# ShreyasBhaktharam/RDEIC

Hardware: AMD Instinct MI355X
Metric: 512x512 images/sec encode+relay-decode @ fixed bpp; 1/2/4/8 GPU (higher is better)
Workload: dtype bf16; 1 GPU; config 2: global batch 16 (16/GPU) 512x512, 2-step relay DDIM, encode+entropy-code+decode+VAE-decode; global_batch=16, image_size=512, ddim_steps=2, sampler=ddim, parallelism=dp1, codec_sessions_per_gpu=5

## Files before the change

### include/rdeic_hip.h

```cpp
#ifndef RDEIC_HIP_H
#define RDEIC_HIP_H
#include <stddef.h>
#include <stdint.h>
#ifdef __cplusplus
extern "C" {
#endif

int rdeic_version(void);
int rdeic_abi_count(void);

typedef struct rdeic_conv_desc {
  const void* in0;
  const void* in1;
  int32_t c0, c1;
  int32_t ld0, ld1;
  int32_t n, h, w;
  int32_t up2;
  const void* weight;
  int32_t wld;
  const float* bias;
  int32_t cout, kh, kw, stride, pad_t, pad_l;
  int32_t ho, wo;
  const float* gn_ab;
  int32_t gn_silu;
  const float* emb;
  int32_t emb_ld;
  int32_t act;
  float act_param;
  const void* res;
  int32_t res_ld;
  void* out;
  int32_t out_ld;
  int32_t out_mode;
  int32_t dtype;
  int32_t out_f32;
  int32_t batch;
  int64_t in_bs, w_bs, out_bs;
  float* gn_part;
  int32_t gn_hw;
  int32_t reserved;
  const float* ln_rows;
  const float* ln_colsum;
} rdeic_conv_desc;

int rdeic_conv2d(const rdeic_conv_desc* d, void* stream);
int rdeic_conv2d_tile(const rdeic_conv_desc* d, int32_t tile, void* stream);
int rdeic_conv2d_splitk(const rdeic_conv_desc* d, int32_t splits, float* ws, size_t ws_floats, void* stream);
int rdeic_conv2d_up2_phases(const rdeic_conv_desc* d, int64_t phase_stride, int32_t tile, void* stream);
int rdeic_conv2d_up2_group(const rdeic_conv_desc* d);
int rdeic_conv2d_band_rows(const rdeic_conv_desc* d, int32_t row_tile);
int rdeic_set_conv_path(int32_t path);
int rdeic_set_conv_option(int32_t key, int32_t value);

size_t rdeic_groupnorm_ws_floats(int32_t n, int32_t hw, int32_t c);
size_t rdeic_groupnorm_parts_floats(int64_t rows, int32_t c, int32_t hw);
int rdeic_groupnorm_parts_ab(const float* p0, int32_t c0, const float* p1, int32_t c1, int32_t n, int32_t hw,
                             int32_t groups, float eps, const float* gamma, const float* beta, float* ab,
                             void* stream);
int rdeic_groupnorm_stats(const void* x0, int32_t c0, int32_t ld0, const void* x1, int32_t c1, int32_t ld1,
                          int32_t n, int32_t hw, int32_t groups, float eps, const float* gamma, const float* beta,
                          float* ab, float* ws, int32_t dtype, void* stream);
int rdeic_groupnorm_parts_apply(const float* p0, int32_t c0, const float* p1, int32_t c1, const void* x0, int32_t ld0,
                                const void* x1, int32_t ld1, int32_t n, int32_t hw, int32_t groups, float eps,
                                const float* gamma, const float* beta, int32_t silu, float* ab, void* y, int32_t yld,
                                void* stream);
int rdeic_groupnorm_apply(const void* x, int32_t n, int32_t hw, int32_t c, int32_t ld, const float* ab,
                          int32_t ab_c, int32_t silu, float out_mul, void* y, int32_t yld, int32_t dtype,
                          void* stream);
int rdeic_layernorm(const void* x, int32_t rows, int32_t c, int32_t ld, const float* gamma, const float* beta,
                    float eps, void* y, int32_t yld, int32_t dtype, void* stream);

int rdeic_attention(const void* q, int32_t ldq, const void* k, int32_t ldk, const void* v, int32_t ldv,
                    void* o, int32_t ldo, int32_t batch, int32_t heads, int32_t lq, int32_t lk, int32_t dh,
                    float scale, int32_t kv_bcast, int32_t dtype, void* stream);
int rdeic_softmax_rows(const float* s, int64_t rows, int32_t cols, float scale, void* p, int32_t dtype, void* stream);
int rdeic_transpose(const void* in, int32_t rows, int32_t cols, int32_t ldin, void* out, int32_t ldout,
                    int32_t batch, int64_t in_bs, int64_t out_bs, int32_t dtype, void* stream);
int rdeic_attention_causal(const void* q, int32_t ldq, const void* k, int32_t ldk, const void* v, int32_t ldv,
                           void* o, int32_t ldo, int32_t batch, int32_t heads, int32_t l, int32_t dh,
                           float scale, int32_t dtype, void* stream);
int rdeic_embed_tokens(const float* table, int32_t ld_table, const float* pos, int32_t ld_pos, const int32_t* tokens,
                       int32_t batch, int32_t context, int32_t width, void* out, int32_t ld_out, int32_t dtype,
                       void* stream);

int rdeic_geglu(const void* in, int32_t rows, int32_t c, int32_t ldin, void* out, int32_t ldout,
                int32_t dtype, void* stream);
int rdeic_nchw_to_nhwc(const float* in, int32_t n, int32_t c, int32_t h, int32_t w, float mul, float add,
                       void* out, int32_t ld, int32_t dtype, void* stream);
int rdeic_nhwc_to_nchw(const void* in, int32_t n, int32_t c, int32_t h, int32_t w, int32_t ld, float mul,
                       float add, float* out, int32_t dtype, void* stream);
int rdeic_axpby(const float* x, const float* z, int32_t n_img, int32_t per_img, const float* a,
                const float* b, float* y, void* stream);
int rdeic_timestep_embedding(const int64_t* t, const float* freqs, int32_t n, int32_t dim, float* out, void* stream);
int rdeic_ddim_step(const float* x, const float* e, int64_t count, float c_sq1m, float c_sqa, float c_sqap,
                    float c_dir, float* xp, float* x0, void* stream);
int rdeic_cfg_combine(const float* e_cond, const float* e_uncond, int64_t count, float scale, float* out,
                      void* stream);
int rdeic_spaced_step(const float* x, const float* e, const float* noise, int64_t count, float a, float b, float c1,
                      float c2, float s, float* xp, float* x0, void* stream);
int rdeic_silu_f32(const float* x, float* y, int64_t count, void* stream);
int rdeic_image_u8_to_nhwc(const uint8_t* img, int32_t n, int32_t h, int32_t w, void* out, int32_t ld,
                           int32_t dtype, void* stream);
int rdeic_nhwc_to_image_u8(const void* x, int32_t n, int32_t h, int32_t w, int32_t ld, uint8_t* img,
                           int32_t dtype, void* stream);
int rdeic_image_mse(const uint8_t* a, const uint8_t* b, int32_t n, int64_t per_img, float* out, void* stream);
int rdeic_fill_uniform(float* out, int64_t count, uint64_t seed, float scale, float offset, void* stream);
int rdeic_pack_conv_weight(const float* w, int32_t cout, int32_t cin, int32_t kh, int32_t kw, void* out,
                           int32_t wld, int32_t dtype, void* stream);
int rdeic_cast(const void* in, int32_t in_dtype, void* out, int32_t out_dtype, int64_t count, void* stream);

int rdeic_resample_v_u8(const uint8_t* src, int64_t src_stride, int32_t src_row_bytes, int32_t src_row0,
                        int32_t src_rows, const int32_t* bounds, const int32_t* kk, int32_t ksize,
                        int32_t out_size, int32_t y0, int32_t nrows, int32_t cb0, int32_t ncb, uint8_t* dst,
                        int64_t dst_stride, void* stream);
int rdeic_resample_h_u8(const uint8_t* src, int64_t src_stride, int32_t src_h, int32_t src_w,
                        const int32_t* bounds, const int32_t* kk, int32_t ksize, int32_t out_size,
                        int32_t seg_max, int32_t y0, int32_t nrows, int32_t x0, int32_t npix, uint8_t* dst,
                        int64_t dst_stride, void* stream);
int rdeic_crop_flip_u8(const uint8_t* src, int64_t src_stride, int32_t src_h, int32_t src_w, int32_t crop_y,
                       int32_t crop_x, int32_t h, int32_t w, int32_t hflip, int32_t vflip, int32_t transpose,
                       uint8_t* dst, void* stream);

int rdeic_ckbd_encode(const void* y, int32_t yld, const void* params, int32_t pld, int32_t n, int32_t hy,
                      int32_t wy, int32_t c, int32_t phase, const float* scale_table, int32_t levels,
                      float scale_bound, int32_t* sym, int32_t* idx, int64_t img_stride, int64_t off,
                      void* yhat, int32_t yhld, void* anchor_out, int32_t ald, int32_t dtype, void* stream);
int rdeic_ckbd_indexes(const void* params, int32_t pld, int32_t n, int32_t hy, int32_t wy, int32_t c,
                       int32_t phase, const float* scale_table, int32_t levels, float scale_bound,
                       int32_t* idx, int64_t img_stride, int64_t off, int32_t dtype, void* stream);
int rdeic_ckbd_dequant(const int32_t* sym, const void* params, int32_t pld, int32_t n, int32_t hy,
                       int32_t wy, int32_t c, int32_t phase, int64_t img_stride, int64_t off, void* yhat,
                       int32_t yhld, void* anchor_out, int32_t ald, int32_t dtype, void* stream);
int rdeic_vq_argmin(const float* dot, const float* zn, const float* en, int32_t rows, int32_t ncode, int32_t* idx,
                    void* stream);
int rdeic_gather_rows(const float* table, int32_t ld_table, const int32_t* idx, int32_t rows, int32_t dim,
                      void* out, int32_t ld_out, int32_t dtype, void* stream);
int rdeic_row_sqnorm(const void* x, int32_t rows, int32_t dim, int32_t ld, float* out, int32_t dtype,
                     void* stream);

size_t rdeic_image_ssim_ws_floats(int32_t n, int32_t h, int32_t w, int32_t levels);
int rdeic_image_ssim(const uint8_t* a, const uint8_t* b, int32_t n, int32_t h, int32_t w, int32_t levels, float* ws,
                     size_t ws_floats, float* out, void* stream);

int rdeic_lpips_prep(const uint8_t* img, int32_t n, int32_t h, int32_t w, float* out, void* stream);
int rdeic_maxpool2d(const float* in, int32_t n, int32_t h, int32_t w, int32_t c, int32_t ld_in, int32_t k,
                    int32_t s, float* out, int32_t ld_out, void* stream);
size_t rdeic_lpips_layer_ws_floats(int32_t n, int64_t hw, int32_t c);
int rdeic_lpips_layer(const float* f0, int32_t ld0, const float* f1, int32_t ld1, const float* lin, int32_t n,
                      int64_t hw, int32_t c, int32_t accumulate, float* ws, size_t ws_floats, float* out,
                      void* stream);
int rdeic_lpips_prep_float(const void* img, int32_t ld, int32_t dtype, int64_t npix, float* out, void* stream);
int rdeic_lpips_layer_bwd(const float* f0, int32_t ld0, const float* f1, int32_t ld1, const float* lin,
                          const float* gscore, int32_t n, int64_t hw, int32_t c, int32_t accumulate, float* df0,
                          int32_t ldd, void* stream);
int rdeic_maxpool2d_bwd(const float* in, int32_t n, int32_t h, int32_t w, int32_t c, int32_t ld_in, const float* dy,
                        int32_t ld_dy, int32_t k, int32_t s, float* dx, int32_t ld_dx, void* stream);
int rdeic_conv_dgrad_small(const float* dz, int32_t ld_dz, const float* z, int32_t ld_z, const float* wt, int32_t n,
                           int32_t h, int32_t w, int32_t cin, int32_t cout, int32_t kh, int32_t kw, int32_t stride,
                           int32_t pad, int32_t prep_bwd, void* dx, int32_t ld_dx, int32_t dx_dtype, void* stream);

int rdeic_pmf_to_quantized_cdf(const float* pmf, int32_t n, int32_t precision, uint32_t* cdf_out);
int rdeic_build_gaussian_tables(const float* pmf, const int32_t* pmf_len, int32_t levels, int32_t pmf_ld,
                                int32_t* cdf, int32_t cdf_ld, int32_t* cdf_len, void* reserved);

int rdeic_rans_encode(const int32_t* sym, const int32_t* idx, size_t n, const int32_t* cdf, int32_t cdf_ld,
                      const int32_t* cdf_len, const int32_t* offset, int32_t levels, uint8_t* out, size_t cap,
                      size_t* out_len);
int rdeic_rans_encode_batch(int32_t count, const int32_t* sym, const int32_t* idx, size_t n_per,
                            size_t stride, const int32_t* cdf, int32_t cdf_ld, const int32_t* cdf_len,
                            const int32_t* offset, int32_t levels, uint8_t* out, size_t cap_per,
                            size_t* out_len, int32_t threads);
void* rdeic_rans_enc_tables_create(const int32_t* cdf, int32_t cdf_ld, const int32_t* cdf_len,
                                   const int32_t* offset, int32_t levels);
void rdeic_rans_enc_tables_destroy(void* tables);
int rdeic_rans_encode_batch_t(const void* tables, int32_t count, const int32_t* sym, const int32_t* idx,
                              size_t n_per, size_t stride, uint8_t* out, size_t cap_per, size_t* out_len,
                              int32_t threads);
int rdeic_rans_enc_quotient(const void* tables, int32_t row, int32_t value, uint64_t x, uint64_t* q);
void* rdeic_rans_dec_open(const uint8_t* data, size_t len);
int rdeic_rans_decode(void* handle, const int32_t* idx, size_t n, const int32_t* cdf, int32_t cdf_ld,
                      const int32_t* cdf_len, const int32_t* offset, int32_t levels, int32_t* out);
int rdeic_rans_decode_batch(int32_t count, void** handles, const int32_t* idx, size_t n_per, size_t stride,
                            const int32_t* cdf, int32_t cdf_ld, const int32_t* cdf_len, const int32_t* offset,
                            int32_t levels, int32_t* out, int32_t threads);
void rdeic_rans_dec_close(void* handle);

int rdeic_ac_encode(const int16_t* sym, size_t n, const int16_t* cdf_row, int32_t lp, uint8_t* out,
                    size_t cap, size_t* out_len);
int rdeic_ac_decode(const uint8_t* data, size_t len, size_t n, const int16_t* cdf_row, int32_t lp,
                    int16_t* out);
int rdeic_ac_uniform_cdf(int32_t codebook_size, int16_t* cdf_row);

#define RDEIC_PROF_CONV 0
#define RDEIC_PROF_ATTN 1
#define RDEIC_PROF_ATTN_SMALL 2
#define RDEIC_PROF_GN_STATS 3
#define RDEIC_PROF_GN_APPLY 4
#define RDEIC_PROF_GEMM 5
#define RDEIC_PROF_ATTN_D512 6
#define RDEIC_PROF_CONV_BYTES 7
int rdeic_prof_start(int32_t capacity, int32_t every);
int rdeic_prof_read_keys(int32_t kind, int64_t* keys, int64_t* launches, double* work, double* ms, int32_t cap);
#define RDEIC_COUNT_HALO_CONV 0
#define RDEIC_COUNT_GN_APPLY 1
#define RDEIC_COUNT_LAYERNORM 2
#define RDEIC_COUNT_HALO_SMALL 3
#define RDEIC_COUNT_LN_FUSED 4
#define RDEIC_COUNT_SPLITK 5
#define RDEIC_COUNT_EDGE 6
#define RDEIC_COUNT_GN_PARTS_APPLY 7
#define RDEIC_COUNT_DMA_CONV 8
#define RDEIC_COUNT_UP2_PHASES 9
#define RDEIC_COUNT_KINDS 10
int64_t rdeic_launch_count(int32_t kind);
int rdeic_layernorm_rowstats(const void* x, int32_t rows, int32_t c, int32_t ld, float eps, float* ms,
                             void* stream);
int rdeic_launch_count_reset(void);
int rdeic_prof_stop(void);
int rdeic_prof_read(int32_t kind, int64_t* launches, double* work, double* ms);

typedef struct rdeic_gemm_desc {
  const void* a;
  int64_t a_bs1, a_bs2, a_sm, a_sk;
  const void* b;
  int64_t b_bs1, b_bs2, b_sk, b_sn;
  void* c;
  int64_t c_bs1, c_bs2, c_sm;
  int32_t batch, nb2, m, n, k, ksplit, dtype, c_f32;
  float alpha, beta;
  float* rsum;
  int64_t rsum_bs;
} rdeic_gemm_desc;
int rdeic_gemm_strided(const rdeic_gemm_desc* d, void* stream);
int rdeic_pack_conv_weight_dgrad(const float* w, int32_t cout, int32_t cin, int32_t kh, int32_t kw, void* out,
                                 int32_t wld, int32_t to_bf16, void* stream);
typedef struct rdeic_pack_job {
  const float* w;
  void* out;
  int64_t start;
  int32_t cout, cin, kh, kw, wld, mode;
} rdeic_pack_job;
int rdeic_pack_batch(const rdeic_pack_job* jobs, int32_t njobs, int64_t total, int32_t row_floats, int32_t to_bf16,
                     void* stream);
int rdeic_zero_insert2(const void* src, int32_t n, int32_t h, int32_t w, int32_t c, int32_t ld, void* dst,
                       int32_t dst_ld, int32_t dtype, void* stream);
int rdeic_sum_pool2(const void* src, int32_t n, int32_t h, int32_t w, int32_t c, int32_t ld, void* dst,
                    int32_t dst_ld, int32_t dtype, void* stream);
int rdeic_pixel_unshuffle2(const void* src, int32_t n, int32_t h, int32_t w, int32_t c, int32_t ld, void* dst,
                           int32_t dst_ld, int32_t dtype, void* stream);
int rdeic_im2col(const void* x, int32_t n, int32_t h, int32_t w, int32_t c, int32_t ld, int32_t kh, int32_t kw,
                 int32_t stride, int32_t pad_t, int32_t pad_l, int32_t ho, int32_t wo, int32_t up2, void* out,
                 int64_t out_ld, int32_t dtype, void* stream);
int rdeic_wgrad_finalize(const float* part, int32_t splits, int32_t cout, int32_t cin, int32_t kh, int32_t kw,
                         float* dw, int32_t accumulate, const float* rpart, float* db, void* stream);
size_t rdeic_col_sum_ws_floats(int64_t rows, int32_t c, int32_t groups);
int rdeic_col_sum(const void* x, int64_t rows, int32_t c, int32_t ld, int32_t groups, float* out, int32_t accumulate,
                  float* ws, size_t ws_floats, int32_t dtype, void* stream);
int rdeic_act_fwd(const void* z, int64_t rows, int32_t c, int32_t ldz, const void* res, int32_t ldr, int32_t act,
                  float slope, void* out, int32_t ldo, int32_t dtype, void* stream);
int rdeic_act_bwd(const void* dy, int32_t ldy, const void* z, int32_t ldz, int64_t rows, int32_t c, int32_t act,
                  float slope, void* dz, int32_t lddz, int32_t dtype, void* stream);
size_t rdeic_gn_train_ws_doubles(int32_t n, int32_t hw, int32_t c);
int rdeic_gn_train_fwd(const void* x, int32_t ldx, int32_t n, int32_t hw, int32_t c, int32_t groups, float eps,
                       const float* gamma, const float* beta, float* mr, float* ab, double* ws, int32_t dtype,
                       void* stream);
int rdeic_gn_train_bwd(const void* x, int32_t ldx, const void* dy, int32_t ldy, int32_t n, int32_t hw, int32_t c,
                       int32_t groups, const float* mr, const float* gamma, const float* beta, int32_t silu, void* dx,
                       int32_t lddx, float* dgamma, float* dbeta, int32_t accumulate, double* ws, float* coef,
                       int32_t dtype, void* stream);
int rdeic_gn_train_bwd_res(const void* x, int32_t ldx, const void* dy, int32_t ldy, int32_t n, int32_t hw, int32_t c,
                           int32_t groups, const float* mr, const float* gamma, const float* beta, int32_t silu,
                           const void* dres, int32_t ldr, void* dx, int32_t lddx, float* dgamma, float* dbeta,
                           int32_t accumulate, double* ws, float* coef, int32_t dtype, void* stream);
size_t rdeic_layernorm_bwd_ws_floats(int64_t rows, int32_t c);
int rdeic_layernorm_bwd(const void* x, int32_t ldx, int64_t rows, int32_t c, const float* gamma, float eps,
                        const void* dy, int32_t ldy, void* dx, int32_t lddx, float* dgamma, float* dbeta,
                        int32_t accumulate, float* ws, size_t ws_floats, int32_t dtype, void* stream);
int rdeic_layernorm_bwd_res(const void* x, int32_t ldx, int64_t rows, int32_t c, const float* gamma, float eps,
                            const void* dy, int32_t ldy, const void* dres, int32_t ldr, void* dx, int32_t lddx,
                            float* dgamma, float* dbeta, int32_t accumulate, float* ws, size_t ws_floats,
                            int32_t dtype, void* stream);
int rdeic_softmax_bwd_rows(const void* p, const float* dp, int64_t rows, int32_t cols, float scale, void* ds,
                           int32_t dtype, void* stream);
int rdeic_attention_fwd_lse(const void* q, int32_t ldq, const void* k, int32_t ldk, const void* v, int32_t ldv,
                            void* o, int32_t ldo, float* lse, int32_t batch, int32_t heads, int32_t lq, int32_t lk,
                            int32_t dh, float scale, int32_t dtype, void* stream);
size_t rdeic_attention_bwd_workspace(int32_t batch, int32_t heads, int32_t lq, int32_t lk, int32_t dh);
int rdeic_attention_bwd(const void* q, int32_t ldq, const void* k, int32_t ldk, const void* v, int32_t ldv,
                        const void* o, int32_t ldo, const void* d_o, int32_t lddo, const float* lse,
                        void* dq, int32_t lddq, void* dk, int32_t lddk, void* dv, int32_t lddv,
                        void* ws, size_t ws_bytes, int32_t batch, int32_t heads, int32_t lq, int32_t lk,
                        int32_t dh, float scale, int32_t dtype, void* stream);
int rdeic_geglu_bwd(const void* x, int32_t ldx, int64_t rows, int32_t c, const void* dy, int32_t ldy, void* dx,
                    int32_t lddx, int32_t dtype, void* stream);
int rdeic_ckbd_train_anchor(const void* y, int32_t ldy, const void* pa, int32_t ldpa, int32_t n, int32_t h, int32_t w,
                            int32_t c, void* out, int32_t ldo, int32_t dtype, void* stream);
int rdeic_ckbd_mask(const void* x, int32_t ldx, int32_t n, int32_t h, int32_t w, int32_t c, int32_t which, void* out,
                    int32_t ldo, int32_t dtype, void* stream);
size_t rdeic_ckbd_train_ws_doubles(int32_t n, int32_t h, int32_t w, int32_t c);
int rdeic_ckbd_train_lik(const void* y, int32_t ldy, const void* pa, int32_t ldpa, const void* pn, int32_t ldpn,
                         const float* noise, int32_t n, int32_t h, int32_t w, int32_t c, void* nonanchor_hat,
                         int32_t ldo, double* ws, float* out2, int32_t dtype, void* stream);
int rdeic_ckbd_train_lik_bwd(const void* y, int32_t ldy, const void* pa, int32_t ldpa, const void* pn, int32_t ldpn,
                             const float* noise, int32_t n, int32_t h, int32_t w, int32_t c, const float* g_sum,
                             const void* d_nonanchor, int32_t ldd, void* dy, int32_t lddy, void* dpa, int32_t lddpa,
                             void* dpn, int32_t lddpn, int32_t dtype, void* stream);
int rdeic_vq_train(const float* dot, const float* zn, const float* en, const float* z, const int32_t* idx, int32_t P,
                   int32_t K, int32_t D, float* E, float* embed_prob, float beta, float decay, float temp,
                   float* code_out, float* dE_unit, float* loss3, void* stream);
int rdeic_vq_z_grad(const float* z, const float* zq, const void* dzq, int64_t count, const float* g_loss, float coef,
                    void* dz, int32_t dtype, void* stream);
int rdeic_scale_dev(const float* x, int64_t count, const float* s, float* y, int32_t accumulate, void* stream);
int rdeic_adamw(float* p, const float* g, float* m, float* v, int64_t count, float lr, float beta1, float beta2,
                float eps, float weight_decay, int32_t step, void* stream);
int rdeic_adamw_dev(float* p, const float* g, float* m, float* v, int64_t count, float lr, float beta1, float beta2,
                    float eps, float weight_decay, const float* step_scalars, void* stream);

#ifdef __cplusplus
}
#endif
#endif
```

### rdeic_amd/_lib.py

```python
from __future__ import annotations

import ctypes as C
import os
import threading

_HERE = os.path.dirname(os.path.abspath(__file__))
LIB_PATH = os.environ.get("RDEIC_LIB") or os.path.join(_HERE, "lib", "librdeic_hip.so")

EINVAL, ENOSPC, EBADMSG, ELAUNCH = -22, -28, -74, -5
_ERRNAMES = {EINVAL: "EINVAL (bad argument/shape)", ENOSPC: "ENOSPC (output capacity)",
             EBADMSG: "EBADMSG (corrupt or truncated bitstream)", ELAUNCH: "kernel launch failure"}


class RdeicError(RuntimeError):
    def __init__(self, fn: str, code: int):
        super().__init__(f"{fn} failed: {code} {_ERRNAMES.get(code, '')}")
        self.code = code


class BitstreamError(RdeicError, ValueError):
    """Corrupt / truncated bitstream (the reference's 'decode failure')."""


class ConvDesc(C.Structure):
    _fields_ = [
        ("in0", C.c_void_p), ("in1", C.c_void_p),
        ("c0", C.c_int32), ("c1", C.c_int32), ("ld0", C.c_int32), ("ld1", C.c_int32),
        ("n", C.c_int32), ("h", C.c_int32), ("w", C.c_int32), ("up2", C.c_int32),
        ("weight", C.c_void_p), ("wld", C.c_int32),
        ("bias", C.c_void_p),
        ("cout", C.c_int32), ("kh", C.c_int32), ("kw", C.c_int32), ("stride", C.c_int32),
        ("pad_t", C.c_int32), ("pad_l", C.c_int32),
        ("ho", C.c_int32), ("wo", C.c_int32),
        ("gn_ab", C.c_void_p), ("gn_silu", C.c_int32),
        ("emb", C.c_void_p), ("emb_ld", C.c_int32),
        ("act", C.c_int32), ("act_param", C.c_float),
        ("res", C.c_void_p), ("res_ld", C.c_int32),
        ("out", C.c_void_p), ("out_ld", C.c_int32), ("out_mode", C.c_int32),
        ("dtype", C.c_int32), ("out_f32", C.c_int32),
        ("batch", C.c_int32), ("in_bs", C.c_int64), ("w_bs", C.c_int64), ("out_bs", C.c_int64),
        ("gn_part", C.c_void_p), ("gn_hw", C.c_int32), ("reserved", C.c_int32),
        ("ln_rows", C.c_void_p), ("ln_colsum", C.c_void_p),
    ]


class GemmDesc(C.Structure):
    _fields_ = [
        ("a", C.c_void_p), ("a_bs1", C.c_int64), ("a_bs2", C.c_int64), ("a_sm", C.c_int64), ("a_sk", C.c_int64),
        ("b", C.c_void_p), ("b_bs1", C.c_int64), ("b_bs2", C.c_int64), ("b_sk", C.c_int64), ("b_sn", C.c_int64),
        ("c", C.c_void_p), ("c_bs1", C.c_int64), ("c_bs2", C.c_int64), ("c_sm", C.c_int64),
        ("batch", C.c_int32), ("nb2", C.c_int32), ("m", C.c_int32), ("n", C.c_int32), ("k", C.c_int32),
        ("ksplit", C.c_int32), ("dtype", C.c_int32), ("c_f32", C.c_int32),
        ("alpha", C.c_float), ("beta", C.c_float), ("rsum", C.c_void_p), ("rsum_bs", C.c_int64),
    ]


_p, _i32, _i64, _u64, _f, _sz = C.c_void_p, C.c_int32, C.c_int64, C.c_uint64, C.c_float, C.c_size_t

PROTOTYPES = {
    "rdeic_version": (C.c_int, []),
    "rdeic_abi_count": (C.c_int, []),
    "rdeic_conv2d": (C.c_int, [C.POINTER(ConvDesc), _p]),
    "rdeic_conv2d_splitk": (C.c_int, [C.POINTER(ConvDesc), _i32, _p, C.c_size_t, _p]),
    "rdeic_conv2d_tile": (C.c_int, [C.POINTER(ConvDesc), _i32, _p]),
    "rdeic_conv2d_up2_phases": (C.c_int, [C.POINTER(ConvDesc), _i64, _i32, _p]),
    "rdeic_conv2d_up2_group": (C.c_int, [C.POINTER(ConvDesc)]),
    "rdeic_conv2d_band_rows": (C.c_int, [C.POINTER(ConvDesc), _i32]),
    "rdeic_prof_start": (C.c_int, [_i32, _i32]),
    "rdeic_prof_stop": (C.c_int, []),
    "rdeic_launch_count": (C.c_int64, [_i32]),
    "rdeic_launch_count_reset": (C.c_int, []),
    "rdeic_layernorm_rowstats": (C.c_int, [C.c_void_p, _i32, _i32, _i32, C.c_float, C.c_void_p, C.c_void_p]),
    "rdeic_prof_read": (C.c_int, [_i32, C.POINTER(C.c_int64), C.POINTER(C.c_double), C.POINTER(C.c_double)]),
    "rdeic_prof_read_keys": (C.c_int, [_i32, C.POINTER(C.c_int64), C.POINTER(C.c_int64), C.POINTER(C.c_double),
                                       C.POINTER(C.c_double), _i32]),
    "rdeic_groupnorm_ws_floats": (_sz, [_i32, _i32, _i32]),
    "rdeic_groupnorm_stats": (C.c_int, [_p, _i32, _i32, _p, _i32, _i32, _i32, _i32, _i32, _f, _p, _p, _p, _p,
                                        _i32, _p]),
    "rdeic_groupnorm_apply": (C.c_int, [_p, _i32, _i32, _i32, _i32, _p, _i32, _i32, _f, _p, _i32, _i32, _p]),
    "rdeic_set_conv_path": (C.c_int, [_i32]),
    "rdeic_set_conv_option": (C.c_int, [_i32, _i32]),
    "rdeic_layernorm": (C.c_int, [_p, _i32, _i32, _i32, _p, _p, _f, _p, _i32, _i32, _p]),
    "rdeic_softmax_rows": (C.c_int, [_p, _i64, _i32, _f, _p, _i32, _p]),
    "rdeic_transpose": (C.c_int, [_p, _i32, _i32, _i32, _p, _i32, _i32, _i64, _i64, _i32, _p]),
    "rdeic_attention": (C.c_int, [_p, _i32, _p, _i32, _p, _i32, _p, _i32, _i32, _i32, _i32, _i32, _i32, _f,
                                  _i32, _i32, _p]),
    "rdeic_attention_causal": (C.c_int, [_p, _i32, _p, _i32, _p, _i32, _p, _i32, _i32, _i32, _i32, _i32, _f, _i32,
                                         _p]),
    "rdeic_embed_tokens": (C.c_int, [_p, _i32, _p, _i32, _p, _i32, _i32, _i32, _p, _i32, _i32, _p]),
    "rdeic_geglu": (C.c_int, [_p, _i32, _i32, _i32, _p, _i32, _i32, _p]),
    "rdeic_nchw_to_nhwc": (C.c_int, [_p, _i32, _i32, _i32, _i32, _f, _f, _p, _i32, _i32, _p]),
    "rdeic_nhwc_to_nchw": (C.c_int, [_p, _i32, _i32, _i32, _i32, _i32, _f, _f, _p, _i32, _p]),
    "rdeic_axpby": (C.c_int, [_p, _p, _i32, _i32, _p, _p, _p, _p]),
    "rdeic_timestep_embedding": (C.c_int, [_p, _p, _i32, _i32, _p, _p]),
    "rdeic_ddim_step": (C.c_int, [_p, _p, _i64, _f, _f, _f, _f, _p, _p, _p]),
    "rdeic_spaced_step": (C.c_int, [_p, _p, _p, _i64, _f, _f, _f, _f, _f, _p, _p, _p]),
    "rdeic_cfg_combine": (C.c_int, [_p, _p, _i64, _f, _p, _p]),
    "rdeic_silu_f32": (C.c_int, [_p, _p, _i64, _p]),
    "rdeic_image_u8_to_nhwc": (C.c_int, [_p, _i32, _i32, _i32, _p, _i32, _i32, _p]),
    "rdeic_nhwc_to_image_u8": (C.c_int, [_p, _i32, _i32, _i32, _i32, _p, _i32, _p]),
    "rdeic_image_mse": (C.c_int, [_p, _p, _i32, _i64, _p, _p]),
    "rdeic_fill_uniform": (C.c_int, [_p, _i64, _u64, _f, _f, _p]),
    "rdeic_pack_conv_weight": (C.c_int, [_p, _i32, _i32, _i32, _i32, _p, _i32, _i32, _p]),
    "rdeic_cast": (C.c_int, [_p, _i32, _p, _i32, _i64, _p]),
    "rdeic_resample_v_u8": (C.c_int, [_p, _i64, _i32, _i32, _i32, _p, _p, _i32, _i32, _i32, _i32, _i32, _i32, _p,
                                      _i64, _p]),
    "rdeic_resample_h_u8": (C.c_int, [_p, _i64, _i32, _i32, _p, _p, _i32, _i32, _i32, _i32, _i32, _i32, _i32, _p,
                                      _i64, _p]),
    "rdeic_crop_flip_u8": (C.c_int, [_p, _i64, _i32, _i32, _i32, _i32, _i32, _i32, _i32, _i32, _i32, _p, _p]),
    "rdeic_ckbd_encode": (C.c_int, [_p, _i32, _p, _i32, _i32, _i32, _i32, _i32, _i32, _p, _i32, _f, _p, _p,
                                    _i64, _i64, _p, _i32, _p, _i32, _i32, _p]),
    "rdeic_ckbd_indexes": (C.c_int, [_p, _i32, _i32, _i32, _i32, _i32, _i32, _p, _i32, _f, _p, _i64, _i64,
                                     _i32, _p]),
    "rdeic_ckbd_dequant": (C.c_int, [_p, _p, _i32, _i32, _i32, _i32, _i32, _i32, _i64, _i64, _p, _i32, _p,
                                     _i32, _i32, _p]),
    "rdeic_vq_argmin": (C.c_int, [_p, _p, _p, _i32, _i32, _p, _p]),
    "rdeic_gather_rows": (C.c_int, [_p, _i32, _p, _i32, _i32, _p, _i32, _i32, _p]),
    "rdeic_row_sqnorm": (C.c_int, [_p, _i32, _i32, _i32, _p, _i32, _p]),
    "rdeic_pmf_to_quantized_cdf": (C.c_int, [_p, _i32, _i32, _p]),
    "rdeic_build_gaussian_tables": (C.c_int, [_p, _p, _i32, _i32, _p, _i32, _p, _p]),
    "rdeic_rans_encode": (C.c_int, [_p, _p, _sz, _p, _i32, _p, _p, _i32, _p, _sz, C.POINTER(_sz)]),
    "rdeic_rans_encode_batch": (C.c_int, [_i32, _p, _p, _sz, _sz, _p, _i32, _p, _p, _i32, _p, _sz, _p, _i32]),
    "rdeic_image_ssim_ws_floats": (C.c_size_t, [_i32, _i32, _i32, _i32]),
    "rdeic_image_ssim": (C.c_int, [_p, _p, _i32, _i32, _i32, _i32, _p, C.c_size_t, _p, _p]),
    "rdeic_lpips_prep": (C.c_int, [_p, _i32, _i32, _i32, _p, _p]),
    "rdeic_maxpool2d": (C.c_int, [_p, _i32, _i32, _i32, _i32, _i32, _i32, _i32, _p, _i32, _p]),
    "rdeic_lpips_layer_ws_floats": (_sz, [_i32, _i64, _i32]),
    "rdeic_lpips_layer": (C.c_int, [_p, _i32, _p, _i32, _p, _i32, _i64, _i32, _i32, _p, _sz, _p, _p]),
    "rdeic_lpips_prep_float": (C.c_int, [_p, _i32, _i32, _i64, _p, _p]),
    "rdeic_lpips_layer_bwd": (C.c_int, [_p, _i32, _p, _i32, _p, _p, _i32, _i64, _i32, _i32, _p, _i32, _p]),
    "rdeic_maxpool2d_bwd": (C.c_int, [_p, _i32, _i32, _i32, _i32, _i32, _p, _i32, _i32, _i32, _p, _i32, _p]),
    "rdeic_conv_dgrad_small": (C.c_int, [_p, _i32, _p, _i32, _p, _i32, _i32, _i32, _i32, _i32, _i32, _i32, _i32,
                                         _i32, _i32, _p, _i32, _i32, _p]),
    "rdeic_groupnorm_parts_floats": (C.c_size_t, [_i64, _i32, _i32]),
    "rdeic_groupnorm_parts_ab": (C.c_int, [_p, _i32, _p, _i32, _i32, _i32, _i32, _f, _p, _p, _p, _p]),
    "rdeic_groupnorm_parts_apply": (C.c_int, [_p, _i32, _p, _i32, _p, _i32, _p, _i32, _i32, _i32, _i32, _f, _p, _p,
                                              _i32, _p, _p, _i32, _p]),
    "rdeic_rans_enc_tables_create": (_p, [_p, _i32, _p, _p, _i32]),
    "rdeic_rans_enc_tables_destroy": (None, [_p]),
    "rdeic_rans_encode_batch_t": (C.c_int, [_p, _i32, _p, _p, _sz, _sz, _p, _sz, _p, _i32]),
    "rdeic_rans_enc_quotient": (C.c_int, [_p, _i32, _i32, C.c_uint64, C.POINTER(C.c_uint64)]),
    "rdeic_rans_dec_open": (_p, [_p, _sz]),
    "rdeic_rans_decode": (C.c_int, [_p, _p, _sz, _p, _i32, _p, _p, _i32, _p]),
    "rdeic_rans_decode_batch": (C.c_int, [_i32, _p, _p, _sz, _sz, _p, _i32, _p, _p, _i32, _p, _i32]),
    "rdeic_rans_dec_close": (None, [_p]),
    "rdeic_ac_encode": (C.c_int, [_p, _sz, _p, _i32, _p, _sz, C.POINTER(_sz)]),
    "rdeic_ac_decode": (C.c_int, [_p, _sz, _sz, _p, _i32, _p]),
    "rdeic_ac_uniform_cdf": (C.c_int, [_i32, _p]),
    "rdeic_gemm_strided": (C.c_int, [C.POINTER(GemmDesc), _p]),
    "rdeic_pack_conv_weight_dgrad": (C.c_int, [_p, _i32, _i32, _i32, _i32, _p, _i32, _i32, _p]),
    "rdeic_pack_batch": (C.c_int, [_p, _i32, _i64, _i32, _i32, _p]),
    "rdeic_zero_insert2": (C.c_int, [_p, _i32, _i32, _i32, _i32, _i32, _p, _i32, _i32, _p]),
    "rdeic_sum_pool2": (C.c_int, [_p, _i32, _i32, _i32, _i32, _i32, _p, _i32, _i32, _p]),
    "rdeic_pixel_unshuffle2": (C.c_int, [_p, _i32, _i32, _i32, _i32, _i32, _p, _i32, _i32, _p]),
    "rdeic_im2col": (C.c_int, [_p, _i32, _i32, _i32, _i32, _i32, _i32, _i32, _i32, _i32, _i32, _i32, _i32, _i32, _p,
                               _i64, _i32, _p]),
    "rdeic_wgrad_finalize": (C.c_int, [_p, _i32, _i32, _i32, _i32, _i32, _p, _i32, _p, _p, _p]),
    "rdeic_col_sum_ws_floats": (_sz, [_i64, _i32, _i32]),
    "rdeic_col_sum": (C.c_int, [_p, _i64, _i32, _i32, _i32, _p, _i32, _p, _sz, _i32, _p]),
    "rdeic_act_fwd": (C.c_int, [_p, _i64, _i32, _i32, _p, _i32, _i32, _f, _p, _i32, _i32, _p]),
    "rdeic_act_bwd": (C.c_int, [_p, _i32, _p, _i32, _i64, _i32, _i32, _f, _p, _i32, _i32, _p]),
    "rdeic_gn_train_ws_doubles": (_sz, [_i32, _i32, _i32]),
    "rdeic_gn_train_fwd": (C.c_int, [_p, _i32, _i32, _i32, _i32, _i32, _f, _p, _p, _p, _p, _p, _i32, _p]),
    "rdeic_gn_train_bwd": (C.c_int, [_p, _i32, _p, _i32, _i32, _i32, _i32, _i32, _p, _p, _p, _i32, _p, _i32, _p, _p,
                                     _i32, _p, _p, _i32, _p]),
    "rdeic_gn_train_bwd_res": (C.c_int, [_p, _i32, _p, _i32, _i32, _i32, _i32, _i32, _p, _p, _p, _i32, _p, _i32, _p,
                                         _i32, _p, _p, _i32, _p, _p, _i32, _p]),
    "rdeic_layernorm_bwd_ws_floats": (_sz, [_i64, _i32]),
    "rdeic_layernorm_bwd": (C.c_int, [_p, _i32, _i64, _i32, _p, _f, _p, _i32, _p, _i32, _p, _p, _i32, _p, _sz, _i32,
                                      _p]),
    "rdeic_layernorm_bwd_res": (C.c_int, [_p, _i32, _i64, _i32, _p, _f, _p, _i32, _p, _i32, _p, _i32, _p, _p, _i32, _p,
                                          _sz, _i32, _p]),
    "rdeic_softmax_bwd_rows": (C.c_int, [_p, _p, _i64, _i32, _f, _p, _i32, _p]),
    "rdeic_attention_fwd_lse": (C.c_int, [_p, _i32, _p, _i32, _p, _i32, _p, _i32, _p, _i32, _i32, _i32, _i32, _i32, _f,
                                          _i32, _p]),
    "rdeic_attention_bwd_workspace": (_sz, [_i32, _i32, _i32, _i32, _i32]),
    "rdeic_attention_bwd": (C.c_int, [_p, _i32, _p, _i32, _p, _i32, _p, _i32, _p, _i32, _p, _p, _i32, _p, _i32, _p,
                                      _i32, _p, _sz, _i32, _i32, _i32, _i32, _i32, _f, _i32, _p]),
    "rdeic_geglu_bwd": (C.c_int, [_p, _i32, _i64, _i32, _p, _i32, _p, _i32, _i32, _p]),
    "rdeic_ckbd_train_anchor": (C.c_int, [_p, _i32, _p, _i32, _i32, _i32, _i32, _i32, _p, _i32, _i32, _p]),
    "rdeic_ckbd_mask": (C.c_int, [_p, _i32, _i32, _i32, _i32, _i32, _i32, _p, _i32, _i32, _p]),
    "rdeic_ckbd_train_ws_doubles": (_sz, [_i32, _i32, _i32, _i32]),
    "rdeic_ckbd_train_lik": (C.c_int, [_p, _i32, _p, _i32, _p, _i32, _p, _i32, _i32, _i32, _i32, _p, _i32, _p, _p,
                                       _i32, _p]),
    "rdeic_ckbd_train_lik_bwd": (C.c_int, [_p, _i32, _p, _i32, _p, _i32, _p, _i32, _i32, _i32, _i32, _p, _p, _i32, _p,
                                           _i32, _p, _i32, _p, _i32, _i32, _p]),
    "rdeic_vq_train": (C.c_int, [_p, _p, _p, _p, _p, _i32, _i32, _i32, _p, _p, _f, _f, _f, _p, _p, _p, _p]),
    "rdeic_vq_z_grad": (C.c_int, [_p, _p, _p, _i64, _p, _f, _p, _i32, _p]),
    "rdeic_scale_dev": (C.c_int, [_p, _i64, _p, _p, _i32, _p]),
    "rdeic_adamw": (C.c_int, [_p, _p, _p, _p, _i64, _f, _f, _f, _f, _f, _i32, _p]),
    "rdeic_adamw_dev": (C.c_int, [_p, _p, _p, _p, _i64, _f, _f, _f, _f, _f, _p, _p]),
}

_lib = None
_lock = threading.Lock()


def load() -> C.CDLL:
    global _lib
    if _lib is not None:
        return _lib
    with _lock:
        if _lib is not None:
            return _lib
        if not os.path.exists(LIB_PATH):
            raise ImportError(f"librdeic_hip.so not built at {LIB_PATH}; run `make` (or __graft_entry__.build()).")
        import torch
        lib = C.CDLL(LIB_PATH, mode=C.RTLD_GLOBAL)
        for name, (res, args) in PROTOTYPES.items():
            fn = getattr(lib, name)
            fn.restype = res
            fn.argtypes = args
        _lib = lib
    return _lib


def check(name: str, rc: int) -> None:
    if rc != 0:
        if rc == EBADMSG:
            raise BitstreamError(name, rc)
# ... 24 lines not shown
```

### rdeic_amd/compression.py

```python
from __future__ import annotations

from typing import List, Sequence, Tuple

import numpy as np
import torch

from . import coders, ops
from .params import ParamStore
from .plan import PlanCache, host_step

LEAK = 0.01


class Compression:
    def __init__(self, store: ParamStore, in_nc: int, out_nc: int, N: int, M: int, slice_num: int,
                 slice_ch: Sequence[int], codebook_size: int, prefix: str = "preprocess_model."):
        self.store, self.p = store, prefix
        self.N, self.M = N, M
        self.slice_num, self.slice_ch = slice_num, list(slice_ch)
        self.slice_off = [sum(self.slice_ch[:i]) for i in range(slice_num)]
        self.codebook_size = codebook_size
        p = prefix
        d = store
        self.g_a = []
        spec = [("rb", in_nc, M), ("rb", M, M), ("rb", M, M), ("rb", M, M), ("rbs", M, M), ("rb", M, M),
                ("rb", M, M), ("rb", M, M)]
        for i, (kind, ci, co) in enumerate(spec):
            self.g_a.append(self._declare_block(f"{p}encoder.g_a.{i}", kind, ci, co))
        d.declare_conv(f"{p}encoder.g_a.8", M, M, 3)
        self.g_a.append((f"{p}encoder.g_a.8", "conv", M, M))
        self.hyper_enc = [self._declare_block(f"{p}hyper_enc.hyper_enc.{i}", k, ci, co) for i, (k, ci, co) in
                          enumerate([("rb", M, N), ("rb", N, N), ("rbs", N, N), ("rbs", N, N)])]
        self.hyper_dec = [self._declare_block(f"{p}hyper_dec.hyper_dec.{i}", k, ci, co) for i, (k, ci, co) in
                          enumerate([("rbu", N, M), ("rbu", M, M), ("rb", M, M * 3 // 2), ("rb", M * 3 // 2, M * 2)])]
        d.declare_conv(f"{p}decoder.g_s.0", M, M, 3)
        self.g_s = [(f"{p}decoder.g_s.0", "conv", M, M)]
        for i, (k, ci, co) in enumerate([("rb", M, M)] * 3 + [("rbu", M, M)] + [("rb", M, M)] * 4):
            self.g_s.append(self._declare_block(f"{p}decoder.g_s.{i + 1}", k, ci, co))
        d.declare_conv(f"{p}out", out_nc, M, 3)
        for i, c in enumerate(self.slice_ch):
            d.declare_conv(f"{p}local_context.{i}", 2 * c, c, 5)
            if i:
                cin = sum(self.slice_ch[:i])
                d.declare_conv(f"{p}channel_context.{i}.fushion.0", 224, cin, 5)
                d.declare_conv(f"{p}channel_context.{i}.fushion.2", 128, 224, 5)
                d.declare_conv(f"{p}channel_context.{i}.fushion.4", 2 * c, 128, 5)
            for nm, cin in (("entropy_parameters_anchor", 2 * M + (2 * c if i else 0)),
                            ("entropy_parameters_nonanchor", 2 * M + (4 * c if i else 2 * c))):
                out = 2 * c
                d.declare_conv(f"{p}{nm}.{i}.fusion.0", out * 5 // 3, cin, 1)
                d.declare_conv(f"{p}{nm}.{i}.fusion.2", out * 4 // 3, out * 5 // 3, 1)
                d.declare_conv(f"{p}{nm}.{i}.fusion.4", out, out * 4 // 3, 1)
        d.declare(f"{p}quantize.embedding.weight", (codebook_size, N))
        self.tables = None
        self._en = None
        self.coder_groups = 1
        self.use_plans = True
        self._plans = PlanCache()
        self._io = {}

    def _declare_block(self, pre, kind, ci, co):
        d = self.store
        if kind == "rb":
            d.declare_conv(pre + ".conv1", co, ci, 3)
            d.declare_conv(pre + ".conv2", co, co, 3)
            if ci != co:
                d.declare_conv(pre + ".adaptor", co, ci, 1)
        elif kind == "rbs":
            d.declare_conv(pre + ".conv1", co, ci, 3)
            d.declare_conv(pre + ".conv2", co, co, 3)
            d.declare_conv(pre + ".downsample", co, ci, 1)
        elif kind == "rbu":
            d.declare_conv(pre + ".subpel_conv.0", co * 4, ci, 1)
            d.declare_conv(pre + ".conv", co, co, 3)
            d.declare_conv(pre + ".upsample.0", co * 4, ci, 1)
        return (pre, kind, ci, co)

    def update(self, scale_table=None, force: bool = False):
        if self.tables is None or force or scale_table is not None:
            self.tables = coders.GaussianTables(scale_table)
            self._plans.clear()
        return True

    def _block(self, blk, x):
        pre, kind, ci, co = blk
        s = self.store
        if kind == "conv":
            return ops.conv2d(x, s.conv(pre))
        if kind == "rb":
            identity = x if ci == co else ops.conv2d(x, s.conv(pre + ".adaptor"))
            out = ops.conv2d(x, s.conv(pre + ".conv1"), act=ops.LEAKY, slope=LEAK)
            return ops.conv2d(out, s.conv(pre + ".conv2"), act=ops.LEAKY, slope=LEAK, res=identity)
        if kind == "rbs":
            out = ops.conv2d(x, s.conv(pre + ".conv1", stride=2, pad=1), act=ops.LEAKY, slope=LEAK)
            identity = ops.conv2d(x, s.conv(pre + ".downsample", stride=2, pad=0))
            return ops.conv2d(out, s.conv(pre + ".conv2"), act=ops.LEAKY, slope=0.1, res=identity)
        if kind == "rbu":
            out = ops.conv2d(x, s.conv(pre + ".subpel_conv.0"), pixel_shuffle=True, act=ops.LEAKY, slope=LEAK)
            identity = ops.conv2d(x, s.conv(pre + ".upsample.0"), pixel_shuffle=True)
            return ops.conv2d(out, s.conv(pre + ".conv"), act=ops.LEAKY, slope=0.1, res=identity)
        raise ValueError(kind)

    def _seq(self, blocks, x):
        for b in blocks:
            x = self._block(b, x)
        return x

    def _pad_width(self, c: int):
        if self.store.compute_dtype != torch.bfloat16:
            return None
        return -(-c // 64) * 64 if c > 32 else -(-c // 16) * 16

    def _ep(self, name: str, i: int, x: torch.Tensor, x2: torch.Tensor) -> torch.Tensor:
        s, p = self.store, self.p
        f0, f2, f4 = (f"{p}{name}.{i}.fusion.{j}" for j in (0, 2, 4))
        w0, w2 = s.shapes[f0 + ".weight"][0], s.shapes[f2 + ".weight"][0]
        p0, p2 = self._pad_width(w0), self._pad_width(w2)
        h = ops.conv2d(x, s.conv(f0, cout_pad=p0), x2=x2, act=ops.GELU)
        h = ops.conv2d(h, s.conv(f2, cin_pad=p0, cout_pad=p2), act=ops.GELU)
        return ops.conv2d(h, s.conv(f4, cin_pad=p2))

    def _channel_ctx(self, i: int, yhat_prefix: torch.Tensor, out: torch.Tensor) -> torch.Tensor:
        s, p = self.store, self.p
        f0, f2, f4 = (f"{p}channel_context.{i}.fushion.{j}" for j in (0, 2, 4))
        p0 = self._pad_width(s.shapes[f0 + ".weight"][0])
        h = ops.conv2d(yhat_prefix, s.conv(f0, cout_pad=p0), act=ops.GELU)
        h = ops.conv2d(h, s.conv(f2, cin_pad=p0), act=ops.GELU)
        return ops.conv2d(h, s.conv(f4), out=out)

    def _codebook(self) -> torch.Tensor:
        return self.store.get(self.p + "quantize.embedding.weight")

    def vq_quant(self, z: torch.Tensor):
        B, hz, wz, N = z.shape
        rows = B * hz * wz
        E = self._codebook()
        zf = ops.cast(z.contiguous(), torch.float32).view(rows, N)
        zn = torch.empty(rows, dtype=torch.float32, device=z.device)
        ops.call("rdeic_row_sqnorm", zf.data_ptr(), rows, N, N, zn.data_ptr(), 0, ops.stream_ptr())
        if self._en is None or self._en.device != z.device:
            self._en = torch.empty(E.shape[0], dtype=torch.float32, device=z.device)
            ops.call("rdeic_row_sqnorm", E.data_ptr(), E.shape[0], N, N, self._en.data_ptr(), 0, ops.stream_ptr())
        dot = ops.linear(zf, self.store.conv(self.p + "quantize.embedding", dtype=torch.float32), images=B)
        idx = torch.empty(rows, dtype=torch.int32, device=z.device)
        ops.call("rdeic_vq_argmin", dot.data_ptr(), zn.data_ptr(), self._en.data_ptr(), rows, E.shape[0],
                 idx.data_ptr(), ops.stream_ptr())
        return self.codebook_entry(idx, B, hz, wz), idx.view(B, hz, wz)

    def codebook_entry(self, idx: torch.Tensor, B: int, hz: int, wz: int) -> torch.Tensor:
        E = self._codebook()
        N = E.shape[1]
        zq = torch.empty((B, hz, wz, N), dtype=self.store.compute_dtype, device=E.device)
        ops.call("rdeic_gather_rows", E.data_ptr(), N, idx.contiguous().data_ptr(), B * hz * wz, N, zq.data_ptr(), N,
                 ops.dt_code(zq), ops.stream_ptr())
        return zq

    def _pinned(self, key: str, n: int, dtype=torch.int32) -> torch.Tensor:
        cache = self.__dict__.setdefault("_pin_cache", {})
        buf = cache.get(key)
        if buf is None or buf.numel() < n or buf.dtype != dtype:
            buf = torch.empty(max(n, 1), dtype=dtype, pin_memory=True)
            cache[key] = buf
        return buf[:n]

    def stage_sizes(self, hy: int, wy: int) -> List[int]:
        sizes = []
        for c in self.slice_ch:
            sizes += [c * hy * (wy // 2)] * 2
        return sizes

    def _stage_common(self, hy, wy, B, device, dt):
        yhat = torch.empty((B, hy, wy, self.M), dtype=dt, device=device)
        cmax = max(self.slice_ch)
        ctx = torch.empty((B, hy, wy, 4 * cmax), dtype=dt, device=device)
        anchor = torch.empty((B, hy, wy, cmax), dtype=dt, device=device)
        return yhat, ctx, anchor

    def _stage_gen(self, hyper, hy, wy, emit, bufs):
        yhat, ctxbuf, anchor_full = bufs
        off = 0
        for i, c in enumerate(self.slice_ch):
            s0 = self.slice_off[i]
            ctx = ctxbuf[..., :4 * c]
            anchor = anchor_full[..., :c]
            if i == 0:
                pa = self._ep("entropy_parameters_anchor", 0, hyper, None)
            else:
                self._channel_ctx(i, yhat[..., :s0], out=ctx[..., 2 * c:4 * c])
                pa = self._ep("entropy_parameters_anchor", i, ctx[..., 2 * c:4 * c], hyper)
            r = emit(i, 0, pa, c, off, yhat[..., s0:s0 + c], anchor)
            if r is not None:
                yield from r
            off += c * hy * (wy // 2)
            ops.conv2d(anchor, self.store.conv(f"{self.p}local_context.{i}"), out=ctx[..., :2 * c])
            pn = self._ep("entropy_parameters_nonanchor", i, ctx[..., :(4 * c if i else 2 * c)], hyper)
            r = emit(i, 1, pn, c, off, yhat[..., s0:s0 + c], None)
            if r is not None:
                yield from r
            off += c * hy * (wy // 2)

    def _run_stages(self, hyper, B, hy, wy, emit):
        bufs = self._stage_common(hy, wy, B, hyper.device, hyper.dtype)
        for _ in self._stage_gen(hyper, hy, wy, emit, bufs):
            pass
        return bufs[0]

    def _groups(self, B: int) -> List[Tuple[int, int]]:
        g = max(1, min(int(self.coder_groups), B))
        cut = [B * k // g for k in range(g + 1)]
        return [(cut[k], cut[k + 1]) for k in range(g)]

    @staticmethod
    def _interleave(gens) -> None:
        live = list(gens)
        while live:
            for g in list(live):
                try:
                    next(g)
                except StopIteration:
                    live.remove(g)

    def _run_region(self, name, fn, inputs, before=None):
        if not self.use_plans:
            if before is not None:
                before()
            return fn(*inputs)
        key = (name, self.coder_groups) + tuple((tuple(t.shape), t.dtype) for t in inputs)
        return self._plans.run(key, fn, inputs, before=before)

    def _splitk(self):
        import contextlib
        if self.store.compute_dtype == torch.bfloat16 and ops.SPLITK_ENTROPY:
            return ops.splitk_allowed()
        return contextlib.nullcontext()

    def _compress_gpu(self, h: torch.Tensor) -> torch.Tensor:
        with self._splitk():
            return self._compress_gpu_body(h)

    def _compress_gpu_body(self, h: torch.Tensor) -> torch.Tensor:
        B = h.shape[0]
        y = self._seq(self.g_a, h)
        z = self._seq(self.hyper_enc, y)
        z_q, z_idx = self.vq_quant(z)
        hyper = self._seq(self.hyper_dec, z_q)
        _, hy, wy, _ = y.shape
        total = sum(self.stage_sizes(hy, wy))
        table = self.tables.device_scale_table(h.device)
        dtc = ops.dt_code(h)
        bufs = self._stage_common(hy, wy, B, h.device, hyper.dtype)
        zi_p = self._pinned("enc_zidx", z_idx.numel()).view(z_idx.shape)
        host_step(lambda: zi_p.copy_(z_idx, non_blocking=True))

        def group(gi: int, b0: int, b1: int):
            nb = b1 - b0
            yg = y[b0:b1]
            sym_p = self._pinned(f"enc_sym{gi}", nb * total).view(nb, total)
            idx_p = self._pinned(f"enc_idx{gi}", nb * total).view(nb, total)
            done = torch.cuda.Event()

            def emit(i, phase, params, c, off, yhat_slice, anchor):
                s0 = self.slice_off[i]
                ys = yg[..., s0:s0 + c]
                ops.call("rdeic_ckbd_encode", ys.data_ptr(), ops.pix_ld(ys), params.data_ptr(), ops.pix_ld(params), nb,
                         hy, wy, c, phase, table.data_ptr(), table.numel(), float(coders.SCALE_BOUND), sym_p.data_ptr(),
                         idx_p.data_ptr(), total, off, yhat_slice.data_ptr(), ops.pix_ld(yhat_slice),
                         None if anchor is None else anchor.data_ptr(), 0 if anchor is None else ops.pix_ld(anchor),
                         dtc, ops.stream_ptr())

            yield from self._stage_gen(hyper[b0:b1], hy, wy, emit, [t[b0:b1] for t in bufs])

            def to_host():
                done.record()
# ... 113 lines not shown
```

### rdeic_amd/csrc/coders.cpp

```cpp
#include <stdint.h>
#include <string.h>

#include <algorithm>
#include <atomic>
#include <condition_variable>
#include <functional>
#include <mutex>
#include <cmath>
#include <new>
#include <stdexcept>
#include <thread>
#include <vector>

#include "../../include/rdeic_hip.h"

#define RDEIC_OK 0
#define RDEIC_EINVAL (-22)
#define RDEIC_ENOSPC (-28)
#define RDEIC_EBADMSG (-74)

namespace {

constexpr int kPrecision = 16;
constexpr uint32_t kBypassBits = 4;
// ... 244 lines not shown
  }
  return d->bad ? RDEIC_EBADMSG : RDEIC_OK;
}

class WorkerPool {
 public:
  static WorkerPool& get() {
    thread_local WorkerPool* p = new WorkerPool();
    return *p;
  }
  void run(int32_t count, int32_t threads, const std::function<void(int32_t)>& f) {
    std::lock_guard<std::mutex> job(job_mu_);
    int32_t helpers = std::max(0, std::min(threads, count) - 1);
    while ((int32_t)workers_.size() < helpers) {
      const int32_t id = (int32_t)workers_.size();
      try {
        workers_.reserve(workers_.size() + 1);
        std::thread(&WorkerPool::loop, this, id).detach();
      } catch (...) {
        helpers = (int32_t)workers_.size();
        break;
      }
      workers_.push_back(id);
    }
    {
      std::lock_guard<std::mutex> lk(mu_);
      fn_ = &f;
      count_ = count;
      next_.store(0);
      helpers_ = helpers;
      active_ = helpers;
      ++gen_;
    }
    cv_.notify_all();
    work();
    std::unique_lock<std::mutex> lk(mu_);
    done_cv_.wait(lk, [&] { return active_ == 0; });
    fn_ = nullptr;
  }

 private:
  void work() {
    for (;;) {
      const int32_t i = next_.fetch_add(1);
      if (i >= count_) break;
      (*fn_)(i);
    }
  }
  void loop(int32_t id) {
    uint64_t seen = 0;
    for (;;) {
      {
        std::unique_lock<std::mutex> lk(mu_);
        cv_.wait(lk, [&] { return gen_ != seen; });
        seen = gen_;
        if (id >= helpers_) continue;
      }
      work();
      std::lock_guard<std::mutex> lk(mu_);
      if (--active_ == 0) done_cv_.notify_all();
    }
  }

  std::mutex job_mu_, mu_;
  std::condition_variable cv_, done_cv_;
  std::vector<int32_t> workers_;
  const std::function<void(int32_t)>* fn_ = nullptr;
  std::atomic<int32_t> next_{0};
  int32_t count_ = 0, active_ = 0, helpers_ = 0;
  uint64_t gen_ = 0;
};

template <typename F>
int guard(F&& f) noexcept {
  try {
    return f();
  } catch (const std::bad_alloc&) {
    return RDEIC_ENOSPC;
  } catch (...) {
    return RDEIC_EINVAL;
  }
}

template <typename F>
void parallel_for(int32_t count, int32_t threads, F&& f) {
  if (threads <= 1 || count <= 1) {
    for (int32_t i = 0; i < count; ++i) f(i);
    return;
  }
  const std::function<void(int32_t)> fn = f;
  WorkerPool::get().run(count, threads, fn);
}

struct BitWriter {
  uint8_t* out;
  size_t cap;
  size_t len = 0;
  uint8_t cache = 0;
  int count = 0;
  bool overflow = false;
  void put(int bit) {
    cache = (uint8_t)((cache << 1) | (bit & 1));
    if (++count == 8) {
      if (len < cap) out[len] = cache; else overflow = true;
      ++len;
      count = 0;
      cache = 0;
    }
  }
  void put_with_pending(int bit, uint64_t& pending) {
    put(bit);
    while (pending > 0) { put(!bit); --pending; }
  }
  void flush() {
    while (count > 0) put(0);
  }
};

struct BitReader {
  const uint8_t* in;
  size_t n;
  size_t ptr = 0;
  uint8_t cache = 0;
  int cached = 0;
  void get(uint32_t& value) {
    if (cached == 0) {
      if (ptr == n) { value <<= 1; return; }
      cache = in[ptr++];
      cached = 8;
    }
    value = (value << 1) | ((cache >> (cached - 1)) & 1);
    --cached;
  }
};

inline uint16_t binsearch_u16(const uint16_t* cdf, uint16_t target, uint16_t max_sym) {
  uint16_t left = 0, right = (uint16_t)(max_sym + 1);
  while (left + 1 < right) {
    const uint16_t m = (uint16_t)((left + right) / 2);
    const uint16_t v = cdf[m];
    if (v < target) left = m;
    else if (v > target) right = m;
    else return m;
  }
  return left;
}

}

extern "C" {

int rdeic_version(void) { return 1; }

int rdeic_abi_count(void) { return 112; }

static int pmf_to_quantized_cdf_impl(const float* pmf, int32_t n, int32_t precision, uint32_t* cdf_out) {
  if (!pmf || !cdf_out || n <= 0 || precision <= 0 || precision > 24) return RDEIC_EINVAL;
  for (int32_t i = 0; i < n; ++i)
    if (!(pmf[i] >= 0.f) || !std::isfinite(pmf[i])) return RDEIC_EINVAL;
  const uint32_t one = 1u << precision;
  std::vector<uint32_t> cdf((size_t)n + 1);
  cdf[0] = 0;
  for (int32_t i = 0; i < n; ++i) cdf[i + 1] = (uint32_t)std::round(pmf[i] * (float)one);
  uint64_t total = 0;
  for (uint32_t v : cdf) total += v;
  if (total == 0) return RDEIC_EINVAL;
  for (auto& v : cdf) v = (uint32_t)(((uint64_t)one * v) / total);
  for (size_t i = 1; i < cdf.size(); ++i) cdf[i] += cdf[i - 1];
  cdf.back() = one;
  const int32_t m = (int32_t)cdf.size();
  for (int32_t i = 0; i < m - 1; ++i) {
    if (cdf[i] == cdf[i + 1]) {
      uint32_t best_freq = ~0u;
      int32_t best = -1;
      for (int32_t j = 0; j < m - 1; ++j) {
        const uint32_t f = cdf[j + 1] - cdf[j];
        if (f > 1 && f < best_freq) { best_freq = f; best = j; }
      }
      if (best < 0) return RDEIC_EINVAL;
      if (best < i) {
        for (int32_t j = best + 1; j <= i; ++j) cdf[j]--;
      } else {
        for (int32_t j = i + 1; j <= best; ++j) cdf[j]++;
      }
    }
  }
  memcpy(cdf_out, cdf.data(), cdf.size() * sizeof(uint32_t));
  return RDEIC_OK;
}

int rdeic_pmf_to_quantized_cdf(const float* pmf, int32_t n, int32_t precision, uint32_t* cdf_out) {
  return guard([&] { return pmf_to_quantized_cdf_impl(pmf, n, precision, cdf_out); });
}

static int build_gaussian_tables_impl(const float* pmf, const int32_t* pmf_len, int32_t levels, int32_t pmf_ld,
                                      int32_t* cdf, int32_t cdf_ld, int32_t* cdf_len) {
  if (!pmf || !pmf_len || !cdf || !cdf_len || levels <= 0) return RDEIC_EINVAL;
  std::vector<float> row;
  std::vector<uint32_t> q;
  for (int32_t i = 0; i < levels; ++i) {
    const int32_t L = pmf_len[i];
    if (L <= 0 || L + 1 > pmf_ld || L + 2 > cdf_ld) return RDEIC_EINVAL;
    row.assign(pmf + (size_t)i * pmf_ld, pmf + (size_t)i * pmf_ld + L + 1);
    q.assign((size_t)L + 2, 0u);
    int rc = pmf_to_quantized_cdf_impl(row.data(), L + 1, kPrecision, q.data());
    if (rc) return rc;
    int32_t* out = cdf + (size_t)i * cdf_ld;
    for (int32_t j = 0; j < cdf_ld; ++j) out[j] = j < L + 2 ? (int32_t)q[j] : 0;
    cdf_len[i] = L + 2;
  }
  return RDEIC_OK;
}

int rdeic_build_gaussian_tables(const float* pmf, const int32_t* pmf_len, int32_t levels, int32_t pmf_ld, int32_t* cdf,
                                int32_t cdf_ld, int32_t* cdf_len, void* reserved) {
  (void)reserved;
  return guard([&] { return build_gaussian_tables_impl(pmf, pmf_len, levels, pmf_ld, cdf, cdf_ld, cdf_len); });
}

int rdeic_rans_encode(const int32_t* sym, const int32_t* idx, size_t n, const int32_t* cdf, int32_t cdf_ld,
                      const int32_t* cdf_len, const int32_t* offset, int32_t levels, uint8_t* out, size_t cap,
                      size_t* out_len) {
  if ((!sym || !idx) && n) return RDEIC_EINVAL;
  if (!cdf || !cdf_len || !offset || !out || !out_len || levels <= 0) return RDEIC_EINVAL;
  return guard([&] {
    std::vector<RansSym> syms;
    std::vector<uint32_t> words;
    return rans_encode_impl(sym, idx, n, cdf, cdf_ld, cdf_len, offset, levels, out, cap, out_len, syms, words);
  });
}

int rdeic_rans_encode_batch(int32_t count, const int32_t* sym, const int32_t* idx, size_t n_per, size_t stride,
                            const int32_t* cdf, int32_t cdf_ld, const int32_t* cdf_len, const int32_t* offset,
                            int32_t levels, uint8_t* out, size_t cap_per, size_t* out_len, int32_t threads) {
  if (count <= 0 || !sym || !idx || !out || !out_len) return RDEIC_EINVAL;
  return guard([&] {
    std::vector<int> rc(count, 0);
    parallel_for(count, threads, [&](int32_t i) {
      rc[i] = guard([&] {
        std::vector<RansSym> syms;
        std::vector<uint32_t> words;
        return rans_encode_impl(sym + i * stride, idx + i * stride, n_per, cdf, cdf_ld, cdf_len, offset, levels,
                                out + i * cap_per, cap_per, &out_len[i], syms, words);
      });
    });
    for (int v : rc)
      if (v) return v;
    return (int)RDEIC_OK;
  });
}

void* rdeic_rans_enc_tables_create(const int32_t* cdf, int32_t cdf_ld, const int32_t* cdf_len, const int32_t* offset,
                                   int32_t levels) {
  if (!cdf || !cdf_len || !offset || levels <= 0 || cdf_ld < 2) return nullptr;
  EncTables* T = new (std::nothrow) EncTables();
  if (!T) return nullptr;
  try {
    T->levels = levels;
    T->row_off.resize(levels);
    T->max_value.resize(levels);
    T->offset.assign(offset, offset + levels);
    size_t total = 0;
    for (int32_t ci = 0; ci < levels; ++ci) {
      const int32_t len = cdf_len[ci];
      if (len < 2 || len > cdf_ld) throw std::invalid_argument("cdf_len");
      T->row_off[ci] = (int32_t)total;
      T->max_value[ci] = len - 2;
      total += (size_t)len - 1;
    }
    T->sym.resize(total);
    for (int32_t ci = 0; ci < levels; ++ci) {
      const int32_t* row = cdf + (size_t)ci * cdf_ld;
      for (int32_t v = 0; v <= T->max_value[ci]; ++v) {
        const int32_t start = row[v], freq = row[v + 1] - row[v];
        if (start < 0 || freq <= 0 || start + freq > (1 << kPrecision)) throw std::invalid_argument("cdf row");
        T->sym[(size_t)T->row_off[ci] + v] = make_enc_sym((uint32_t)start, (uint32_t)freq);
      }
    }
  } catch (...) {
    delete T;
    return nullptr;
  }
  return T;
}

void rdeic_rans_enc_tables_destroy(void* tables) { delete (EncTables*)tables; }

int rdeic_rans_encode_batch_t(const void* tables, int32_t count, const int32_t* sym, const int32_t* idx, size_t n_per,
                              size_t stride, uint8_t* out, size_t cap_per, size_t* out_len, int32_t threads) {
  if (!tables || count <= 0 || ((!sym || !idx) && n_per) || !out || !out_len) return RDEIC_EINVAL;
  const EncTables& T = *(const EncTables*)tables;
  return guard([&] {
    std::vector<int> rc(count, 0);
    parallel_for(count, threads, [&](int32_t i) {
      rc[i] = guard([&] {
        thread_local std::vector<uint32_t> buf;
        return rans_encode_tab_impl(T, sym + i * stride, idx + i * stride, n_per, out + i * cap_per, cap_per,
                                    &out_len[i], buf);
      });
    });
    for (int v : rc)
      if (v) return v;
    return (int)RDEIC_OK;
  });
}

int rdeic_rans_enc_quotient(const void* tables, int32_t row, int32_t value, uint64_t x, uint64_t* q) {
// ... 151 lines not shown
```

### rdeic_amd/csrc/conv_common.h

```cpp
#pragma once
#include "common.h"
#include "../../include/rdeic_hip.h"
#include "prof.h"

namespace rdeic_conv {

struct ConvArgs {
  const char* in0; const char* in1;
  int c0, c1, ld0, ld1;
  int n, h, w, up2;
  const char* weight; int wld;
  const float* bias;
  int cout, kh, kw, stride, pad_t, pad_l, ho, wo;
  const float* gn_ab; int gn_silu;
  const float* emb; int emb_ld;
  int act; float act_param;
  const char* res; int res_ld;
  char* out; int out_ld, out_mode;
  int out_f32;
  int M, cin, ktot, nk;
  long in_bs, w_bs, out_bs;
  int batch;
  int epi_vec;
  int splits, kper;
// ... 316 lines not shown
  constexpr int WTM = BM / WGM;
  return (WTM == 32 || WTM == 64) && (WTM / P) % 16 == 0;
}

template <int BM, int BN, int WGM, int WGN, int NT, int P>
__device__ __forceinline__ void epilogue_geglu(const f32x4 (&acc)[BM / WGM / 16][BN / WGN / 16], const ConvArgs& a,
                                               int m0, int n0, int wm, int wn, int lane, int tid, char* lds) {
  constexpr int WTM = BM / WGM, WTN = BN / WGN;
  constexpr int TM = WTM / 16, TN = WTN / 16;
  constexpr int HM = TM / P;
  constexpr int PR = BM / P;
  constexpr int SDW = BN + 4;
  constexpr int DPR = BN / 16;
  constexpr int ND = (PR * DPR + NT - 1) / NT;
  constexpr int NPF = ND < 2 ? ND : 2;
  constexpr bool HOIST = (NT % DPR) == 0;
  static_assert(TM % P == 0 && BN % 16 == 0, "P passes, chunk pairs");
  const int lr = lane & 15, lq = lane >> 4;
  float* L = reinterpret_cast<float*>(lds);
  auto bar = []() { asm volatile("s_waitcnt lgkmcnt(0)\n\ts_barrier" ::: "memory"); };
  auto row_of = [&](int d, int p) {
    const int pr = d / DPR;
    const int wmr = pr / (WTM / P), wr = pr - wmr * (WTM / P);
    return m0 + wmr * WTM + p * (WTM / P) + wr;
  };
  float4 bh[4], chh[4];
#pragma unroll
  for (int q = 0; q < 4; ++q) bh[q] = chh[q] = float4{0.f, 0.f, 0.f, 0.f};
  if constexpr (HOIST) {
    const int nn = n0 + (tid % DPR) * 16;
    if (nn < a.cout) {
#pragma unroll
      for (int q = 0; q < 4; ++q) {
        if (a.bias) bh[q] = *reinterpret_cast<const float4*>(a.bias + nn + 4 * q);
        if (a.ln_rows) chh[q] = *reinterpret_cast<const float4*>(a.ln_cs + nn + 4 * q);
      }
    }
  }
#pragma unroll
  for (int p = 0; p < P; ++p) {
    float2 lpf[NPF];
#pragma unroll
    for (int k = 0; k < NPF; ++k) {
      const int d = tid + k * NT;
      const int m = row_of(d, p);
      lpf[k] = float2{0.f, 0.f};
      if (a.ln_rows && d < PR * DPR && m < a.M) lpf[k] = reinterpret_cast<const float2*>(a.ln_rows)[m];
    }
    bar();
#pragma unroll
    for (int ii = 0; ii < HM; ++ii)
#pragma unroll
      for (int r = 0; r < 4; ++r) {
        const int pr = wm * (WTM / P) + ii * 16 + lq * 4 + r;
#pragma unroll
        for (int j = 0; j < TN; ++j) L[pr * SDW + wn * WTN + j * 16 + lr] = acc[p * HM + ii][j][r];
      }
    bar();
#pragma unroll
    for (int k = 0; k < ND; ++k) {
      const int d = tid + k * NT;
      if (d >= PR * DPR) continue;
      const int pr = d / DPR, cq = d - pr * DPR;
      const int m = row_of(d, p);
      const int nn = n0 + cq * 16;
      if (m >= a.M || nn >= a.cout) continue;
      float v[16];
#pragma unroll
      for (int q = 0; q < 4; ++q) {
        const float4 x = *reinterpret_cast<const float4*>(L + pr * SDW + cq * 16 + 4 * q);
        v[4 * q] = x.x; v[4 * q + 1] = x.y; v[4 * q + 2] = x.z; v[4 * q + 3] = x.w;
      }
      if (a.ln_rows) {
        const float2 ms = k < NPF ? lpf[k < NPF ? k : 0] : reinterpret_cast<const float2*>(a.ln_rows)[m];
        const f32x2 nm = {-ms.x, -ms.x}, rs = {ms.y, ms.y};
#pragma unroll
        for (int q = 0; q < 4; ++q) {
          const float4 c = HOIST ? chh[q] : *reinterpret_cast<const float4*>(a.ln_cs + nn + 4 * q);
          const float cs[4] = {c.x, c.y, c.z, c.w};
#pragma unroll
          for (int e = 0; e < 4; e += 2) {
            const f32x2 r = rs * pk_fma(nm, f32x2{cs[e], cs[e + 1]}, f32x2{v[4 * q + e], v[4 * q + e + 1]});
            v[4 * q + e] = r.x;
            v[4 * q + e + 1] = r.y;
          }
        }
      }
      if (a.bias) {
#pragma unroll
        for (int q = 0; q < 4; ++q) {
          const float4 b = HOIST ? bh[q] : *reinterpret_cast<const float4*>(a.bias + nn + 4 * q);
          const f32x2 r0 = f32x2{v[4 * q], v[4 * q + 1]} + f32x2{b.x, b.y};
          const f32x2 r1 = f32x2{v[4 * q + 2], v[4 * q + 3]} + f32x2{b.z, b.w};
          v[4 * q] = r0.x; v[4 * q + 1] = r0.y; v[4 * q + 2] = r1.x; v[4 * q + 3] = r1.y;
        }
      }
#pragma unroll
      for (int e = 0; e < 16; ++e) v[e] = apply_act(v[e], a.act, a.act_param);
      bf16 gv[8];
#pragma unroll
      for (int h = 0; h < 2; ++h)
#pragma unroll
        for (int e = 0; e < 4; e += 2) {
          const f32x2 xv = {to_f32(from_f32<bf16>(v[8 * h + e])), to_f32(from_f32<bf16>(v[8 * h + e + 1]))};
          const f32x2 gt = {to_f32(from_f32<bf16>(v[8 * h + 4 + e])), to_f32(from_f32<bf16>(v[8 * h + 5 + e]))};
          const f32x2 r = xv * gelu_fast2(gt);
          gv[4 * h + e] = from_f32<bf16>(r.x);
          gv[4 * h + e + 1] = from_f32<bf16>(r.y);
        }
      *reinterpret_cast<uint4*>(reinterpret_cast<bf16*>(a.out) + (long)m * a.out_ld + (nn >> 1)) =
          *reinterpret_cast<uint4*>(gv);
    }
  }
}

constexpr unsigned kOOB = 0x80000000u;

template <int N>
__device__ __forceinline__ void wait_vm() {
  asm volatile("s_waitcnt vmcnt(%0)" ::"n"(N) : "memory");
}

__device__ __forceinline__ int dma_key(int r) { return (((r >> 3) & 1) << 1) | (((r >> 1) & 1) << 2); }

typedef __attribute__((address_space(3))) void* lds_ptr_t;

__device__ __forceinline__ void dma16(__amdgpu_buffer_rsrc_t rs, char* lds_dst, unsigned voff, int soff) {
  __builtin_amdgcn_raw_ptr_buffer_load_lds(rs, (lds_ptr_t)lds_dst, 16, (int)voff, soff, 0, 0);
}

#ifdef RDEIC_HALO_STAMPS
__device__ unsigned long long* g_halo_stamps;
#define HALO_STAMP(k)                                                                      \
  do {                                                                                     \
    if (threadIdx.x == 0) g_halo_stamps[(long)blockIdx.x * 8 + (k)] = __builtin_amdgcn_s_memtime(); \
  } while (0)
#else
#define HALO_STAMP(k) do {} while (0)
#endif

__device__ __forceinline__ void wait_vm_rt(int n) {
  switch (n) {
    case 0: wait_vm<0>(); break;
    case 1: wait_vm<1>(); break;
    case 2: wait_vm<2>(); break;
    case 3: wait_vm<3>(); break;
    case 4: wait_vm<4>(); break;
    case 5: wait_vm<5>(); break;
    case 6: wait_vm<6>(); break;
    default: wait_vm<7>(); break;
  }
}

extern int g_conv_path, g_epi_vec, g_swz, g_force_tile, g_dma, g_halo, g_halo8, g_edge, g_up2_phases;
extern int g_launch_limit;

long image_span(const rdeic_conv_desc* d);
int band_rows(const rdeic_conv_desc* d, int row_tile);
struct Band {
  int r0, rows;
  int i0, h;
  int pad_t;
};
Band band_at(const rdeic_conv_desc* d, int r0, int rows);

int make_args(const rdeic_conv_desc* d, ConvArgs& a, bool& vec);
bool dma_ok(const rdeic_conv_desc* d, const ConvArgs& a, unsigned& b0, unsigned& b1, unsigned& bw);
int launch_dma_auto(const ConvArgs& a, unsigned b0, unsigned b1, unsigned bw, hipStream_t s, int tile,
                    int gn_hw = 0, bool* fused = nullptr);
int dma_grouped(const rdeic_conv_desc* d, int tile, hipStream_t s, bool* fused = nullptr);
bool halo_ok(const rdeic_conv_desc* d, const ConvArgs& a);
int launch_halo(const rdeic_conv_desc* d, ConvArgs a, hipStream_t s, bool* fused);
int launch_edge(const rdeic_conv_desc* d, const ConvArgs& a, hipStream_t s, bool* fused);
int up2_phase_group(const rdeic_conv_desc* d);
bool up2_phases_ok(const rdeic_conv_desc* d, long phase_stride);
int launch_up2_phases(const rdeic_conv_desc* d, long phase_stride, int tile, hipStream_t s, bool* fused);
}
```

### rdeic_amd/csrc/conv_gemm.hip

```cpp
#include "conv_common.h"

namespace rdeic_conv {

int g_conv_path = 2;
int g_epi_vec = 1;
int g_swz = 1;
int g_force_tile = -1;
int g_dma = 1;
int g_halo = 1;
int g_halo8 = 1;
int g_up2_phases = 1;
int g_launch_limit = 0x7fffffff;

namespace {

template <typename T, int BM, int BN, int WGM, int WGN, bool VEC, bool GNP = true, bool SWZ = true>
__global__ __launch_bounds__(WGM * WGN * 64) void conv_kernel(ConvArgs a) {
  constexpr int NT = WGM * WGN * 64;
  constexpr int BK = MmaTraits<T>::BK;
  constexpr int EPC = MmaTraits<T>::EPC;
  constexpr int ES = sizeof(T);
  constexpr int WTM = BM / WGM, WTN = BN / WGN;
  constexpr int TM = WTM / 16, TN = WTN / 16;
  constexpr int RPI = NT / 8;
// ... 591 lines not shown
  const double b = d->batch > 1 ? d->batch : 1;
  const double es = d->dtype == 1 ? 2.0 : 4.0, os = (d->dtype == 0 || d->out_f32) ? 4.0 : 2.0;
  const double in = b * d->n * (double)d->h * d->w * (d->c0 + d->c1) * es;
  const double w = (double)(d->batch > 1 ? b : 1) * d->cout * d->wld * es;
  double outc = d->out_mode == 2 ? d->cout / 2.0 : (double)d->cout;
  const double out = b * d->n * (d->out_mode == 1 ? 4.0 : 1.0) * d->ho * d->wo * (d->out_mode == 1 ? outc / 4 : outc) * os;
  return in + w + out + (d->res ? out : 0.0);
}

static int conv2d_impl(const rdeic_conv_desc* d, int32_t tile, void* stream) {
  if (d && d->gn_part &&
      (d->gn_hw <= 0 || d->gn_hw % 64 || d->batch > 1 || d->out_mode != 0 || (long)d->n * d->ho * d->wo % d->gn_hw))
    return RDEIC_EINVAL;
  bool fused = false;
  int rc;
  {
    rdeic_prof_add_bytes(conv_bytes(d));
    ProfScope ps((hipStream_t)stream, RDEIC_PROF_CONV, conv_flops(d));
    rc = tile == -2 ? conv2d_run(d, stream, &fused) : conv2d_tile_run(d, tile, stream, &fused);
  }
  if (rc != RDEIC_OK || !d->gn_part || fused) return rc;
  const long rows = (long)d->n * d->ho * d->wo;
  return gn_rows_partial(d->out, rows, d->cout, d->out_ld, d->gn_hw, d->gn_part,
                         (d->out_f32 || d->dtype == 0) ? 0 : 1, (hipStream_t)stream);
}

static int conv2d_splitk_impl(const rdeic_conv_desc* d, int32_t splits, float* ws, size_t ws_floats,
                              void* stream) {
  ConvArgs a;
  bool vec = false;
  const int rc = make_args(d, a, vec);
  if (rc != RDEIC_OK) return rc;
  if (!vec || d->gn_ab || d->out_mode != 0 || a.batch != 1 || d->cout % 8 || splits < 2 || !ws ||
      (d->out_ld % 8) || ((uintptr_t)d->out % 16) || ((uintptr_t)ws % 16))
    return RDEIC_EINVAL;
  if (ws_floats < (size_t)splits * a.M * a.cout) return RDEIC_ENOSPC;
  hipStream_t s = (hipStream_t)stream;
  float* const part = ws;
  if (d->dtype == 0) {
    ConvArgs p = a;
    p.bias = nullptr; p.emb = nullptr; p.act = 0; p.res = nullptr; p.gn_part = nullptr; p.ln_rows = nullptr;
    p.out = (char*)part; p.out_ld = a.cout; p.out_f32 = 0;
    p.splits = splits;
    p.kper = (a.nk + splits - 1) / splits;
    dim3 grid(cdiv(a.M, 64), cdiv(a.cout, 64), splits);
    constexpr int lds = conv_lds_bytes<float, 64, 64>();
    hipLaunchKernelGGL((conv_kernel<float, 64, 64, 2, 2, true, false, true>), grid, dim3(256), lds, s, p);
    a.splits = splits;
    a.out_f32 = 1;
    const long chunks = (long)a.M * (a.cout / 8);
    hipLaunchKernelGGL(splitk_reduce_kernel, dim3((unsigned)((chunks + 255) / 256)), dim3(256), 0, s, a,
                       (const float*)part);
    return launch_status();
  }
  if (g_dma) {
    rdeic_conv_desc e = *d;
    e.bias = nullptr; e.emb = nullptr; e.act = 0; e.res = nullptr; e.gn_part = nullptr; e.ln_rows = nullptr;
    e.out = part; e.out_ld = d->cout; e.out_f32 = 1;
    ConvArgs pa;
    bool pv = false;
    unsigned b0, b1, bw;
    if (make_args(&e, pa, pv) == RDEIC_OK && pv && dma_ok(&e, pa, b0, b1, bw)) {
      pa.splits = splits; pa.kper = (pa.nk + splits - 1) / splits;
      if (launch_dma_auto(pa, b0, b1, bw, s, -1) == RDEIC_OK) {
        a.splits = splits;
        const long chunks = (long)a.M * (a.cout / 8);
        hipLaunchKernelGGL(splitk_reduce_kernel, dim3((unsigned)((chunks + 255) / 256)), dim3(256), 0, s, a,
                           (const float*)part);
        return launch_status();
      }
    }
  }
  ConvArgs p = a;
  p.bias = nullptr; p.emb = nullptr; p.act = 0; p.res = nullptr; p.gn_part = nullptr; p.ln_rows = nullptr;
  p.out = (char*)part; p.out_ld = a.cout; p.out_f32 = 1;
  p.splits = splits;
  p.kper = (a.nk + splits - 1) / splits;
  dim3 grid(cdiv(a.M, 128), cdiv(a.cout, 128), splits);
  constexpr int lds = conv_lds_bytes<bf16, 128, 128>();
  hipLaunchKernelGGL((conv_kernel<bf16, 128, 128, 2, 2, true, false, true>), grid, dim3(256), lds, s, p);
  a.splits = splits;
  const long chunks = (long)a.M * (a.cout / 8);
  hipLaunchKernelGGL(splitk_reduce_kernel, dim3((unsigned)((chunks + 255) / 256)), dim3(256), 0, s, a,
                     (const float*)part);
  return launch_status();
}

extern "C" int rdeic_conv2d(const rdeic_conv_desc* d, void* stream) { return conv2d_impl(d, -2, stream); }

extern "C" int rdeic_conv2d_tile(const rdeic_conv_desc* d, int32_t tile, void* stream) {
  return conv2d_impl(d, tile, stream);
}

extern "C" int rdeic_conv2d_splitk(const rdeic_conv_desc* d, int32_t splits, float* ws, size_t ws_floats,
                                   void* stream) {
  if (d && d->gn_part && (d->gn_hw <= 0 || d->gn_hw % 64 || (long)d->n * d->ho * d->wo % d->gn_hw))
    return RDEIC_EINVAL;
  int rc;
  {
    rdeic_prof_add_bytes(conv_bytes(d));
    ProfScope ps((hipStream_t)stream, RDEIC_PROF_CONV, conv_flops(d));
    rc = conv2d_splitk_impl(d, splits, ws, ws_floats, stream);
  }
  if (rc == RDEIC_OK) rdeic_count_launch(RDEIC_COUNT_SPLITK);
  if (rc != RDEIC_OK || !d->gn_part) return rc;
  return gn_rows_partial(d->out, (long)d->n * d->ho * d->wo, d->cout, d->out_ld, d->gn_hw, d->gn_part,
                         d->out_f32 ? 0 : 1, (hipStream_t)stream);
}

extern "C" int rdeic_conv2d_up2_phases(const rdeic_conv_desc* d, int64_t phase_stride, int32_t tile, void* stream) {
  if (!d) return RDEIC_EINVAL;
  if (!g_up2_phases || !g_dma || g_conv_path == 0) return 1;
  if (d->gn_part && (d->gn_hw <= 0 || d->gn_hw % 64 || (long)d->n * d->ho * d->wo % d->gn_hw)) return RDEIC_EINVAL;
  if (!up2_phases_ok(d, phase_stride)) return 1;
  bool fused = false;
  int rc;
  {
    const double pix = (double)d->n * d->h * d->w;
    rdeic_prof_add_bytes(2.0 * (pix * d->c0 + 4.0 * d->cout * d->wld + 4.0 * pix * d->cout));
    ProfScope ps((hipStream_t)stream, RDEIC_PROF_CONV, 2.0 * pix * 4.0 * d->c0 * d->cout * 4.0);
    rc = launch_up2_phases(d, phase_stride, tile, (hipStream_t)stream, &fused);
  }
  if (rc == -1) return RDEIC_EINVAL;
  if (rc != RDEIC_OK || !d->gn_part || fused) return rc;
  return gn_rows_partial(d->out, (long)d->n * d->ho * d->wo, d->cout, d->out_ld, d->gn_hw, d->gn_part, 1,
                         (hipStream_t)stream);
}

extern "C" int rdeic_conv2d_up2_group(const rdeic_conv_desc* d) { return d ? up2_phase_group(d) : 0; }

extern "C" int rdeic_conv2d_band_rows(const rdeic_conv_desc* d, int32_t row_tile) { return d ? band_rows(d, row_tile) : 0; }

extern "C" int rdeic_set_conv_path(int32_t path) {
  int prev = g_conv_path;
  g_conv_path = path;
  return prev;
}

extern int rdeic_g_attn64;
extern int rdeic_g_attn512;

extern "C" int rdeic_set_conv_option(int32_t key, int32_t value) {
  if (key == 0) { int prev = g_epi_vec; g_epi_vec = value; return prev; }
  if (key == 1) { int prev = rdeic_g_attn64; rdeic_g_attn64 = value; return prev; }
  if (key == 3) { int prev = g_swz; g_swz = value; return prev; }
  if (key == 4) { int prev = g_force_tile; g_force_tile = value; return prev; }
  if (key == 5) { int prev = g_dma; g_dma = value; return prev; }
  if (key == 6) { int prev = g_halo; g_halo = value; return prev; }
  if (key == 8) { int prev = rdeic_g_attn512; rdeic_g_attn512 = value; return prev; }
  if (key == 9) { int prev = g_halo8; g_halo8 = value; return prev; }
  if (key == 10) { int prev = g_edge; g_edge = value; return prev; }
  if (key == 11) { int prev = g_up2_phases; g_up2_phases = value; return prev; }
  if (key == 12) { int prev = g_launch_limit; g_launch_limit = value > 0 ? value : 0x7fffffff; return prev; }
  return RDEIC_EINVAL;
}
```

### rdeic_amd/finetune.py

```python
from __future__ import annotations

import math
from typing import Dict, List, Optional, Sequence

import torch

from . import autograd as AG
from . import ops
from .rdeic import RDEIC
from .unet import Conv, Down, ResBlock, SpatialTransformer, Up

TRAINABLE_PREFIXES = ("control_model.", "preprocess_model.")


class FineTuneConfig:

    def __init__(self, learning_rate=2e-5, l_guide_weight=3.0, l_bpp_weight=1.0, used_timesteps=300,
                 betas=(0.9, 0.999), eps=1e-8, weight_decay=1e-2, vq_beta=0.25, vq_decay=0.99, vq_temp=0.07,
                 is_refine=False, fixed_step=2):
        self.is_refine, self.fixed_step = bool(is_refine), int(fixed_step)
        self.learning_rate = learning_rate
        self.l_guide_weight = l_guide_weight
        self.l_bpp_weight = l_bpp_weight
        self.used_timesteps = used_timesteps
        self.betas, self.eps, self.weight_decay = betas, eps, weight_decay
        self.vq_beta, self.vq_decay, self.vq_temp = vq_beta, vq_decay, vq_temp


FT_SPLITK = "short"


def _ft_splitk_ctx():
    import contextlib
    if FT_SPLITK == "off":
        return contextlib.nullcontext()
    return ops.splitk_allowed(short_k=FT_SPLITK == "short")


class FineTuner:

    def __init__(self, model: RDEIC, cfg: Optional[FineTuneConfig] = None,
                 embed_prob: Optional[torch.Tensor] = None, lpips=None):
        self.m = model
        self.cfg = cfg or FineTuneConfig(used_timesteps=model.used_timesteps)
        self.lpips = lpips
        if self.cfg.is_refine and lpips is None:
            raise ValueError("the refine step (is_refine) needs an LPIPS model: FineTuner(..., lpips=LPIPS('alex', ...))")
        st = model.store
        self.dtype = st.compute_dtype
        dev = st.device
        names = [n for n in st.names() if n.startswith(TRAINABLE_PREFIXES)]
        self.names = names
        total = sum(math.prod(st.shapes[n]) for n in names)
        self.flat = torch.empty(total, dtype=torch.float32, device=dev)
        self.grad = torch.zeros(total, dtype=torch.float32, device=dev)
        self.exp_avg = torch.zeros(total, dtype=torch.float32, device=dev)
        self.exp_avg_sq = torch.zeros(total, dtype=torch.float32, device=dev)
        self.offsets: Dict[str, tuple] = {}
        off = 0
        for n in names:
            shape = st.shapes[n]
            k = math.prod(shape)
            self.flat[off:off + k].copy_(st.t[n].reshape(-1))
            p = self.flat[off:off + k].view(shape)
            p.requires_grad_(True)
            p.grad = self.grad[off:off + k].view(shape)
            p._rdeic_gview = p.grad
            st.t[n] = p
            self.offsets[n] = (off, k)
            off += k
        st._packed.clear()
        AG.PACKS.clear()
        AG.STEP_PACKS.clear()
        cb = model.preprocess_model.codebook_size
        self.embed_prob = torch.zeros(cb, dtype=torch.float32, device=dev)
        if embed_prob is not None:
            if tuple(embed_prob.shape) != (cb,):
                raise ValueError(f"embed_prob has shape {tuple(embed_prob.shape)}, the codebook has {cb} codes")
            self.embed_prob.copy_(embed_prob.to(torch.float32))
        self.step_count = 0
        self.buckets = None

    def load_optimizer_state(self, exp_avg: torch.Tensor, exp_avg_sq: torch.Tensor, step: int) -> None:
        for dst, src, name in ((self.exp_avg, exp_avg, "exp_avg"), (self.exp_avg_sq, exp_avg_sq, "exp_avg_sq")):
            if src.numel() != dst.numel():
                raise ValueError(f"optimizer.{name} holds {src.numel()} values, the trainable buffer {dst.numel()}")
            dst.copy_(src.reshape(-1).to(torch.float32))
        self.step_count = int(step)

    def enable_ddp(self, bucket_bytes: int = 32 << 20, group=None):
        from .parallel import GradBuckets
        params = [(self.m.store.t[n], o, k) for n, (o, k) in self.offsets.items()]
        self.buckets = GradBuckets(self.grad, params, bucket_bytes, group)
        return self.buckets

    def sync_inference(self) -> None:
        def trainable(key) -> bool:
            for part in key:
                names = part if isinstance(part, tuple) else (part,)
                if any(isinstance(n, str) and n.startswith(TRAINABLE_PREFIXES) for n in names):
                    return True
            return False

        st = self.m.store
        for key in [k for k in st._packed if trainable(k)]:
            del st._packed[key]
        self.m._clear_plans()
        self.m.preprocess_model.update(force=True)

    def p(self, name: str) -> torch.Tensor:
        return self.m.store.t[name]

    def num_params(self) -> int:
        return self.flat.numel()

    def conv(self, x, prefix, *, stride=1, pad=None, up2=False, emb=None, res=None, act=AG.NONE, slope=0.0,
             pixel_shuffle=False, out_f32=False):
        w = self.p(prefix + ".weight")
        b = self.m.store.t.get(prefix + ".bias")
        kh = w.shape[2] if w.dim() == 4 else 1
        cfg = AG.ConvCfg(kh, kh, stride, kh // 2 if pad is None else pad, up2, pixel_shuffle, act, slope, out_f32,
                         key=None if w.requires_grad else prefix)
        return AG.conv2d(x, w, b, emb=emb, res=res, cfg=cfg)

    def linear(self, x, prefix, *, res=None, out_f32=False):
        w = self.p(prefix + ".weight")
        b = self.m.store.t.get(prefix + ".bias")
        return AG.linear(x, w, b, res=res, key=None if w.requires_grad else prefix, out_f32=out_f32)

    def gn(self, x, prefix, groups, eps, silu, passthrough=False):
        return AG.group_norm(x, self.p(prefix + ".weight"), self.p(prefix + ".bias"), groups, eps, silu, passthrough)

    def ln(self, x, prefix, passthrough=False):
        return AG.layer_norm(x, self.p(prefix + ".weight"), self.p(prefix + ".bias"), 1e-5, passthrough)

    def time_embed(self, net, temb):
        e = AG.act(self.linear(temb, net.prefix + "time_embed.0"), AG.SILU)
        e = self.linear(e, net.prefix + "time_embed.2")
        return AG.act(e, AG.SILU)

    def resblock(self, rb: ResBlock, x, semb):
        h, xs = self.gn(x, rb.prefix + ".in_layers.0", rb.gn_in, 1e-5, True, passthrough=True)
        emb = self.linear(semb, rb.prefix + ".emb_layers.1")
        h = self.conv(h, rb.prefix + ".in_layers.2", emb=emb)
        h = self.gn(h, rb.prefix + ".out_layers.0", rb.gn_out, 1e-5, True)
        skip = xs if rb.cin == rb.cout else self.conv(xs, rb.prefix + ".skip_connection")
        return self.conv(h, rb.prefix + ".out_layers.3", res=skip)

    def transformer(self, t: SpatialTransformer, x, ctx_rows, batch):
        B, H, W_, C = x.shape
        L = H * W_
        tb = t.prefix + ".transformer_blocks.0"
        h, xs = self.gn(x, t.prefix + ".norm", t.gn, 1e-6, False, passthrough=True)
        h = self.linear(h.reshape(B * L, C), t.prefix + ".proj_in")
        scale = t.dh ** -0.5
        n1, hs = self.ln(h, tb + ".norm1", passthrough=True)
        q = self.linear(n1, tb + ".attn1.to_q")
        k = self.linear(n1, tb + ".attn1.to_k")
        v = self.linear(n1, tb + ".attn1.to_v")
        o = AG.attention(q, k, v, batch, t.heads, scale)
        h = self.linear(o, tb + ".attn1.to_out.0", res=hs)
        n2, hs = self.ln(h, tb + ".norm2", passthrough=True)
        q = self.linear(n2, tb + ".attn2.to_q")
        k = self.linear(ctx_rows, tb + ".attn2.to_k")
        v = self.linear(ctx_rows, tb + ".attn2.to_v")
        o = AG.attention(q, k, v, batch, t.heads, scale)
        h = self.linear(o, tb + ".attn2.to_out.0", res=hs)
        n3, hs = self.ln(h, tb + ".norm3", passthrough=True)
        g = AG.geglu(self.linear(n3, tb + ".ff.net.0.proj"))
        h = self.linear(g, tb + ".ff.net.2", res=hs)
        out = self.linear(h, t.prefix + ".proj_out", res=xs.reshape(B * L, C))
        return out.view(B, H, W_, C)

    def run_layers(self, net, layers, x, semb, ctx_rows, batch):
        for layer in layers:
            if isinstance(layer, Conv):
                x = self.conv(x, layer.prefix)
            elif isinstance(layer, ResBlock):
                x = self.resblock(layer, x, semb)
            elif isinstance(layer, SpatialTransformer):
                x = self.transformer(layer, x, ctx_rows, batch)
            elif isinstance(layer, Down):
                x = self.conv(x, layer.prefix, stride=2, pad=1)
            elif isinstance(layer, Up):
                x = self.conv(x, layer.prefix, up2=True)
            else:
                raise TypeError(layer)
        return x

    def noise_estimator(self, x_noisy, hint, t, ctx):
        ne = self.m.control_model
        if ne.control_scale != 1.0:
            raise NotImplementedError("control_scale != 1 in the fine-tune step")
        B = x_noisy.shape[0]
        temb = ne.timestep_embedding(t.to(device=x_noisy.device, dtype=torch.int64).contiguous())
        semb_c = self.time_embed(ne.ctrl, temb)
        semb_b = self.time_embed(ne.base, temb)
        Bc, Lc, Dc = ctx.shape
        if Bc != B:
            ctx = ctx.expand(B, Lc, Dc)
        ctx_rows = ctx.reshape(B * Lc, Dc).to(self.dtype).contiguous()
        h_base = AG.cast(x_noisy, self.dtype)
        h_ctr = torch.cat([h_base, hint], dim=3)
        hs_base, hs_ctr = [], []
        for i, (lb, lc) in enumerate(zip(ne.base.input_blocks, ne.ctrl.input_blocks)):
            h_base = self.run_layers(ne.base, lb, h_base, semb_b, ctx_rows, B)
            h_ctr = self.run_layers(ne.ctrl, lc, h_ctr, semb_c, ctx_rows, B)
            h_base = self.conv(h_ctr, ne.enc_zero[i], res=h_base)
            hs_base.append(h_base)
            hs_ctr.append(h_ctr)
        h_base = self.run_layers(ne.base, ne.base.middle, h_base, semb_b, ctx_rows, B)
        h_ctr = self.run_layers(ne.ctrl, ne.ctrl.middle, h_ctr, semb_c, ctx_rows, B)
        h_base = self.conv(h_ctr, ne.mid_zero, res=h_base)
        for i, lb in enumerate(ne.base.output_blocks):
            h_base = self.conv(hs_ctr.pop(), ne.dec_zero[i], res=h_base)
            h_base = torch.cat([h_base, hs_base.pop()], dim=3)
            h_base = self.run_layers(ne.base, lb, h_base, semb_b, ctx_rows, B)
        p = ne.base.prefix
        h = self.gn(h_base, p + "out.0", 32, 1e-5, True)
        return self.conv(h, p + "out.2", out_f32=True)

    def _block(self, blk, x):
        pre, kind, ci, co = blk
        L = AG.LEAKY
        if kind == "conv":
            return self.conv(x, pre)
        if kind == "rb":
            identity = x if ci == co else self.conv(x, pre + ".adaptor")
            out = self.conv(x, pre + ".conv1", act=L, slope=0.01)
            return self.conv(out, pre + ".conv2", act=L, slope=0.01, res=identity)
        if kind == "rbs":
            out = self.conv(x, pre + ".conv1", stride=2, pad=1, act=L, slope=0.01)
            identity = self.conv(x, pre + ".downsample", stride=2, pad=0)
            return self.conv(out, pre + ".conv2", act=L, slope=0.1, res=identity)
        if kind == "rbu":
            out = self.conv(x, pre + ".subpel_conv.0", pixel_shuffle=True, act=L, slope=0.01)
            identity = self.conv(x, pre + ".upsample.0", pixel_shuffle=True)
            return self.conv(out, pre + ".conv", act=L, slope=0.1, res=identity)
        raise ValueError(kind)

    def _seq(self, blocks, x):
        for b in blocks:
            x = self._block(b, x)
        return x

    def _ep(self, name, i, x):
        p = self.m.preprocess_model.p
        h = self.conv(x, f"{p}{name}.{i}.fusion.0", act=AG.GELU)
        h = self.conv(h, f"{p}{name}.{i}.fusion.2", act=AG.GELU)
        return self.conv(h, f"{p}{name}.{i}.fusion.4")

    def _channel_ctx(self, i, x):
        p = self.m.preprocess_model.p
        h = self.conv(x, f"{p}channel_context.{i}.fushion.0", act=AG.GELU)
        h = self.conv(h, f"{p}channel_context.{i}.fushion.2", act=AG.GELU)
        return self.conv(h, f"{p}channel_context.{i}.fushion.4")

    def compression_forward(self, h, slice_noise: Sequence[torch.Tensor]):
        cm = self.m.preprocess_model
# ... 289 lines not shown
```

### rdeic_amd/ops.py

```python
from __future__ import annotations

import ctypes as C
import json
import math
import os
import threading
from dataclasses import dataclass
from typing import Optional

import torch

from . import _lib
from ._lib import ConvDesc, call

NONE, LEAKY, GELU, SILU = 0, 1, 2, 3


def dt_code(t: torch.Tensor) -> int:
    if t.dtype == torch.bfloat16:
        return 1
    if t.dtype == torch.float32:
        return 0
    raise TypeError(f"unsupported activation dtype {t.dtype}")

# ... 47 lines not shown
             1 if dtype == torch.bfloat16 else 0, stream_ptr())
        bias = None if b is None else b.detach().to(device="cuda", dtype=torch.float32).contiguous()
        return ConvParams(packed, wld, bias, cout, cin, kh, kw, stride, pad)


def conv2d(x: torch.Tensor, p: ConvParams, *, x2: Optional[torch.Tensor] = None, up2: bool = False,
           pad_t: Optional[int] = None, pad_l: Optional[int] = None, out_hw=None,
           gn: Optional[torch.Tensor] = None, gn_silu: bool = False, emb: Optional[torch.Tensor] = None,
           act: int = NONE, slope: float = 0.0, res: Optional[torch.Tensor] = None,
           out: Optional[torch.Tensor] = None, out_f32: bool = False, pixel_shuffle: bool = False,
           geglu: bool = False, stats: bool = False, stats_hw: Optional[int] = None,
           images: Optional[int] = None, ln_rows: Optional[torch.Tensor] = None,
           phases: Optional[ConvParams] = None) -> torch.Tensor:
    if gn is not None and _gn_materialize(x, x2, p) and not _halo_eligible(x, x2, p, up2, pad_t, pad_l, out_hw,
                                                                           geglu or pixel_shuffle, out) \
            and not _edge_narrow_eligible(x, x2, p, up2, pad_t, pad_l, out_hw, geglu or pixel_shuffle or emb is not None):
        xin = torch.empty(x.shape[:3] + (p.cin,), dtype=x.dtype, device=x.device)
        c0 = x.shape[3]
        pend = getattr(gn, "_rdeic_pending", None)
        if pend is not None and c0 % 8 == 0 and pix_ld(x) % 8 == 0 and x.data_ptr() % 16 == 0 and \
                (x2 is None or (x2.shape[3] % 8 == 0 and pix_ld(x2) % 8 == 0 and x2.data_ptr() % 16 == 0)):
            p0, pc0, p1, c1, n_, hw_, groups, eps, gamma, beta = pend
            _launch(("gn_apply", float(2 * xin.numel() * xin.element_size()), None), "rdeic_groupnorm_parts_apply",
                    p0.data_ptr(), pc0, _ptr(p1), c1, x.data_ptr(), pix_ld(x), _ptr(x2),
                    pix_ld(x2) if x2 is not None else 0, n_, hw_, groups, float(eps), gamma.data_ptr(),
                    beta.data_ptr(), int(gn_silu), gn.data_ptr(), xin.data_ptr(), pix_ld(xin), stream_ptr())
            del gn._rdeic_pending
        else:
            group_norm_apply(x, gn, gn_silu, out=xin[..., :c0])
            if x2 is not None:
                group_norm_apply(x2, gn[:, c0:], gn_silu, out=xin[..., c0:])
        x, x2, gn = xin, None, None
    n, h, w, c0 = x.shape
    ld0 = pix_ld(x)
    c1, ld1 = 0, 0
    if x2 is not None:
        if x2.shape[:3] != x.shape[:3] or x2.dtype != x.dtype:
            raise ValueError("concat inputs must share n, h, w and dtype")
        c1 = x2.shape[3]
        ld1 = pix_ld(x2)
    if c0 + c1 != p.cin:
        raise ValueError(f"conv expects cin={p.cin}, got {c0}+{c1}")
    if p.weight.dtype != x.dtype:
        raise TypeError(f"weight dtype {p.weight.dtype} != activation dtype {x.dtype}")
    hi, wi = (2 * h, 2 * w) if up2 else (h, w)
    pt = p.pad if pad_t is None else pad_t
    pl = p.pad if pad_l is None else pad_l
    if out_hw is None:
        ho = (hi + 2 * p.pad - p.kh) // p.stride + 1
        wo = (wi + 2 * p.pad - p.kw) // p.stride + 1
    else:
        ho, wo = out_hw
    odt = torch.float32 if (out_f32 or x.dtype == torch.float32) else x.dtype
    if geglu:
        if x.dtype != torch.bfloat16 or c0 % 64 or c1 % 64 or p.cout % 8 or res is not None or emb is not None \
                or act != NONE or out_f32 or pixel_shuffle:
            raise ValueError("fused GEGLU: bf16, 64-channel-aligned input, no residual / emb / activation")
        oshape = (n, ho, wo, p.cout // 2)
    elif pixel_shuffle:
        oshape = (n, 2 * ho, 2 * wo, p.cout // 4)
    else:
        oshape = (n, ho, wo, p.cout)
    if out is None:
        out = torch.empty(oshape, dtype=odt, device=x.device)
    elif tuple(out.shape) != oshape or out.dtype != odt:
        raise ValueError(f"out has shape {tuple(out.shape)}/{out.dtype}, expected {oshape}/{odt}")
    d = ConvDesc()
    d.in0 = x.data_ptr()
    d.in1 = _ptr(x2)
    d.c0, d.c1, d.ld0, d.ld1 = c0, c1, ld0, ld1
    d.n, d.h, d.w, d.up2 = n, h, w, int(up2)
    d.weight, d.wld, d.bias = p.weight.data_ptr(), p.wld, _ptr(p.bias)
    d.cout, d.kh, d.kw, d.stride, d.pad_t, d.pad_l = p.cout, p.kh, p.kw, p.stride, pt, pl
    d.ho, d.wo = ho, wo
    if gn is not None:
        if gn.shape != (n, p.cin, 2):
            raise ValueError("gn affine must be [n, cin, 2]")
        _ab_ready(gn)
        d.gn_ab = gn.data_ptr()
        d.gn_silu = int(gn_silu)
    if emb is not None:
        if emb.dtype != torch.float32 or emb.shape[0] != n or emb.stride(1) != 1:
            raise ValueError("emb must be fp32 [n, >=cout] row-major")
        d.emb = emb.data_ptr()
        d.emb_ld = emb.stride(0)
    d.act, d.act_param = act, float(slope)
    if res is not None:
        if tuple(res.shape) != oshape or res.dtype != odt:
            raise ValueError(f"residual {tuple(res.shape)}/{res.dtype} does not match output {oshape}/{odt}")
        d.res = res.data_ptr()
        d.res_ld = pix_ld(res)
    d.out = out.data_ptr()
    d.out_ld = pix_ld(out)
    d.out_mode = 2 if geglu else (1 if pixel_shuffle else 0)
    d.dtype = dt_code(x)
    d.out_f32 = int(odt == torch.float32 and x.dtype != torch.float32)
    d.batch = 1
    if ln_rows is not None:
        if p.ln_cs is None or ln_rows.dtype != torch.float32 or tuple(ln_rows.shape) != (n * ho * wo, 2) \
                or not ln_rows.is_contiguous():
            raise ValueError("ln_rows needs a ParamStore.conv_ln weight and an fp32 [M, 2] contiguous (mean, rstd)")
        d.ln_rows, d.ln_colsum = ln_rows.data_ptr(), p.ln_cs.data_ptr()
    elif p.ln_cs is not None:
        raise ValueError("a LayerNorm-folded weight needs ln_rows")
    part = None
    if stats and GN_STATS_FUSE and x.dtype == torch.bfloat16 and not (geglu or pixel_shuffle):
        ghw = int(stats_hw or ho * wo)
        nf = int(_lib.load().rdeic_groupnorm_parts_floats(n * ho * wo, p.cout, ghw))
        if nf:
            part = torch.empty(nf, dtype=torch.float32, device=x.device)
            d.gn_part, d.gn_hw = part.data_ptr(), ghw
    flops = 2.0 * n * ho * wo * p.cout * p.kh * p.kw * p.cin
    splits = _splitk_count(x, x2, n * ho * wo, p, gn is not None or pixel_shuffle or geglu, out,
                           n if images is None else images)

    tile = -1
    if splits == 1 and x.dtype == torch.bfloat16 and gn is None and _gn_materialize(x, x2, p):
        key = tile_key(n * ho * wo, c0, c1, p, up2, d.out_mode, res is not None, emb is not None, act, odt)
        tile = TILE_TABLE.get(key, -1) if FORCE_TILE is None else FORCE_TILE
        if AUTOTUNE and FORCE_TILE is None and key not in TILE_TABLE:
            scratch = torch.empty_strided(out.size(), out.stride(), dtype=out.dtype, device=out.device)
            dma = c0 % 64 == 0 and c1 % 64 == 0
            tile = _autotune_tile(d, scratch, DMA_TILE_CANDIDATES if dma else TILE_CANDIDATES)
            if tile >= 0:
                TILE_TABLE[key] = tile

    if up2 and phases is not None and UP2_PHASES and splits == 1 and x.dtype == torch.bfloat16 and gn is None \
            and x2 is None and emb is None and res is None and ln_rows is None and d.out_mode == 0 and not d.out_f32 \
            and (p.kh, p.kw, p.stride, pt, pl) == (3, 3, 1, 1, 1) and (ho, wo) == (2 * h, 2 * w) \
            and phases.weight.dtype == torch.bfloat16 and phases.cout == p.cout and phases.wld == 4 * c0:
        dp = ConvDesc.from_buffer_copy(d)
        dp.weight, dp.wld = phases.weight.data_ptr(), phases.wld
        key = tile_key(n * h * w, c0, 0, phases, 2, 0, False, False, act, odt)
        ptile = TILE_TABLE.get(key, -1) if FORCE_TILE is None else FORCE_TILE
        ptag = ("conv", 2.0 * n * h * w * 4 * c0 * p.cout * 4,
                (n, h, w, c0, c1, p.cout, p.kh, p.stride, False, 2, d.out_mode))
        if _launch_soft(ptag, "rdeic_conv2d_up2_phases", C.byref(dp), phases.weight.stride(0), ptile, stream_ptr()):
            if part is not None:
                _attach_gn_part(out, part, d.gn_hw)
            return out
    tag = ("conv", flops, (n, h, w, c0, c1, p.cout, p.kh, p.stride, gn is not None, int(up2), d.out_mode))
    if splits > 1:
        ws = _splitk_workspace(splits * n * ho * wo * p.cout, x.device)
        _launch(tag, "rdeic_conv2d_splitk", C.byref(d), splits, ws.data_ptr(), ws.numel(), stream_ptr())
    elif tile >= 0:
        _launch(tag, "rdeic_conv2d_tile", C.byref(d), tile, stream_ptr())
    else:
        _launch(tag, "rdeic_conv2d", C.byref(d), stream_ptr())
    if part is not None:
        _attach_gn_part(out, part, d.gn_hw)
    return out


GN_STATS_FUSE = True


def _attach_gn_part(t: torch.Tensor, part: torch.Tensor, hw: int) -> None:
    t._rdeic_gn_part = (part, t.data_ptr(), tuple(t.shape), tuple(t.stride()), hw)


def _gn_part_of(t: Optional[torch.Tensor], hw: int):
    info = getattr(t, "_rdeic_gn_part", None) if t is not None else None
    if info is None:
        return None
    part, ptr, shape, stride, phw = info
    if ptr != t.data_ptr() or shape != tuple(t.shape) or stride != tuple(t.stride()) or phw != hw:
        return None
    return part


AUTOTUNE = False
UP2_PHASES = True
FORCE_TILE: Optional[int] = None
GEGLU_FUSED = True
TILE_CANDIDATES = (0, 1, 3, 4, 6, 8, 10)
DMA_TILE_CANDIDATES = (25, 32, 34, 26, 30, 33, 24, 31, 35, 36, 37, 38)
ALL_TILES = (0, 1, 2, 3, 4, 6, 7, 8, 9, 10) + tuple(range(21, 39))
TILE_TABLE_PATH = os.environ.get("RDEIC_TILE_TABLE") or os.path.join(os.path.dirname(os.path.abspath(__file__)),
                                                                     "conv_tiles.json")


def tile_key(m: int, c0: int, c1: int, p: "ConvParams", up2, out_mode: int, res: bool, emb: bool, act: int,
             odt) -> str:
    return (f"m{m}:c{c0}+{c1}:o{p.cout}:k{p.kh}x{p.kw}:s{p.stride}:up{int(up2)}:om{out_mode}:"
            f"r{int(res)}:e{int(emb)}:a{act}:{'f32' if odt == torch.float32 else 'bf16'}")


def _load_tile_table() -> dict:
    if not os.path.exists(TILE_TABLE_PATH):
        return {}
    with open(TILE_TABLE_PATH) as f:
        tab = json.load(f)["tiles"]
    bad = {k: v for k, v in tab.items() if v not in ALL_TILES}
    if bad:
        raise ValueError(f"{TILE_TABLE_PATH}: unknown tile ids {bad}")
    return tab


TILE_TABLE: dict = _load_tile_table()


def _autotune_tile(d0, scratch: torch.Tensor, candidates=None) -> int:
    if _lib.RECORDER is not None:
        return -1
    d = ConvDesc.from_buffer_copy(d0)
    d.out = scratch.data_ptr()
    s = stream_ptr()
    best, best_t = -1, float("inf")
    for t in (TILE_CANDIDATES if candidates is None else candidates):
        call("rdeic_conv2d_tile", C.byref(d), t, s)
        e0 = torch.cuda.Event(enable_timing=True)
        e1 = torch.cuda.Event(enable_timing=True)
        e0.record()
        for _ in range(2):
            call("rdeic_conv2d_tile", C.byref(d), t, s)
        e1.record()
        e1.synchronize()
        ms = e0.elapsed_time(e1)
        if ms < best_t:
            best, best_t = t, ms
    return best


_SPLITK_WS: dict = {}
_SPLITK_TLS = threading.local()


def splitk_state():
    return getattr(_SPLITK_TLS, "allowed", False), getattr(_SPLITK_TLS, "short", False)


SPLITK_NOMINAL_BATCH = 16
SPLITK_BLOCKS, SPLITK_MAX = 512, 8
SPLITK_TRAIN = None
SPLITK_ENTROPY = True


class splitk_allowed:

    def __init__(self, short_k: bool = False):
        self.short_k = short_k

    def __enter__(self):
        self._prev = splitk_state()
        _SPLITK_TLS.allowed, _SPLITK_TLS.short = True, self.short_k or self._prev[1]
        return self

    def __exit__(self, *exc):
        _SPLITK_TLS.allowed, _SPLITK_TLS.short = self._prev


class splitk_as:

    def __init__(self, state):
        self.state = tuple(state)

    def __enter__(self):
        self._prev = splitk_state()
        _SPLITK_TLS.allowed, _SPLITK_TLS.short = self.state
        return self

    def __exit__(self, *exc):
        _SPLITK_TLS.allowed, _SPLITK_TLS.short = self._prev


def _splitk_count(x, x2, M: int, p: "ConvParams", fused: bool, out: torch.Tensor, n: int) -> int:
    allowed, short = splitk_state()
    if not short:
        M = (M // max(1, n)) * SPLITK_NOMINAL_BATCH
    if not allowed or fused or x.dtype not in (torch.bfloat16, torch.float32) or p.cout % 8 \
            or pix_ld(out) % 8 or out.data_ptr() % 16:
        return 1
    for t in (x, x2):
        if t is not None and (t.shape[3] % 8 or pix_ld(t) % 8 or t.data_ptr() % 16):
            return 1
    if x.dtype == torch.float32:
        tiles = -(-M // 64) * -(-p.cout // 64)
        nk = -(-(p.kh * p.kw * p.cin) // 32)
        if short and tiles < 256 and 8 <= nk < 32:
            return max(1, min(-(-512 // tiles), nk // 4, 16))
        if tiles >= 256 or nk < 32:
            return 1
        return max(1, min(-(-512 // tiles), nk // 8, 16))
    tiles = -(-M // 128) * -(-p.cout // 128)
    nk = -(-(p.kh * p.kw * p.cin) // 64)
    if short and tiles < 128 and 8 <= nk < 32:
        return max(1, min(-(-512 // tiles), nk // 4, 8))
    if short and SPLITK_TRAIN is not None and tiles < 192 and nk >= 32:
        kdiv, smax, target = SPLITK_TRAIN
        return max(1, min(-(-target // tiles), nk // kdiv, smax))
    if tiles >= 192 or nk < 32:
        return 1
    return max(1, min(SPLITK_BLOCKS // tiles, nk // 16, SPLITK_MAX))


_SPLITK_KEEP: list = []


def _splitk_workspace(n: int, device) -> torch.Tensor:
    key = (str(device), stream_ptr())
    buf = _SPLITK_WS.get(key)
    if buf is None or buf.numel() < n:
        buf = torch.empty(n, dtype=torch.float32, device=device)
        _SPLITK_WS[key] = buf
        _SPLITK_KEEP.append(buf)
    return buf


PROFILE = None
PROFILE_OTHER: dict = {}


def _launch(tag, name: str, *args):
    if PROFILE is None:
        return call(name, *args, tag=tag)
    ev0 = torch.cuda.Event(enable_timing=True)
    ev1 = torch.cuda.Event(enable_timing=True)
    ev0.record()
    call(name, *args, tag=tag)
    ev1.record()
    record_profile(tag, ev0, ev1)


def _launch_soft(tag, name: str, *args) -> bool:
    if PROFILE is None:
        return _lib.call_soft(name, *args, tag=tag)
    ev0 = torch.cuda.Event(enable_timing=True)
    ev1 = torch.cuda.Event(enable_timing=True)
    ev0.record()
    if not _lib.call_soft(name, *args, tag=tag):
        return False
    ev1.record()
    record_profile(tag, ev0, ev1)
    return True


def record_profile(tag, ev0, ev1):
    kind, work, meta = tag
    if kind == "conv":
        PROFILE.append((work, ev0, ev1, None, meta))
    else:
        PROFILE_OTHER.setdefault(kind, []).append((work, ev0, ev1))


PROF_KINDS = {"conv": 0, "attention": 1, "attention_dh16": 2, "gn_stats": 3, "gn_apply": 4, "gemm": 5,
              "attention_d512": 6, "conv_bytes": 7}


def prof_start(capacity: int = 65536, every: int = 1) -> None:
    call("rdeic_prof_start", capacity, every)


def prof_stop() -> int:
    return int(_lib.load().rdeic_prof_stop())


def prof_read() -> dict:
    out = {}
    for kind, code in PROF_KINDS.items():
        n, w, ms = C.c_int64(), C.c_double(), C.c_double()
        call("rdeic_prof_read", code, C.byref(n), C.byref(w), C.byref(ms))
        if n.value:
            out[kind] = (n.value, w.value, ms.value)
    return out


def prof_read_keys(kind: str, cap: int = 64) -> list:
    keys, n = (C.c_int64 * cap)(), (C.c_int64 * cap)()
    w, ms = (C.c_double * cap)(), (C.c_double * cap)()
    m = int(_lib.load().rdeic_prof_read_keys(PROF_KINDS[kind], keys, n, w, ms, cap))
    return [(int(keys[i]), int(n[i]), float(w[i]), float(ms[i])) for i in range(max(0, m))]


def attention_key(key: int) -> dict:
    return {"dh": (key >> 48) & 0xffff, "lq": (key >> 32) & 0xffff, "lk": (key >> 16) & 0xffff, "bh": key & 0xffff}


def other_profile_summary():
    out = {}
    for kind, recs in PROFILE_OTHER.items():
        out[kind] = (len(recs), sum(r[0] for r in recs), sum(r[1].elapsed_time(r[2]) for r in recs))
    return out


def conv_profile_summary(records):
    total_ms = 0.0
    total_flops = 0.0
    for rec in records:
        flops, e0, e1 = rec[0], rec[1], rec[2]
        total_ms += e0.elapsed_time(e1)
        total_flops += flops
    return len(records), total_flops, total_ms


def conv_profile_breakdown(records):
    out = {}
    for rec in records:
        flops, e0, e1, meta = rec[0], rec[1], rec[2], rec[4]
        key = str(meta)
        v = out.setdefault(key, [0, 0.0, 0.0])
        v[0] += 1
        v[1] += flops / 1e9
        v[2] += e0.elapsed_time(e1)
    return out


CONV_PATH = 2


def set_conv_path(path: int) -> int:
    global CONV_PATH
    prev = CONV_PATH
    CONV_PATH = int(path)
    _lib.load().rdeic_set_conv_path(CONV_PATH)
    return prev


def set_conv_option(key: int, value: int) -> int:
    return int(_lib.load().rdeic_set_conv_option(int(key), int(value)))


LAUNCH_LIMIT_MAX = 2 ** 31 - 1


def set_launch_limit(nbytes: int) -> int:
    return set_conv_option(12, max(1, min(int(nbytes), LAUNCH_LIMIT_MAX)))


def _band_plan_ok(x: torch.Tensor, p: "ConvParams", out, row_tile: int) -> bool:
    n, h, w, _ = x.shape
    d = ConvDesc()
    d.n, d.h, d.w, d.ho, d.wo = n, h, w, h, w
    d.c0, d.ld0, d.cout = x.shape[3], pix_ld(x), p.cout
    d.kh, d.kw, d.stride, d.pad_t, d.pad_l = 3, 3, 1, 1, 1
    d.out_ld = pix_ld(out) if out is not None else p.cout
    d.dtype = 1
    return int(_lib.load().rdeic_conv2d_band_rows(C.byref(d), row_tile)) > 0


HALO_CONV = 1
HALO_MAX_C = 512


COUNT_HALO_CONV, COUNT_GN_APPLY, COUNT_LAYERNORM, COUNT_HALO_SMALL, COUNT_LN_FUSED, COUNT_SPLITK, COUNT_EDGE, \
    COUNT_GN_PARTS_APPLY, COUNT_DMA_CONV, COUNT_UP2_PHASES = 0, 1, 2, 3, 4, 5, 6, 7, 8, 9


def set_up2_phases(on: bool) -> bool:
    global UP2_PHASES
    prev = UP2_PHASES
    UP2_PHASES = bool(on)
    _lib.load().rdeic_set_conv_option(11, int(UP2_PHASES))
    return prev


def launch_count(kind: int) -> int:
    return int(_lib.load().rdeic_launch_count(int(kind)))


def launch_count_reset() -> None:
    call("rdeic_launch_count_reset")


def set_halo_conv(mode: int) -> int:
    global HALO_CONV
    prev = HALO_CONV
    HALO_CONV = int(mode)
    _lib.load().rdeic_set_conv_option(6, HALO_CONV)
    return prev


def _halo_eligible(x, x2, p: "ConvParams", up2, pad_t, pad_l, out_hw, special, out) -> bool:
    if not HALO_CONV or x.dtype != torch.bfloat16 or x2 is not None or up2 or special:
        return False
    if p.kh != 3 or p.kw != 3 or p.stride != 1 or p.pad != 1 or (pad_t not in (None, 1)) or (pad_l not in (None, 1)):
        return False
    n, h, w, c = x.shape
    if out_hw is not None and tuple(out_hw) != (h, w):
        return False
    if c % 32 or c > min(512, HALO_MAX_C) or p.cout > HALO_MAX_C or p.cout % 128 or h % 4 or w % 64 \
            or x.stride(2) % 8 or x.data_ptr() % 16:
        return False
    if out is not None and (pix_ld(out) % 8 or out.data_ptr() % 16):
        return False
    return _band_plan_ok(x, p, out, 8 if h % 8 == 0 else 4)


EDGE_CONV = 1


def set_edge_conv(mode: int) -> int:
    global EDGE_CONV
    prev = EDGE_CONV
    EDGE_CONV = int(mode)
    _lib.load().rdeic_set_conv_option(10, EDGE_CONV)
    return prev


def _edge_narrow_eligible(x, x2, p: "ConvParams", up2, pad_t, pad_l, out_hw, special) -> bool:
# ... 262 lines not shown
```

### rdeic_amd/params.py

```python
from __future__ import annotations

from typing import Dict, Iterable, Optional, Sequence, Tuple

import torch

from . import ops
from . import weights as W


def fold_up2_phases(w: torch.Tensor, dtype=torch.float32) -> torch.Tensor:
    cout, cin, kh, kw = w.shape
    if (kh, kw) != (3, 3):
        raise ValueError("the phase fold is for 3x3 convs")
    r = torch.tensor([[[1, 0, 0], [0, 1, 1]], [[1, 1, 0], [0, 0, 1]]], dtype=torch.float64, device=w.device)
    f = torch.einsum("ayk,oikl,bxl->aboyxi", r, w.double(), r)
    return f.reshape(4, cout, 4 * cin).to(dtype).contiguous()


class ParamStore:
    def __init__(self, compute_dtype=torch.bfloat16, device="cuda"):
        self.compute_dtype = compute_dtype
        self.device = torch.device(device)
        self.shapes: Dict[str, Tuple[int, ...]] = {}
        self.t: Dict[str, torch.Tensor] = {}
        self._packed: Dict[tuple, ops.ConvParams] = {}

    def declare(self, name: str, shape: Sequence[int]):
        shape = tuple(int(s) for s in shape)
        if name in self.shapes and self.shapes[name] != shape:
            raise ValueError(f"{name} declared twice with different shapes")
        self.shapes[name] = shape

    def declare_conv(self, prefix: str, cout: int, cin: int, k: int, bias: bool = True):
        self.declare(prefix + ".weight", (cout, cin, k, k))
        if bias:
            self.declare(prefix + ".bias", (cout,))

    def declare_linear(self, prefix: str, cout: int, cin: int, bias: bool = True):
        self.declare(prefix + ".weight", (cout, cin))
        if bias:
            self.declare(prefix + ".bias", (cout,))

    def declare_norm(self, prefix: str, c: int):
        self.declare(prefix + ".weight", (c,))
        self.declare(prefix + ".bias", (c,))

    def init_synthetic(self, global_seed: int = W.GLOBAL_SEED, rate_gain: float = 1.0):
        for name, shape in self.shapes.items():
            scale, offset = W.init_spec(name, shape, rate_gain)
            t = torch.empty(shape, dtype=torch.float32, device=self.device)
            ops.fill_uniform(t, W.param_seed(name, global_seed), scale, offset)
            self.t[name] = t
        self._packed.clear()

    def load_state_dict(self, sd: Dict[str, torch.Tensor], strict: bool = True):
        missing = [n for n in self.shapes if n not in sd]
        if strict and missing:
            raise KeyError(f"missing parameters: {missing[:8]}{' ...' if len(missing) > 8 else ''}")
        for name, shape in self.shapes.items():
            if name not in sd:
                continue
            v = sd[name]
            if tuple(v.shape) != shape:
                raise ValueError(f"{name}: checkpoint shape {tuple(v.shape)} != {shape}")
            self.t[name] = v.detach().to(device=self.device, dtype=torch.float32).contiguous()
        self._packed.clear()

    def names(self) -> Iterable[str]:
        return self.shapes.keys()

    def get(self, name: str) -> torch.Tensor:
        return self.t[name]

    def has(self, name: str) -> bool:
        return name in self.shapes

    def conv(self, prefix: str, stride: int = 1, pad: Optional[int] = None, dtype=None,
             scale: float = 1.0, cin_pad: Optional[int] = None, cout_pad: Optional[int] = None) -> ops.ConvParams:
        dtype = dtype or self.compute_dtype
        key = (prefix, stride, pad, dtype, scale, cin_pad, cout_pad)
        p = self._packed.get(key)
        if p is None:
            w = self.t[prefix + ".weight"]
            b = self.t.get(prefix + ".bias")
            if scale != 1.0:
                w, b = w * scale, (None if b is None else b * scale)
            if cin_pad is not None and cin_pad > w.shape[1]:
                w = torch.nn.functional.pad(w, (0, 0) * (w.dim() - 2) + (0, cin_pad - w.shape[1]))
            if cout_pad is not None and cout_pad > w.shape[0]:
                w = torch.nn.functional.pad(w, (0, 0) * (w.dim() - 1) + (0, cout_pad - w.shape[0]))
                if b is not None:
                    b = torch.nn.functional.pad(b, (0, cout_pad - b.shape[0]))
            k = w.shape[-1] if w.dim() == 4 else 1
            p = ops.ConvParams.pack(w, b, stride=stride, pad=(k // 2 if pad is None else pad), dtype=dtype)
            self._packed[key] = p
        return p

    def conv_up2_phases(self, prefix: str) -> Optional[ops.ConvParams]:
        w = self.t[prefix + ".weight"]
        if self.compute_dtype != torch.bfloat16 or w.dim() != 4 or tuple(w.shape[2:]) != (3, 3) or w.shape[1] % 64:
            return None
        key = (prefix, "up2_phases")
        p = self._packed.get(key)
        if p is None:
            b = self.t.get(prefix + ".bias")
            f = fold_up2_phases(w).to(torch.bfloat16).contiguous()
            p = ops.ConvParams(f, 4 * w.shape[1], self.conv(prefix).bias if b is not None else None, w.shape[0],
                               w.shape[1], 2, 2, 1, 1)
            self._packed[key] = p
        return p

    def conv_split_pad(self, prefix: str, c0: int, c0_pad: int, dtype=None) -> ops.ConvParams:
        dtype = dtype or self.compute_dtype
        key = (prefix, "split_pad", c0, c0_pad, dtype)
        p = self._packed.get(key)
        if p is None:
            w = self.t[prefix + ".weight"]
            cout, cin, kh, kw = w.shape
            wp = torch.zeros((cout, cin - c0 + c0_pad, kh, kw), dtype=w.dtype, device=w.device)
            wp[:, :c0] = w[:, :c0]
            wp[:, c0_pad:] = w[:, c0:]
            p = ops.ConvParams.pack(wp, self.t.get(prefix + ".bias"), stride=1, pad=kh // 2, dtype=dtype)
            self._packed[key] = p
        return p

    def conv_geglu(self, prefix: str, dtype=None) -> ops.ConvParams:
        dtype = dtype or self.compute_dtype
        key = (prefix, "geglu", dtype)
        p = self._packed.get(key)
        if p is None:
            w = self.t[prefix + ".weight"]
            b = self.t.get(prefix + ".bias")
            c = w.shape[0] // 2
            if c % 4:
                raise ValueError("GEGLU width must be a multiple of 4")
            perm = torch.arange(2 * c, device=w.device).view(2, c // 4, 4).permute(1, 0, 2).reshape(-1)
            p = ops.ConvParams.pack(w[perm], None if b is None else b[perm], dtype=dtype)
            self._packed[key] = p
        return p

    def conv_ln(self, prefixes: Sequence[str], ln_prefix: str, geglu: bool = False, dtype=None) -> ops.ConvParams:
        dtype = dtype or self.compute_dtype
        key = (tuple(prefixes), "ln", ln_prefix, geglu, dtype)
        p = self._packed.get(key)
        if p is None:
            gamma, beta = self.t[ln_prefix + ".weight"], self.t[ln_prefix + ".bias"]
            ws, bs = [], []
            for pre in prefixes:
                w = self.t[pre + ".weight"]
                b = self.t.get(pre + ".bias")
                ws.append(w)
                bs.append(b if b is not None else torch.zeros(w.shape[0], device=self.device))
            w = torch.cat(ws, 0)
            b = torch.cat(bs, 0).double() + w.double() @ beta.double()
            w = w * gamma[None, :]
            if geglu:
                c = w.shape[0] // 2
                perm = torch.arange(2 * c, device=w.device).view(2, c // 4, 4).permute(1, 0, 2).reshape(-1)
                w, b = w[perm], b[perm]
            p = ops.ConvParams.pack(w, b.float(), dtype=dtype)
            p.ln_cs = p.weight.double().sum(1).float().contiguous()
            self._packed[key] = p
        return p

    def conv_cat(self, prefixes: Sequence[str], dtype=None) -> ops.ConvParams:
        dtype = dtype or self.compute_dtype
        key = (tuple(prefixes), "cat", dtype)
        p = self._packed.get(key)
        if p is None:
            ws, bs = [], []
            for pre in prefixes:
                w = self.t[pre + ".weight"]
                ws.append(w if w.dim() == 4 else w[:, :, None, None])
                b = self.t.get(pre + ".bias")
                bs.append(b if b is not None else torch.zeros(w.shape[0], device=self.device))
            any_bias = any(self.t.get(pre + ".bias") is not None for pre in prefixes)
            w = torch.cat(ws, 0)
            p = ops.ConvParams.pack(w, torch.cat(bs, 0) if any_bias else None, stride=1, pad=w.shape[-1] // 2,
                                    dtype=dtype)
            self._packed[key] = p
        return p
```

### rdeic_amd/rdeic.py

```python
from __future__ import annotations

import os
from pathlib import Path
from typing import Dict, List, Optional, Sequence

import numpy as np
import torch

from . import bitstream, ops
from .compression import Compression
from .config import default_config
from .params import ParamStore
from .unet import NoiseEstimator
from .vae import AutoencoderKL


def make_schedule(timesteps: int, linear_start: float, linear_end: float) -> Dict[str, torch.Tensor]:
    betas = (torch.linspace(linear_start ** 0.5, linear_end ** 0.5, timesteps, dtype=torch.float64) ** 2).numpy()
    alphas = 1.0 - betas
    ac = np.cumprod(alphas, axis=0)
    ac_prev = np.append(1.0, ac[:-1])
    f = lambda a: torch.tensor(a, dtype=torch.float32)
    return dict(betas=f(betas), alphas_cumprod=f(ac), alphas_cumprod_prev=f(ac_prev),
                sqrt_alphas_cumprod=f(np.sqrt(ac)), sqrt_one_minus_alphas_cumprod=f(np.sqrt(1.0 - ac)),
                log_one_minus_alphas_cumprod=f(np.log(1.0 - ac)), sqrt_recip_alphas_cumprod=f(np.sqrt(1.0 / ac)),
                sqrt_recipm1_alphas_cumprod=f(np.sqrt(1.0 / ac - 1)),
                posterior_variance=f(betas * (1.0 - ac_prev) / (1.0 - ac)),
                posterior_log_variance_clipped=f(np.log(np.maximum(betas * (1.0 - ac_prev) / (1.0 - ac), 1e-20))),
                posterior_mean_coef1=f(betas * np.sqrt(ac_prev) / (1.0 - ac)),
                posterior_mean_coef2=f((1.0 - ac_prev) * np.sqrt(alphas) / (1.0 - ac)))


class RDEIC:
    parameterization = "eps"

    def __init__(self, config: Optional[dict] = None, compute_dtype=torch.bfloat16, device="cuda"):
        cfg = config or default_config()
        self.cfg = cfg
        self.store = ParamStore(compute_dtype, device)
        self.control_model = NoiseEstimator(self.store, cfg["unet"], cfg["control"])
        self.first_stage_model = AutoencoderKL(self.store, cfg["ddconfig"], cfg["embed_dim"])
        self.preprocess_model = Compression(self.store, **cfg["compression"])
        self.scale_factor = float(cfg["scale_factor"])
        self.num_timesteps = int(cfg["timesteps"])
        self.used_timesteps = int(cfg["used_timesteps"])
        self.linear_start, self.linear_end = float(cfg["linear_start"]), float(cfg["linear_end"])
        self.channels = 4
        sched = make_schedule(self.num_timesteps, cfg["linear_start"], cfg["linear_end"])
        self._sched_cpu = sched
        self.device = torch.device(device)
        for k, v in sched.items():
            setattr(self, k, v.to(self.device))
        from .plan import PlanCache
        self.use_plans = True
        self._plans = PlanCache()
        self._consts = {}
        self.cond_stage_model = None

    @property
    def compute_dtype(self):
        return self.store.compute_dtype

    def init_synthetic(self, seed: Optional[int] = None, rate_gain: float = 1.0):
        from . import weights as W
        self.store.init_synthetic(W.GLOBAL_SEED if seed is None else seed, rate_gain)
        self._clear_plans()
        return self

    def load_state_dict(self, sd: Dict[str, torch.Tensor], strict: bool = True):
        self.store.load_state_dict({k: v for k, v in sd.items() if k in self.store.shapes}, strict=strict)
        self._clear_plans()
        from . import text
        if text.has_tower(sd):
            tower = text.OpenCLIPTextEncoder(text.TextConfig.from_state_dict(sd), self.compute_dtype, self.device)
            self.cond_stage_model = tower.load_state_dict(sd)
        return self

    def init_text_synthetic(self, cfg=None, seed: Optional[int] = None):
        from . import text
        self.cond_stage_model = text.OpenCLIPTextEncoder(cfg, self.compute_dtype, self.device).init_synthetic(seed)
        return self

    @torch.no_grad()
    def get_learned_conditioning(self, c, vocab_path: Optional[str] = None) -> torch.Tensor:
        tower = self.cond_stage_model
        if tower is None:
            raise RuntimeError("no text tower loaded: the state dict held no cond_stage_model.model.transformer.* "
                               "weights (load a full RDEIC checkpoint, or call init_text_synthetic)")
        if isinstance(c, torch.Tensor):
            return tower.encode_tokens(c)
        if isinstance(c, str):
            c = [c]
        from . import tokenizer
        c = list(c)
        if len(c) == 1 and isinstance(c[0], str) and not tokenizer.clean(c[0]):
            return tower.encode_empty()
        return tower.encode_tokens(tokenizer.tokenize(c, vocab_path, context=tower.cfg.context))

    @property
    def use_plans(self) -> bool:
        return self._use_plans

    @use_plans.setter
    def use_plans(self, v: bool):
        self._use_plans = bool(v)
        self.preprocess_model.use_plans = bool(v)

    def session(self) -> "RDEIC":
        import copy
        from .plan import PlanCache
        s = copy.copy(self)
        s._plans = PlanCache()
        s._consts = {}
        pm = copy.copy(self.preprocess_model)
        pm._plans = PlanCache()
        pm._io = {}
        pm.__dict__.pop("_pin_cache", None)
        s.preprocess_model = pm
        return s

    def _clear_plans(self):
        self._plans.clear()
        self.preprocess_model._plans.clear()
        self.preprocess_model._en = None

    def param_shapes(self):
        return dict(self.store.shapes)

    def encode_images_nhwc(self, img_u8: torch.Tensor) -> torch.Tensor:
        B, H, W_, _ = img_u8.shape
        cpad = 8 if self.compute_dtype == torch.bfloat16 else 3
        x = torch.empty((B, H, W_, cpad), dtype=self.compute_dtype, device=img_u8.device)
        ops.call("rdeic_image_u8_to_nhwc", img_u8.contiguous().data_ptr(), B, H, W_, x.data_ptr(), cpad,
                 ops.dt_code(x), ops.stream_ptr())
        return self.first_stage_model.encode_hc(x, out_mul=self.scale_factor)

    def encode_nchw_nhwc(self, x: torch.Tensor) -> torch.Tensor:
        xh = ops.nchw_to_nhwc(x.to(self.device), self.compute_dtype, mul=2.0, add=-1.0)
        return self.first_stage_model.encode_hc(xh, out_mul=self.scale_factor)

    def q_sample_nhwc(self, x0: torch.Tensor, t: torch.Tensor, noise: torch.Tensor) -> torch.Tensor:
        B = x0.shape[0]
        t = t.to(self.device).long()
        a = self.sqrt_alphas_cumprod[t].contiguous()
        b = self.sqrt_one_minus_alphas_cumprod[t].contiguous()
        out = torch.empty_like(x0)
        ops.call("rdeic_axpby", x0.contiguous().data_ptr(), noise.contiguous().data_ptr(), B, x0[0].numel(),
                 a.data_ptr(), b.data_ptr(), out.data_ptr(), ops.stream_ptr())
        return out

    def eps_nhwc(self, x: torch.Tensor, t: torch.Tensor, guide_hint: torch.Tensor, context: torch.Tensor):
        return self.control_model.forward(x, guide_hint, t, context.to(self.device))

    def eps_uncond_nhwc(self, x: torch.Tensor, t: torch.Tensor, context: torch.Tensor):
        return self.control_model.forward_unconditional(x, t, context.to(self.device))

    def decode_nhwc(self, z: torch.Tensor, out_f32: bool = True, consts=None) -> torch.Tensor:
        B = z.shape[0]
        zs = torch.empty_like(z)
        consts = consts or self._region_consts(B, 0, z.device)
        inv, zero = consts["inv_scale"], consts["zero"]
        ops.call("rdeic_axpby", z.contiguous().data_ptr(), z.contiguous().data_ptr(), B, z[0].numel(), inv.data_ptr(),
                 zero.data_ptr(), zs.data_ptr(), ops.stream_ptr())
        zc = ops.cast(zs, self.compute_dtype)
        return self.first_stage_model.decode(zc, out_f32=out_f32)

    def to_image_u8(self, x: torch.Tensor) -> torch.Tensor:
        B, H, W_, C = x.shape
        img = torch.empty((B, H, W_, 3), dtype=torch.uint8, device=x.device)
        ops.call("rdeic_nhwc_to_image_u8", x.data_ptr(), B, H, W_, ops.pix_ld(x), img.data_ptr(), ops.dt_code(x),
                 ops.stream_ptr())
        return img

    @torch.no_grad()
    def apply_condition_compress(self, x: torch.Tensor, stream_path: str, H: int, W: int) -> float:
        if x.shape[0] != 1:
            raise ValueError("apply_condition_compress codes one image per file (the reference's decompress "
                             "supports batch 1 only); use compress_images for batches")
        h = self.encode_nchw_nhwc(x)
        out = self.preprocess_model.compress(h)[0]
        with Path(stream_path).open("wb") as f:
            bitstream.write_body(f, out["shape"], out["strings"])
        size = bitstream.filesize(stream_path)
        return float(size) * 8 / (H * W)

    @torch.no_grad()
    def apply_condition_decompress(self, stream_path: str):
        with Path(stream_path).open("rb") as f:
            strings, shape = bitstream.read_body(f)
        c_lat, hint = self.preprocess_model.decompress([strings], shape, device=self.device)
        return ops.nhwc_to_nchw(c_lat), ops.nhwc_to_nchw(hint)

    def q_sample(self, x_start: torch.Tensor, t: torch.Tensor, noise: Optional[torch.Tensor] = None):
        if noise is None:
            noise = torch.randn_like(x_start)
        B, C, H, W_ = x_start.shape
        out = self.q_sample_nhwc(x_start.float().contiguous(), t, noise.float().contiguous().to(x_start.device))
        return out

    @torch.no_grad()
    def apply_model(self, x_noisy: torch.Tensor, t: torch.Tensor, cond: dict) -> torch.Tensor:
        ctx = torch.cat(cond["c_crossattn"], 1)
        x = ops.nchw_to_nhwc(x_noisy.float().to(self.device), torch.float32)
        hint = cond["guide_hint"]
        hint_nhwc = ops.nchw_to_nhwc(hint.float().to(self.device), self.compute_dtype)
        eps = self.eps_nhwc(x, t.to(self.device), hint_nhwc, ctx)
        return ops.nhwc_to_nchw(eps)

    @torch.no_grad()
    def apply_model_unconditional(self, x_noisy: torch.Tensor, t: torch.Tensor, cond: dict) -> torch.Tensor:
        ctx = torch.cat(cond["c_crossattn"], 1)
        x = ops.nchw_to_nhwc(x_noisy.float().to(self.device), torch.float32)
        return ops.nhwc_to_nchw(self.eps_uncond_nhwc(x, t.to(self.device), ctx))

    @torch.no_grad()
    def decode_first_stage(self, z: torch.Tensor) -> torch.Tensor:
        zn = ops.nchw_to_nhwc(z.float().to(self.device), torch.float32)
        return ops.nhwc_to_nchw(self.decode_nhwc(zn, out_f32=True))

    @torch.no_grad()
    def compress_images(self, img_u8: torch.Tensor) -> List[bytes]:
        img = img_u8.to(self.device).contiguous()
        outs = self.preprocess_model.compress_with(self.encode_images_nhwc, img)
        return [bitstream.pack_body(o["shape"], o["strings"]) for o in outs]

    @torch.no_grad()
    def decompress_bodies(self, bodies: Sequence[bytes]):
        parsed = [bitstream.unpack_body(b) for b in bodies]
        shape = parsed[0][1]
        if any(p[1] != shape for p in parsed):
            raise ValueError("batched decompress needs one latent shape per batch")
        return self.preprocess_model.decompress([p[0] for p in parsed], shape, device=self.device)

    @staticmethod
    def _sampler(model, sampler: str):
        if sampler == "ddim":
            from .ddim_sampler_relay import DDIMSampler
            return DDIMSampler(model)
        if sampler == "ddpm":
            from .spaced_sampler_relay import SpacedSampler
            return SpacedSampler(model, var_type="fixed_small")
        raise ValueError(f"sampler {sampler!r} (ddpm | ddim)")

    def _step_timesteps(self, steps: int, sampler: str):
        if sampler == "ddpm":
            from .spaced_sampler_relay import space_timesteps
            return sorted(space_timesteps(self.used_timesteps, str(steps)))
        from .ddim_sampler_relay import make_ddim_timesteps
        return [int(t) for t in make_ddim_timesteps(steps, self.used_timesteps)]

    @torch.no_grad()
    def relay_sample_nhwc(self, c_latent: torch.Tensor, guide_hint: torch.Tensor, context: torch.Tensor,
                          noise: torch.Tensor, steps: int, sampler: str = "ddim", step_noise=None) -> torch.Tensor:
        B = c_latent.shape[0]
        t = torch.full((B,), self.used_timesteps - 1, dtype=torch.long, device=self.device)
        x = self.q_sample_nhwc(c_latent, t, noise)
        if sampler == "ddpm":
            return self._sampler(self, sampler).sample_nhwc(steps, x, guide_hint, context, step_noise=step_noise)
        return self._sampler(self, sampler).sample_nhwc(steps, x, guide_hint, context)

    def _region_consts(self, B: int, steps: int, device, sampler: str = "ddim") -> dict:
        key = (B, steps, str(device), sampler)
        c = self._consts.get(key)
        if c is None:
            t = torch.full((B,), self.used_timesteps - 1, dtype=torch.long, device=device)
            c = {"qa": self.sqrt_alphas_cumprod[t].contiguous(), "qb": self.sqrt_one_minus_alphas_cumprod[t].contiguous(),
                 "inv_scale": torch.full((B,), 1.0 / self.scale_factor, dtype=torch.float32, device=device),
                 "zero": torch.zeros((B,), dtype=torch.float32, device=device), "ts": {}}
            if steps:
                for st in self._step_timesteps(steps, sampler):
                    c["ts"][int(st)] = torch.full((B,), int(st), dtype=torch.long, device=device)
            self._consts[key] = c
        return c

    def _relay_decode_u8(self, c_latent, guide_hint, context, noise, steps: int, sampler: str = "ddim",
                         step_noise=None):
        B = c_latent.shape[0]
        c = self._region_consts(B, steps, c_latent.device, sampler)
        x = torch.empty_like(c_latent)
        ops.call("rdeic_axpby", c_latent.data_ptr(), noise.data_ptr(), B, c_latent[0].numel(), c["qa"].data_ptr(),
                 c["qb"].data_ptr(), x.data_ptr(), ops.stream_ptr())
        smp = self._sampler(self, sampler)
        if sampler == "ddpm":
            z = smp.sample_nhwc(steps, x, guide_hint, context, step_noise=list(step_noise.unbind(0)),
                                ts_tensors=c["ts"])
        else:
            z = smp.sample_nhwc(steps, x, guide_hint, context, ts_tensors=c["ts"])
        return self.to_image_u8(self.decode_nhwc(z, out_f32=True, consts=c))

    @torch.no_grad()
    def relay_decode_u8(self, c_latent: torch.Tensor, guide_hint: torch.Tensor, context: torch.Tensor,
                        noise: torch.Tensor, steps: int, sampler: str = "ddim", step_noise=None) -> torch.Tensor:
        ctx = context.to(device=self.device, dtype=self.compute_dtype).contiguous()
        ins = [c_latent.contiguous(), guide_hint.contiguous(), ctx, noise.contiguous()]
        if sampler == "ddpm":
            if step_noise is None or tuple(step_noise.shape) != (steps,) + tuple(noise.shape):
                raise ValueError("sampler 'ddpm' needs step_noise of shape [steps, *noise.shape]")
            ins.append(step_noise.to(device=self.device, dtype=torch.float32).contiguous())
        elif sampler != "ddim":
            raise ValueError(f"sampler {sampler!r} (ddpm | ddim)")
        fn = (lambda a, b, c, d, *e: self._relay_decode_u8(a, b, c, d, steps, sampler, e[0] if e else None))
        if not self.use_plans:
            return fn(*ins)
        key = ("relay_decode", steps, sampler) + tuple((tuple(t.shape), t.dtype) for t in ins)
        return self._plans.run(key, fn, ins).clone()

    @torch.no_grad()
    def codec_images(self, img_u8: torch.Tensor, context: torch.Tensor, noise_nchw: torch.Tensor, steps: int = 2,
                     sampler: str = "ddim", step_noise_nchw: Optional[torch.Tensor] = None):
        bodies = self.compress_images(img_u8)
        c_lat, hint = self.decompress_bodies(bodies)
        noise = ops.nchw_to_nhwc(noise_nchw.float().to(self.device), torch.float32)
        step_noise = None
        if step_noise_nchw is not None:
            step_noise = torch.stack([ops.nchw_to_nhwc(n.float().to(self.device), torch.float32)
                                      for n in step_noise_nchw])
        return self.relay_decode_u8(c_lat, hint, context, noise, steps, sampler, step_noise), bodies
```

### rdeic_amd/unet.py

```python
from __future__ import annotations

from dataclasses import dataclass, field
from typing import List, Optional

import torch

from . import ops
from .params import ParamStore


def find_denominator(number: int, start: int) -> int:
    if start >= number:
        return number
    while start != 0:
        if number % start == 0:
            return start
        start -= 1
    return 1


@dataclass
class ResBlock:
    prefix: str
    cin: int
# ... 14 lines not shown

@dataclass
class Conv:
    prefix: str
    cin: int
    cout: int


@dataclass
class Down:
    prefix: str
    ch: int


@dataclass
class Up:
    prefix: str
    ch: int


class UNet:

    def __init__(self, store: ParamStore, prefix: str, cfg: dict, control: bool = False):
        self.store, self.prefix, self.control = store, prefix, control
        mc0 = cfg["model_channels"]
        self.mc0 = mc0
        ted = mc0 * 4
        self.ted = ted
        ctx_dim = cfg["context_dim"]
        self.ctx_dim = ctx_dim
        store.declare_linear(prefix + "time_embed.0", ted, mc0)
        store.declare_linear(prefix + "time_embed.2", ted, ted)
        mc = int(mc0 * cfg["control_model_ratio"]) if control else mc0
        in_ch = cfg["in_channels"] + (cfg["hint_channels"] if control else 0)
        nhc = cfg["num_head_channels"]
        attn_res = cfg["attention_resolutions"]
        nrb = cfg["num_res_blocks"]
        mults = cfg["channel_mult"]
        self.resblocks: List[ResBlock] = []
        gn = (lambda c: find_denominator(c, 32)) if control else (lambda c: 32)

        def res(pre, cin, cout):
            rb = ResBlock(pre, cin, cout, gn(cin), gn(cout))
            store.declare_norm(pre + ".in_layers.0", cin)
            store.declare_conv(pre + ".in_layers.2", cout, cin, 3)
            store.declare_linear(pre + ".emb_layers.1", cout, ted)
            store.declare_norm(pre + ".out_layers.0", cout)
            store.declare_conv(pre + ".out_layers.3", cout, cout, 3)
            if cin != cout:
                store.declare_conv(pre + ".skip_connection", cout, cin, 1)
            self.resblocks.append(rb)
            return rb

        def st(pre, ch):
            nonlocal nhc_cur
            if control:
                nhc_cur = find_denominator(ch, nhc)
            heads, dh = ch // nhc_cur, nhc_cur
            inner = heads * dh
            store.declare_norm(pre + ".norm", ch)
            store.declare_linear(pre + ".proj_in", inner, ch)
            tb = pre + ".transformer_blocks.0"
            for a in ("attn1", "attn2"):
                kv_in = ch if a == "attn1" else ctx_dim
                store.declare_linear(f"{tb}.{a}.to_q", inner, ch, bias=False)
                store.declare_linear(f"{tb}.{a}.to_k", inner, kv_in, bias=False)
                store.declare_linear(f"{tb}.{a}.to_v", inner, kv_in, bias=False)
                store.declare_linear(f"{tb}.{a}.to_out.0", ch, inner)
            store.declare_linear(tb + ".ff.net.0.proj", inner * 8, inner)
            store.declare_linear(tb + ".ff.net.2", inner, inner * 4)
            for nn_ in ("norm1", "norm2", "norm3"):
                store.declare_norm(f"{tb}.{nn_}", inner)
            store.declare_linear(pre + ".proj_out", inner, ch)
            return SpatialTransformer(pre, ch, heads, dh, find_denominator(ch, 32))

        nhc_cur = nhc
        self.input_blocks: List[list] = []
        p0 = prefix + "input_blocks.0.0"
        store.declare_conv(p0, mc, in_ch, 3)
        self.input_blocks.append([Conv(p0, in_ch, mc)])
        chans, ch, ds, idx = [mc], mc, 1, 1
        for level, mult in enumerate(mults):
            for _ in range(nrb):
                layers = [res(f"{prefix}input_blocks.{idx}.0", ch, mult * mc)]
                ch = mult * mc
                if ds in attn_res:
                    layers.append(st(f"{prefix}input_blocks.{idx}.1", ch))
                self.input_blocks.append(layers)
                chans.append(ch)
                idx += 1
            if level != len(mults) - 1:
                pre = f"{prefix}input_blocks.{idx}.0.op"
                store.declare_conv(pre, ch, ch, 3)
                self.input_blocks.append([Down(pre, ch)])
                chans.append(ch)
                ds *= 2
                idx += 1
        self.enc_out_ch = list(chans)
        self.middle = [res(prefix + "middle_block.0", ch, ch), st(prefix + "middle_block.1", ch),
                       res(prefix + "middle_block.2", ch, ch)]
        self.mid_ch = ch
        self.output_blocks: List[list] = []
        self.dec_out_ch: List[int] = []
        if not control:
            k = 0
            for level, mult in list(enumerate(mults))[::-1]:
                for i in range(nrb + 1):
                    ich = chans.pop()
                    layers = [res(f"{prefix}output_blocks.{k}.0", ch + ich, mc * mult)]
                    ch = mc * mult
                    if ds in attn_res:
                        layers.append(st(f"{prefix}output_blocks.{k}.1", ch))
                    if level and i == nrb:
                        pre = f"{prefix}output_blocks.{k}.{len(layers)}.conv"
                        store.declare_conv(pre, ch, ch, 3)
                        layers.append(Up(pre, ch))
                        ds //= 2
                    self.output_blocks.append(layers)
                    self.dec_out_ch.append(ch)
                    k += 1
            store.declare_norm(prefix + "out.0", ch)
            store.declare_conv(prefix + "out.2", cfg["out_channels"], mc, 3)
        off = 0
        for rb in self.resblocks:
            rb.emb_off = off
            off += rb.cout
        self.emb_total = off

    def time_embed(self, temb: torch.Tensor) -> torch.Tensor:
        s = self.store
        B = temb.shape[0]
        e = ops.linear(temb, s.conv(self.prefix + "time_embed.0", dtype=torch.float32), act=ops.SILU, images=B)
        e = ops.linear(e, s.conv(self.prefix + "time_embed.2", dtype=torch.float32), act=ops.SILU, images=B)
        stacked = s.conv_cat([rb.prefix + ".emb_layers.1" for rb in self.resblocks], dtype=torch.float32)
        return ops.linear(e, stacked, images=B)

    def resblock(self, rb: ResBlock, x: torch.Tensor, emb_all: torch.Tensor,
                 x2: Optional[torch.Tensor] = None, stats: bool = False) -> torch.Tensor:
        s = self.store
        ab1 = ops.group_norm_ab(x, s.get(rb.prefix + ".in_layers.0.weight"), s.get(rb.prefix + ".in_layers.0.bias"),
                                rb.gn_in, 1e-5, x2=x2, defer=True)
        h = ops.conv2d(x, s.conv(rb.prefix + ".in_layers.2"), x2=x2, gn=ab1, gn_silu=True,
                       emb=emb_all[:, rb.emb_off:rb.emb_off + rb.cout], stats=True)
        ab2 = ops.group_norm_ab(h, s.get(rb.prefix + ".out_layers.0.weight"),
                                s.get(rb.prefix + ".out_layers.0.bias"), rb.gn_out, 1e-5, defer=True)
        if rb.cin != rb.cout:
            skip = ops.conv2d(x, s.conv(rb.prefix + ".skip_connection"), x2=x2)
        else:
            if x2 is not None:
                raise ValueError("identity skip with a concatenated input")
            skip = x
        return ops.conv2d(h, s.conv(rb.prefix + ".out_layers.3"), gn=ab2, gn_silu=True, res=skip, stats=stats)

    def transformer(self, t: SpatialTransformer, x: torch.Tensor, ctx_kv_in: torch.Tensor, ctx_batch: int,
                    ctx_len: int, stats: bool = False) -> torch.Tensor:
        s = self.store
        B, H, W_, C = x.shape
        L = H * W_
        rows = B * L
        tb = t.prefix + ".transformer_blocks.0"
        ab = ops.group_norm_ab(x, s.get(t.prefix + ".norm.weight"), s.get(t.prefix + ".norm.bias"), t.gn, 1e-6,
                               defer=True)
        h4 = ops.conv2d(x, s.conv(t.prefix + ".proj_in"), gn=ab, gn_silu=False)
        h = h4.view(rows, C)
        scale = t.dh ** -0.5
        fold = x.dtype == torch.bfloat16 and ops.LN_FOLD and C % 64 == 0
        qkv_names = [tb + ".attn1.to_q", tb + ".attn1.to_k", tb + ".attn1.to_v"]
        if fold:
            qkv = ops.linear(h, s.conv_ln(qkv_names, tb + ".norm1"), ln_rows=ops.layer_norm_rowstats(h), images=B)
        else:
            n1 = ops.layer_norm(h, s.get(tb + ".norm1.weight"), s.get(tb + ".norm1.bias"))
            qkv = ops.linear(n1, s.conv_cat(qkv_names), images=B)
        o = torch.empty((rows, C), dtype=x.dtype, device=x.device)
        ops.attention(qkv[:, :C], qkv[:, C:2 * C], qkv[:, 2 * C:], o, batch=B, heads=t.heads, lq=L, lk=L, dh=t.dh,
                      scale=scale)
        h = ops.linear(o, s.conv(tb + ".attn1.to_out.0"), res=h, images=B)
        if fold:
            q = ops.linear(h, s.conv_ln([tb + ".attn2.to_q"], tb + ".norm2"), ln_rows=ops.layer_norm_rowstats(h),
                           images=B)
        else:
            n2 = ops.layer_norm(h, s.get(tb + ".norm2.weight"), s.get(tb + ".norm2.bias"))
            q = ops.linear(n2, s.conv(tb + ".attn2.to_q"), images=B)
        kv = ops.linear(ctx_kv_in, s.conv_cat([tb + ".attn2.to_k", tb + ".attn2.to_v"]), images=ctx_batch)
        ops.attention(q, kv[:, :C], kv[:, C:], o, batch=B, heads=t.heads, lq=L, lk=ctx_len, dh=t.dh, scale=scale,
                      kv_bcast=(ctx_batch == 1 and B > 1))
        h = ops.linear(o, s.conv(tb + ".attn2.to_out.0"), res=h, images=B)
        if fold and ops.GEGLU_FUSED:
            gg = ops.linear(h, s.conv_ln([tb + ".ff.net.0.proj"], tb + ".norm3", geglu=True),
                            ln_rows=ops.layer_norm_rowstats(h), geglu=True, images=B)
        else:
            n3 = ops.layer_norm(h, s.get(tb + ".norm3.weight"), s.get(tb + ".norm3.bias"))
            if x.dtype == torch.bfloat16 and ops.GEGLU_FUSED and C % 64 == 0:
                gg = ops.linear(n3, s.conv_geglu(tb + ".ff.net.0.proj"), geglu=True, images=B)
            else:
                gg = ops.geglu(ops.linear(n3, s.conv(tb + ".ff.net.0.proj"), images=B))
        h = ops.linear(gg, s.conv(tb + ".ff.net.2"), res=h, images=B)
        if not x.is_contiguous():
            raise ValueError("transformer input must be contiguous NHWC")
        out = ops.linear(h, s.conv(t.prefix + ".proj_out"), res=x.view(rows, C), stats_hw=L if stats else None,
                         images=B)
        return ops.tokens_to_nhwc(out, B, H, W_)

    def run_layers(self, layers, x, emb_all, ctx_rows, ctx_batch, ctx_len, x2=None, stats_last: bool = True):
        s = self.store
        for li, layer in enumerate(layers):
            st = stats_last or li + 1 < len(layers)
            if isinstance(layer, Conv):
                x = ops.conv2d(x, s.conv(layer.prefix), x2=x2, stats=st)
                x2 = None
            elif isinstance(layer, ResBlock):
                x = self.resblock(layer, x, emb_all, x2=x2, stats=st)
                x2 = None
            elif isinstance(layer, SpatialTransformer):
                x = self.transformer(layer, x, ctx_rows, ctx_batch, ctx_len, stats=st)
            elif isinstance(layer, Down):
                x = ops.conv2d(x, s.conv(layer.prefix, stride=2, pad=1), stats=st)
            elif isinstance(layer, Up):
                x = ops.conv2d(x, s.conv(layer.prefix), up2=True, stats=st, phases=s.conv_up2_phases(layer.prefix))
            else:
                raise TypeError(layer)
        return x


class NoiseEstimator:

    def __init__(self, store: ParamStore, unet_cfg: dict, control_cfg: dict,
                 base_prefix: str = "model.diffusion_model.", ctrl_prefix: str = "control_model."):
        self.store = store
        self.base = UNet(store, base_prefix, unet_cfg, control=False)
        self.ctrl = UNet(store, ctrl_prefix + "control_model.", control_cfg, control=True)
        self.model_channels = unet_cfg["model_channels"]
        self.control_scale = float(control_cfg.get("control_scale", 1.0))
        cp = ctrl_prefix
        enc_c, enc_b = self.ctrl.enc_out_ch, self.base.enc_out_ch
        self.enc_zero = [f"{cp}enc_zero_convs_out.{i}.0" for i in range(len(enc_c))]
        for i, pre in enumerate(self.enc_zero):
            store.declare_conv(pre, enc_b[i], enc_c[i], 1)
        self.mid_zero = f"{cp}middle_block_out.0"
        store.declare_conv(self.mid_zero, self.base.mid_ch, self.ctrl.mid_ch, 1)
        self.dec_zero = []
        for i in range(len(enc_c)):
            pre = f"{cp}dec_zero_convs_out.{i}.0"
            cout = self.base.mid_ch if i == 0 else self.base.dec_out_ch[i - 1]
            store.declare_conv(pre, cout, enc_c[-(i + 1)], 1)
            self.dec_zero.append(pre)
        half = self.model_channels // 2
        import math
        self._freqs_cpu = torch.exp(-math.log(10000) * torch.arange(start=0, end=half, dtype=torch.float32) / half)
        self._freqs = None

    def _pad64(self, x: torch.Tensor) -> torch.Tensor:
        B, H, W_, c = x.shape
        key = (B, H, W_, x.dtype, ops.stream_ptr())
        cache = self.__dict__.setdefault("_pad_cache", {})
        buf = cache.get(key)
        if buf is None:
            buf = torch.zeros((B, H, W_, 64), dtype=x.dtype, device=x.device)
            cache[key] = buf
        xc = x.contiguous()
        ops.call("rdeic_act_fwd", xc.data_ptr(), B * H * W_, c, c, None, 0, 0, 0.0, buf.data_ptr(), 64,
                 ops.dt_code(x), ops.stream_ptr())
        return buf

    def timestep_embedding(self, t: torch.Tensor) -> torch.Tensor:
        if self._freqs is None:
            self._freqs = self._freqs_cpu.to(t.device)
        B = t.shape[0]
        out = torch.empty((B, self.model_channels), dtype=torch.float32, device=t.device)
        ops.call("rdeic_timestep_embedding", t.data_ptr(), self._freqs.data_ptr(), B, self.model_channels,
                 out.data_ptr(), ops.stream_ptr())
        return out

    def forward(self, x: torch.Tensor, hint: torch.Tensor, t: torch.Tensor, ctx: torch.Tensor) -> torch.Tensor:
        with ops.splitk_allowed():
            return self._forward(x, hint, t, ctx)

    def forward_unconditional(self, x: torch.Tensor, t: torch.Tensor, ctx: torch.Tensor) -> torch.Tensor:
        with ops.splitk_allowed():
            s = self.store
            dt = s.compute_dtype
            t = t.to(device=x.device, dtype=torch.int64).contiguous()
            emb_b = self.base.time_embed(self.timestep_embedding(t))
            ctx = ctx.to(dt).contiguous()
            Bc, Lc, Dc = ctx.shape
            ctx_rows = ctx.view(Bc * Lc, Dc)
            h_base = ops.cast(x, dt)
            hs_base = []
            for lb in self.base.input_blocks:
                h_base = self.base.run_layers(lb, h_base, emb_b, ctx_rows, Bc, Lc)
                hs_base.append(h_base)
            h_base = self.base.run_layers(self.base.middle, h_base, emb_b, ctx_rows, Bc, Lc)
            for lb in self.base.output_blocks:
                h_base = self.base.run_layers(lb, h_base, emb_b, ctx_rows, Bc, Lc, x2=hs_base.pop())
            p = self.base.prefix
            ab = ops.group_norm_ab(h_base, s.get(p + "out.0.weight"), s.get(p + "out.0.bias"), 32, 1e-5)
            return ops.conv2d(h_base, s.conv(p + "out.2"), gn=ab, gn_silu=True, out_f32=True)

    def _forward(self, x: torch.Tensor, hint: torch.Tensor, t: torch.Tensor, ctx: torch.Tensor) -> torch.Tensor:
        s = self.store
        dt = s.compute_dtype
        B = x.shape[0]
        t = t.to(device=x.device, dtype=torch.int64).contiguous()
        temb = self.timestep_embedding(t)
        emb_c = self.ctrl.time_embed(temb)
        emb_b = self.base.time_embed(temb)
        ctx = ctx.to(dt).contiguous()
        Bc, Lc, Dc = ctx.shape
        ctx_rows = ctx.view(Bc * Lc, Dc)
        sc = self.control_scale * self.control_scale
        h_base = ops.cast(x, dt)
        h_ctr, ctr_x2 = h_base, hint
        hs_base, hs_ctr = [], []
        for i, (lb, lc) in enumerate(zip(self.base.input_blocks, self.ctrl.input_blocks)):
            h_base0 = h_base
            h_base = self.base.run_layers(lb, h_base, emb_b, ctx_rows, Bc, Lc, stats_last=False)
            if i == 0 and dt == torch.bfloat16 and len(lc) == 1 and isinstance(lc[0], Conv) and \
                    h_base0.shape[3] % 64 and hint.shape[3] % 64 == 0:
                h_ctr = ops.conv2d(self._pad64(h_base0), s.conv_split_pad(lc[0].prefix, h_base0.shape[3], 64),
                                   x2=hint, stats=True)
            else:
                h_ctr = self.ctrl.run_layers(lc, h_ctr, emb_c, ctx_rows, Bc, Lc, x2=ctr_x2)
            ctr_x2 = None
            h_base = ops.conv2d(h_ctr, s.conv(self.enc_zero[i], scale=sc), res=h_base, stats=True)
            hs_base.append(h_base)
            hs_ctr.append(h_ctr)
        h_base = self.base.run_layers(self.base.middle, h_base, emb_b, ctx_rows, Bc, Lc, stats_last=False)
        h_ctr = self.ctrl.run_layers(self.ctrl.middle, h_ctr, emb_c, ctx_rows, Bc, Lc, stats_last=False)
        h_base = ops.conv2d(h_ctr, s.conv(self.mid_zero, scale=sc), res=h_base, stats=True)
        nout = len(self.base.output_blocks)
        for i, lb in enumerate(self.base.output_blocks):
            h_base = ops.conv2d(hs_ctr.pop(), s.conv(self.dec_zero[i], scale=sc), res=h_base, stats=True)
            h_base = self.base.run_layers(lb, h_base, emb_b, ctx_rows, Bc, Lc, x2=hs_base.pop(),
                                          stats_last=(i + 1 == nout))
        p = self.base.prefix
        ab = ops.group_norm_ab(h_base, s.get(p + "out.0.weight"), s.get(p + "out.0.bias"), 32, 1e-5)
        return ops.conv2d(h_base, s.conv(p + "out.2"), gn=ab, gn_silu=True, out_f32=True)
```

Measured before the change: 161.2 images/s.

## Fuse 1x1 MLP chain in entropy model and cache cross-attention KV and time embeddings

Adds a HIP kernel that runs three chained 1x1 convolutions with GELU in one launch, keeping the hidden activations in LDS, and uses it in the compression model's fusion MLPs. Separately, the cross-attention K/V projections for every transformer block are computed once per context and reused across the relay-decode steps. Time embeddings attached to the timestep tensor are also reused, keyed by version and store generation. The intent is to cut kernel launches, intermediate global-memory traffic and repeated context projections. The cost is extra LDS use per block, narrow shape specialisation and more cache-invalidation bookkeeping.

```diff
diff --git a/include/rdeic_hip.h b/include/rdeic_hip.h
--- a/include/rdeic_hip.h
+++ b/include/rdeic_hip.h
@@ -51,6 +51,10 @@
 int rdeic_conv2d_band_rows(const rdeic_conv_desc* d, int32_t row_tile);
 int rdeic_set_conv_path(int32_t path);
 int rdeic_set_conv_option(int32_t key, int32_t value);
+int rdeic_mlp3_1x1(const void* in0, int32_t ld0, int32_t c0, const void* in1, int32_t ld1, int32_t c1, int64_t rows,
+                   const void* w1, int32_t wld1, const float* b1, int32_t n1, const void* w2, int32_t wld2,
+                   const float* b2, int32_t n2, const void* w3, int32_t wld3, const float* b3, int32_t n3, void* out,
+                   int32_t out_ld, void* stream);
 
 size_t rdeic_groupnorm_ws_floats(int32_t n, int32_t hw, int32_t c);
 size_t rdeic_groupnorm_parts_floats(int64_t rows, int32_t c, int32_t hw);
@@ -199,6 +203,7 @@
 #define RDEIC_PROF_GEMM 5
 #define RDEIC_PROF_ATTN_D512 6
 #define RDEIC_PROF_CONV_BYTES 7
+#define RDEIC_PROF_MLP3 8
 int rdeic_prof_start(int32_t capacity, int32_t every);
 int rdeic_prof_read_keys(int32_t kind, int64_t* keys, int64_t* launches, double* work, double* ms, int32_t cap);
 #define RDEIC_COUNT_HALO_CONV 0
diff --git a/rdeic_amd/_lib.py b/rdeic_amd/_lib.py
--- a/rdeic_amd/_lib.py
+++ b/rdeic_amd/_lib.py
@@ -66,6 +66,8 @@
     "rdeic_conv2d_up2_phases": (C.c_int, [C.POINTER(ConvDesc), _i64, _i32, _p]),
     "rdeic_conv2d_up2_group": (C.c_int, [C.POINTER(ConvDesc)]),
     "rdeic_conv2d_band_rows": (C.c_int, [C.POINTER(ConvDesc), _i32]),
+    "rdeic_mlp3_1x1": (C.c_int, [_p, _i32, _i32, _p, _i32, _i32, _i64, _p, _i32, _p, _i32, _p, _i32, _p, _i32, _p, _i32,
+                                 _p, _i32, _p, _i32, _p]),
     "rdeic_prof_start": (C.c_int, [_i32, _i32]),
     "rdeic_prof_stop": (C.c_int, []),
     "rdeic_launch_count": (C.c_int64, [_i32]),
diff --git a/rdeic_amd/compression.py b/rdeic_amd/compression.py
--- a/rdeic_amd/compression.py
+++ b/rdeic_amd/compression.py
@@ -116,9 +116,14 @@
         f0, f2, f4 = (f"{p}{name}.{i}.fusion.{j}" for j in (0, 2, 4))
         w0, w2 = s.shapes[f0 + ".weight"][0], s.shapes[f2 + ".weight"][0]
         p0, p2 = self._pad_width(w0), self._pad_width(w2)
-        h = ops.conv2d(x, s.conv(f0, cout_pad=p0), x2=x2, act=ops.GELU)
-        h = ops.conv2d(h, s.conv(f2, cin_pad=p0, cout_pad=p2), act=ops.GELU)
-        return ops.conv2d(h, s.conv(f4, cin_pad=p2))
+        c0, c2, c4 = s.conv(f0, cout_pad=p0), s.conv(f2, cin_pad=p0, cout_pad=p2), s.conv(f4, cin_pad=p2)
+        if p0 is not None:
+            out = ops.mlp3_1x1(x, x2, c0, c2, c4)
+            if out is not None:
+                return out
+        h = ops.conv2d(x, c0, x2=x2, act=ops.GELU)
+        h = ops.conv2d(h, c2, act=ops.GELU)
+        return ops.conv2d(h, c4)
 
     def _channel_ctx(self, i: int, yhat_prefix: torch.Tensor, out: torch.Tensor) -> torch.Tensor:
         s, p = self.store, self.p
diff --git a/rdeic_amd/csrc/coders.cpp b/rdeic_amd/csrc/coders.cpp
--- a/rdeic_amd/csrc/coders.cpp
+++ b/rdeic_amd/csrc/coders.cpp
@@ -420,7 +420,7 @@
 
 int rdeic_version(void) { return 1; }
 
-int rdeic_abi_count(void) { return 112; }
+int rdeic_abi_count(void) { return 113; }
 
 static int pmf_to_quantized_cdf_impl(const float* pmf, int32_t n, int32_t precision, uint32_t* cdf_out) {
   if (!pmf || !cdf_out || n <= 0 || precision <= 0 || precision > 24) return RDEIC_EINVAL;
diff --git a/rdeic_amd/csrc/conv_common.h b/rdeic_amd/csrc/conv_common.h
--- a/rdeic_amd/csrc/conv_common.h
+++ b/rdeic_amd/csrc/conv_common.h
@@ -492,7 +492,7 @@
   }
 }
 
-extern int g_conv_path, g_epi_vec, g_swz, g_force_tile, g_dma, g_halo, g_halo8, g_edge, g_up2_phases;
+extern int g_conv_path, g_epi_vec, g_swz, g_force_tile, g_dma, g_halo, g_halo8, g_edge, g_up2_phases, g_mlp3;
 extern int g_launch_limit;
 
 long image_span(const rdeic_conv_desc* d);
diff --git a/rdeic_amd/csrc/conv_gemm.hip b/rdeic_amd/csrc/conv_gemm.hip
--- a/rdeic_amd/csrc/conv_gemm.hip
+++ b/rdeic_amd/csrc/conv_gemm.hip
@@ -767,5 +767,6 @@
   if (key == 10) { int prev = g_edge; g_edge = value; return prev; }
   if (key == 11) { int prev = g_up2_phases; g_up2_phases = value; return prev; }
   if (key == 12) { int prev = g_launch_limit; g_launch_limit = value > 0 ? value : 0x7fffffff; return prev; }
+  if (key == 13) { int prev = g_mlp3; g_mlp3 = value; return prev; }
   return RDEIC_EINVAL;
 }
diff --git a/rdeic_amd/csrc/mlp3.hip b/rdeic_amd/csrc/mlp3.hip
--- /dev/null
+++ b/rdeic_amd/csrc/mlp3.hip
@@ -0,0 +1,308 @@
+#include "conv_common.h"
+
+namespace rdeic_conv {
+int g_mlp3 = 1;
+}
+
+using namespace rdeic_conv;
+
+namespace {
+
+constexpr int BM = 64;
+constexpr int NT = 256;
+constexpr int RB = 128;
+constexpr int TILE_B = BM * RB;
+
+struct Mlp3Args {
+  const char* in0; const char* in1;
+  int c0, c1, ld0, ld1;
+  int M;
+  const char* w1; const char* w2; const char* w3;
+  int wld1, wld2, wld3;
+  const float* b1; const float* b2; const float* b3;
+  char* out; int out_ld;
+};
+
+template <int N> struct Lay {
+  static constexpr int WGN = N >= 32 ? 2 : 1, WGM = 4 / WGN;
+  static constexpr int WTM = BM / WGM, WTN = N / WGN;
+  static constexpr int TM = WTM / 16, TN = WTN / 16;
+  static constexpr int BR = (N * 8 + NT - 1) / NT;
+  static constexpr int KT = (N + 63) / 64;
+  static_assert(N % 16 == 0 && WTN % 16 == 0 && TM >= 1 && TN >= 1, "layer width");
+};
+
+__device__ __forceinline__ int key(int r) { return chunk_key<bf16, true>(r); }
+
+template <int N>
+__device__ __forceinline__ void load_w(uint4 (&breg)[Lay<N>::BR], const char* w, int wld, int kt, int tid) {
+#pragma unroll
+  for (int i = 0; i < Lay<N>::BR; ++i) {
+    const int cid = tid + NT * i;
+    const int row = cid >> 3, ch = cid & 7;
+    if (row < N) breg[i] = ld16(w + ((long)row * wld + kt * 64 + ch * 8) * 2);
+  }
+}
+
+template <int N>
+__device__ __forceinline__ void store_w(const uint4 (&breg)[Lay<N>::BR], char* ws, int tid) {
+#pragma unroll
+  for (int i = 0; i < Lay<N>::BR; ++i) {
+    const int cid = tid + NT * i;
+    const int row = cid >> 3, ch = cid & 7;
+    if (row < N) *reinterpret_cast<uint4*>(ws + row * RB + (ch ^ key(row)) * 16) = breg[i];
+  }
+}
+
+template <int N>
+__device__ __forceinline__ void mma_tile(f32x4 (&acc)[Lay<N>::TM][Lay<N>::TN], const char* at, const char* wt, int wm,
+                                         int wn, int lrow, int lq) {
+  using L = Lay<N>;
+  const char* Ab = at + (wm * L::WTM + lrow) * RB;
+  const char* Bb = wt + (wn * L::WTN + lrow) * RB;
+#pragma unroll
+  for (int s = 0; s < 2; ++s) {
+    const int so = ((s * 4 + lq) ^ key(lrow)) * 16;
+    bf16x8 bfv[L::TN];
+#pragma unroll
+    for (int j = 0; j < L::TN; ++j) bfv[j] = *reinterpret_cast<const bf16x8*>(Bb + j * 16 * RB + so);
+#pragma unroll
+    for (int i = 0; i < L::TM; ++i) {
+      const bf16x8 af = *reinterpret_cast<const bf16x8*>(Ab + i * 16 * RB + so);
+#pragma unroll
+      for (int j = 0; j < L::TN; ++j) acc[i][j] = __builtin_amdgcn_mfma_f32_16x16x32_bf16(af, bfv[j], acc[i][j], 0, 0, 0);
+    }
+  }
+}
+
+template <int N>
+__device__ __forceinline__ void zero_acc(f32x4 (&acc)[Lay<N>::TM][Lay<N>::TN]) {
+#pragma unroll
+  for (int i = 0; i < Lay<N>::TM; ++i)
+#pragma unroll
+    for (int j = 0; j < Lay<N>::TN; ++j) acc[i][j] = f32x4{0.f, 0.f, 0.f, 0.f};
+}
+
+template <int N>
+__device__ __forceinline__ void load_bias(float (&bv)[Lay<N>::TN], const float* bias, int wn, int lrow) {
+#pragma unroll
+  for (int j = 0; j < Lay<N>::TN; ++j) bv[j] = bias ? bias[wn * Lay<N>::WTN + j * 16 + lrow] : 0.f;
+}
+
+template <int N, int K>
+__device__ __forceinline__ void layer_lds(f32x4 (&acc)[Lay<N>::TM][Lay<N>::TN], const char* h, const char* w, int wld,
+                                          char* ws, int ws_b, int tid, int wm, int wn, int lrow, int lq) {
+  constexpr int NK = Lay<K>::KT;
+  uint4 breg[Lay<N>::BR];
+  zero_acc<N>(acc);
+  load_w<N>(breg, w, wld, 0, tid);
+  store_w<N>(breg, ws, tid);
+  __syncthreads();
+#pragma unroll
+  for (int kt = 0; kt < NK; ++kt) {
+    const int cur = kt & 1;
+    if (kt + 1 < NK) load_w<N>(breg, w, wld, kt + 1, tid);
+    mma_tile<N>(acc, h + kt * TILE_B, ws + cur * ws_b, wm, wn, lrow, lq);
+    if (kt + 1 < NK) store_w<N>(breg, ws + (cur ^ 1) * ws_b, tid);
+    __syncthreads();
+  }
+}
+
+template <int N>
+__device__ __forceinline__ void epi_hidden(const f32x4 (&acc)[Lay<N>::TM][Lay<N>::TN], const float (&bv)[Lay<N>::TN],
+                                           bool has_bias, char* h, int wm, int wn, int lrow, int lq) {
+  using L = Lay<N>;
+#pragma unroll
+  for (int i = 0; i < L::TM; ++i)
+#pragma unroll
+    for (int r = 0; r < 4; ++r) {
+      const int m = wm * L::WTM + i * 16 + lq * 4 + r;
+#pragma unroll
+      for (int j = 0; j < L::TN; ++j) {
+        const int n = wn * L::WTN + j * 16 + lrow;
+        float v = acc[i][j][r];
+        if (has_bias) v += bv[j];
+        v = gelu_f(v);
+        *reinterpret_cast<bf16*>(h + (n >> 6) * TILE_B + m * RB + ((((n & 63) >> 3) ^ key(m)) * 16) + (n & 7) * 2) =
+            from_f32<bf16>(v);
+      }
+    }
+}
+
+template <int N>
+__device__ __forceinline__ void zero_tail(char* h, int tid) {
+  if constexpr (N % 64 != 0) {
+    constexpr int C0 = (N % 64) / 8, NC = 8 - C0;
+    char* t = h + (N / 64) * TILE_B;
+    for (int idx = tid; idx < BM * NC; idx += NT) {
+      const int row = idx / NC, ch = C0 + idx % NC;
+      *reinterpret_cast<uint4*>(t + row * RB + (ch ^ key(row)) * 16) = make_uint4(0, 0, 0, 0);
+    }
+  }
+}
+
+template <int N1, int N2, int N3>
+constexpr int mlp3_lds_bytes() {
+  return 2 * N1 * RB + 2 * TILE_B + (Lay<N1>::KT + Lay<N2>::KT) * TILE_B;
+}
+
+template <int N1, int N2, int N3>
+__global__ __launch_bounds__(NT) void mlp3_kernel(Mlp3Args a) {
+  static_assert(N1 >= N2 && N1 >= N3, "the weight stage is sized by the first layer");
+  static_assert(BM * N3 * 2 <= Lay<N1>::KT * TILE_B, "the output is staged over the first hidden buffer");
+  using L1 = Lay<N1>;
+  using L2 = Lay<N2>;
+  using L3 = Lay<N3>;
+  extern __shared__ __attribute__((aligned(16))) char lds[];
+  constexpr int WS_B = N1 * RB;
+  char* const ws = lds;
+  char* const as = lds + 2 * WS_B;
+  char* const h1 = as + 2 * TILE_B;
+  char* const h2 = h1 + L1::KT * TILE_B;
+
+  const int tid = threadIdx.x, lane = tid & 63, wave = tid >> 6;
+  const int lrow = lane & 15, lq = lane >> 4;
+  const int m0 = blockIdx.x * BM;
+  const int K1 = a.c0 + a.c1, nk1 = (K1 + 63) / 64;
+
+  zero_tail<N1>(h1, tid);
+  zero_tail<N2>(h2, tid);
+
+  {
+    const int wm = wave / L1::WGN, wn = wave % L1::WGN;
+    const int kc = tid & 7;
+    long roff0[2], roff1[2];
+    bool rok[2];
+#pragma unroll
+    for (int i = 0; i < 2; ++i) {
+      const int m = m0 + (tid >> 3) + 32 * i;
+      rok[i] = m < a.M;
+      roff0[i] = (long)m * a.ld0 * 2;
+      roff1[i] = (long)m * a.ld1 * 2;
+    }
+    uint4 areg[2];
+    uint4 breg[L1::BR];
+    auto gather_a = [&](int kt) {
+      const int k0 = kt * 64 + kc * 8;
+      const bool kval = k0 < K1;
+      const bool s0 = k0 < a.c0;
+      const char* base = s0 ? a.in0 : a.in1;
+      const int cs = s0 ? k0 : k0 - a.c0;
+#pragma unroll
+      for (int i = 0; i < 2; ++i) {
+        if (kval && rok[i]) areg[i] = ld16(base + (s0 ? roff0[i] : roff1[i]) + cs * 2);
+        else areg[i] = make_uint4(0, 0, 0, 0);
+      }
+    };
+    auto store_a = [&](int buf) {
+#pragma unroll
+      for (int i = 0; i < 2; ++i) {
+        const int row = (tid >> 3) + 32 * i;
+        *reinterpret_cast<uint4*>(as + buf * TILE_B + row * RB + (kc ^ key(row)) * 16) = areg[i];
+      }
+    };
+    f32x4 acc[L1::TM][L1::TN];
+    float bv[L1::TN];
+    zero_acc<N1>(acc);
+    gather_a(0);
+    load_w<N1>(breg, a.w1, a.wld1, 0, tid);
+    load_bias<N1>(bv, a.b1, wn, lrow);
+    store_a(0);
+    store_w<N1>(breg, ws, tid);
+    __syncthreads();
+    for (int kt = 0; kt < nk1; ++kt) {
+      const int cur = kt & 1;
+      if (kt + 1 < nk1) { gather_a(kt + 1); load_w<N1>(breg, a.w1, a.wld1, kt + 1, tid); }
+      mma_tile<N1>(acc, as + cur * TILE_B, ws + cur * WS_B, wm, wn, lrow, lq);
+      if (kt + 1 < nk1) { store_a(cur ^ 1); store_w<N1>(breg, ws + (cur ^ 1) * WS_B, tid); }
+      __syncthreads();
+    }
+    epi_hidden<N1>(acc, bv, a.b1 != nullptr, h1, wm, wn, lrow, lq);
+  }
+  {
+    const int wm = wave / L2::WGN, wn = wave % L2::WGN;
+    f32x4 acc[L2::TM][L2::TN];
+    float bv[L2::TN];
+    load_bias<N2>(bv, a.b2, wn, lrow);
+    layer_lds<N2, N1>(acc, h1, a.w2, a.wld2, ws, WS_B, tid, wm, wn, lrow, lq);
+    epi_hidden<N2>(acc, bv, a.b2 != nullptr, h2, wm, wn, lrow, lq);
+  }
+  {
+    const int wm = wave / L3::WGN, wn = wave % L3::WGN;
+    f32x4 acc[L3::TM][L3::TN];
+    float bv[L3::TN];
+    load_bias<N3>(bv, a.b3, wn, lrow);
+    layer_lds<N3, N2>(acc, h2, a.w3, a.wld3, ws, WS_B, tid, wm, wn, lrow, lq);
+    bf16* const o = reinterpret_cast<bf16*>(h1);
+#pragma unroll
+    for (int i = 0; i < L3::TM; ++i)
+#pragma unroll
+      for (int r = 0; r < 4; ++r) {
+        const int m = wm * L3::WTM + i * 16 + lq * 4 + r;
+#pragma unroll
+        for (int j = 0; j < L3::TN; ++j) {
+          const int n = wn * L3::WTN + j * 16 + lrow;
+          float v = acc[i][j][r];
+          if (a.b3) v += bv[j];
+          o[m * N3 + n] = from_f32<bf16>(v);
+        }
+      }
+    __syncthreads();
+    constexpr int CPR = N3 / 8;
+    for (int c = tid; c < BM * CPR; c += NT) {
+      const int row = c / CPR, cc = c - row * CPR;
+      const int m = m0 + row;
+      if (m < a.M)
+        *reinterpret_cast<uint4*>(a.out + ((long)m * a.out_ld + cc * 8) * 2) =
+            *reinterpret_cast<const uint4*>(h1 + (row * N3 + cc * 8) * 2);
+    }
+  }
+}
+
+template <int N1, int N2, int N3>
+int launch_mlp3(const Mlp3Args& a, hipStream_t s) {
+  constexpr int lds = mlp3_lds_bytes<N1, N2, N3>();
+  hipLaunchKernelGGL((mlp3_kernel<N1, N2, N3>), dim3(cdiv(a.M, BM)), dim3(NT), lds, s, a);
+  return launch_status();
+}
+
+bool vec_ok(const void* p, int c, int ld) { return c % 8 == 0 && ld % 8 == 0 && ld >= c && ((uintptr_t)p % 16) == 0; }
+
+}
+
+extern "C" int rdeic_mlp3_1x1(const void* in0, int32_t ld0, int32_t c0, const void* in1, int32_t ld1, int32_t c1,
+                              int64_t rows, const void* w1, int32_t wld1, const float* b1, int32_t n1, const void* w2,
+                              int32_t wld2, const float* b2, int32_t n2, const void* w3, int32_t wld3, const float* b3,
+                              int32_t n3, void* out, int32_t out_ld, void* stream) {
+  if (c0 < 0 || c1 < 0 || (c0 > 0 && !in0) || (c1 > 0 && !in1) || c0 + c1 <= 0 || rows <= 0 || rows > 0x7fffffff - BM ||
+      !w1 || !w2 || !w3 || !out || n1 <= 0 || n2 <= 0 || n3 <= 0)
+    return RDEIC_EINVAL;
+  if (!g_mlp3) return 1;
+  if (c0 == 0) { in0 = in1; ld0 = ld1; c0 = c1; in1 = nullptr; ld1 = 0; c1 = 0; }
+  const int K1 = c0 + c1;
+  if (!vec_ok(in0, c0, ld0) || (c1 && !vec_ok(in1, c1, ld1)) || !vec_ok(out, n3, out_ld)) return 1;
+  if (((uintptr_t)w1 | (uintptr_t)w2 | (uintptr_t)w3) % 16) return 1;
+  if (wld1 % 64 || wld1 < K1 || wld2 % 64 || wld2 < n1 || wld3 % 64 || wld3 < n2) return 1;
+  Mlp3Args a;
+  a.in0 = (const char*)in0; a.in1 = (const char*)(c1 ? in1 : in0);
+  a.c0 = c0; a.c1 = c1; a.ld0 = ld0; a.ld1 = c1 ? ld1 : ld0;
+  a.M = (int)rows;
+  a.w1 = (const char*)w1; a.w2 = (const char*)w2; a.w3 = (const char*)w3;
+  a.wld1 = wld1; a.wld2 = wld2; a.wld3 = wld3;
+  a.b1 = b1; a.b2 = b2; a.b3 = b3;
+  a.out = (char*)out; a.out_ld = out_ld;
+  hipStream_t s = (hipStream_t)stream;
+  const double bytes = 2.0 * ((double)rows * (K1 + n3) + (double)n1 * wld1 + (double)n2 * wld2 + (double)n3 * wld3);
+  const long long shape = ((long long)K1 << 48) | ((long long)n1 << 32) | ((long long)n2 << 16) | n3;
+#define RDEIC_MLP3_CLASS(A, B, C)                          \
+  if (n1 == A && n2 == B && n3 == C) {                     \
+    ProfScope ps(s, RDEIC_PROF_MLP3, bytes, shape);        \
+    return launch_mlp3<A, B, C>(a, s);                     \
+  }
+  RDEIC_MLP3_CLASS(32, 32, 16)
+  RDEIC_MLP3_CLASS(64, 64, 32)
+  RDEIC_MLP3_CLASS(128, 128, 64)
+  RDEIC_MLP3_CLASS(256, 192, 128)
+#undef RDEIC_MLP3_CLASS
+  return 1;
+}
diff --git a/rdeic_amd/finetune.py b/rdeic_amd/finetune.py
--- a/rdeic_amd/finetune.py
+++ b/rdeic_amd/finetune.py
@@ -70,6 +70,7 @@
             self.offsets[n] = (off, k)
             off += k
         st._packed.clear()
+        st.touch()
         AG.PACKS.clear()
         AG.STEP_PACKS.clear()
         cb = model.preprocess_model.codebook_size
@@ -105,6 +106,7 @@
         st = self.m.store
         for key in [k for k in st._packed if trainable(k)]:
             del st._packed[key]
+        st.touch()
         self.m._clear_plans()
         self.m.preprocess_model.update(force=True)
 
diff --git a/rdeic_amd/ops.py b/rdeic_amd/ops.py
--- a/rdeic_amd/ops.py
+++ b/rdeic_amd/ops.py
@@ -223,6 +223,35 @@
     return out
 
 
+EP_FUSED = True
+
+
+def mlp3_1x1(x: torch.Tensor, x2: Optional[torch.Tensor], p1: ConvParams, p2: ConvParams,
+             p3: ConvParams) -> Optional[torch.Tensor]:
+    if not EP_FUSED or x.dtype != torch.bfloat16 or any(
+            q.weight.dtype != torch.bfloat16 or (q.kh, q.kw, q.stride, q.pad) != (1, 1, 1, 0) or q.ln_cs is not None
+            for q in (p1, p2, p3)):
+        return None
+    n, h, w, c0 = x.shape
+    c1 = 0 if x2 is None else x2.shape[3]
+    if x2 is not None and (x2.shape[:3] != x.shape[:3] or x2.dtype != x.dtype):
+        raise ValueError("concat inputs must share n, h, w and dtype")
+    if c0 + c1 != p1.cin or p2.cin != p1.cout or p3.cin != p2.cout:
+        raise ValueError(f"chain expects {p1.cin} -> {p2.cin} -> {p3.cin}, got {c0}+{c1} -> {p1.cout} -> {p2.cout}")
+    rows = n * h * w
+    out = torch.empty((n, h, w, p3.cout), dtype=x.dtype, device=x.device)
+    nbytes = 2.0 * (rows * (c0 + c1 + p3.cout) + p1.cout * p1.wld + p2.cout * p2.wld + p3.cout * p3.wld)
+    tag = ("mlp3", nbytes, (rows, c0, c1, p1.cout, p2.cout, p3.cout))
+    ok = _launch_soft(tag, "rdeic_mlp3_1x1", x.data_ptr(), pix_ld(x), c0, _ptr(x2), 0 if x2 is None else pix_ld(x2),
+                      c1, rows, p1.weight.data_ptr(), p1.wld, _ptr(p1.bias), p1.cout, p2.weight.data_ptr(), p2.wld,
+                      _ptr(p2.bias), p2.cout, p3.weight.data_ptr(), p3.wld, _ptr(p3.bias), p3.cout, out.data_ptr(),
+                      pix_ld(out), stream_ptr())
+    return out if ok else None
+
+
+CONST_CACHE = os.environ.get("RDEIC_CONST_CACHE", "1") != "0"
+
+
 GN_STATS_FUSE = True
 
 
@@ -415,7 +444,7 @@
 
 
 PROF_KINDS = {"conv": 0, "attention": 1, "attention_dh16": 2, "gn_stats": 3, "gn_apply": 4, "gemm": 5,
-              "attention_d512": 6, "conv_bytes": 7}
+              "attention_d512": 6, "conv_bytes": 7, "mlp3": 8}
 
 
 def prof_start(capacity: int = 65536, every: int = 1) -> None:
diff --git a/rdeic_amd/params.py b/rdeic_amd/params.py
--- a/rdeic_amd/params.py
+++ b/rdeic_amd/params.py
@@ -1,4 +1,6 @@
 from __future__ import annotations
+
+import itertools
 
 from typing import Dict, Iterable, Optional, Sequence, Tuple
 
@@ -17,6 +19,9 @@
     return f.reshape(4, cout, 4 * cin).to(dtype).contiguous()
 
 
+_GENERATIONS = itertools.count(1)
+
+
 class ParamStore:
     def __init__(self, compute_dtype=torch.bfloat16, device="cuda"):
         self.compute_dtype = compute_dtype
@@ -24,6 +29,10 @@
         self.shapes: Dict[str, Tuple[int, ...]] = {}
         self.t: Dict[str, torch.Tensor] = {}
         self._packed: Dict[tuple, ops.ConvParams] = {}
+        self.touch()
+
+    def touch(self) -> None:
+        self.generation = next(_GENERATIONS)
 
     def declare(self, name: str, shape: Sequence[int]):
         shape = tuple(int(s) for s in shape)
@@ -52,6 +61,7 @@
             ops.fill_uniform(t, W.param_seed(name, global_seed), scale, offset)
             self.t[name] = t
         self._packed.clear()
+        self.touch()
 
     def load_state_dict(self, sd: Dict[str, torch.Tensor], strict: bool = True):
         missing = [n for n in self.shapes if n not in sd]
@@ -65,6 +75,7 @@
                 raise ValueError(f"{name}: checkpoint shape {tuple(v.shape)} != {shape}")
             self.t[name] = v.detach().to(device=self.device, dtype=torch.float32).contiguous()
         self._packed.clear()
+        self.touch()
 
     def names(self) -> Iterable[str]:
         return self.shapes.keys()
diff --git a/rdeic_amd/rdeic.py b/rdeic_amd/rdeic.py
--- a/rdeic_amd/rdeic.py
+++ b/rdeic_amd/rdeic.py
@@ -55,6 +55,8 @@
         self.use_plans = True
         self._plans = PlanCache()
         self._consts = {}
+        self._kv_bufs = {}
+        self._kv_handoff = None
         self.cond_stage_model = None
 
     @property
@@ -112,6 +114,8 @@
         s = copy.copy(self)
         s._plans = PlanCache()
         s._consts = {}
+        s._kv_bufs = {}
+        s._kv_handoff = None
         pm = copy.copy(self.preprocess_model)
         pm._plans = PlanCache()
         pm._io = {}
@@ -149,8 +153,39 @@
                  a.data_ptr(), b.data_ptr(), out.data_ptr(), ops.stream_ptr())
         return out
 
+    KV_CACHE_SHAPES = 4
+
+    def _context_kv(self, context: torch.Tensor, ctx: torch.Tensor):
+        from . import _lib
+        if not ops.CONST_CACHE:
+            return None
+        k = (tuple(ctx.shape), ctx.dtype, str(ctx.device))
+        ent = self._kv_bufs.get(k)
+        cur = (context._version, self.store.generation, ops.stream_ptr())
+        if ent is not None and ent["obj"] is context and ent["cur"] == cur:
+            return ent
+        if _lib.RECORDER is not None:
+            return None
+        if ent is None:
+            if len(self._kv_bufs) >= self.KV_CACHE_SHAPES:
+                return None
+            ent = self._kv_bufs[k] = {"kv": None}
+        ent["kv"] = self.control_model.context_kv(ctx, out=ent["kv"])
+        ent["obj"], ent["cur"], ent["fill"] = context, cur, object()
+        return ent
+
+    def _hand_kv(self, ctx: torch.Tensor, ent) -> None:
+        self._kv_handoff = None if ent is None else (ctx, ctx._version, ent, ent["fill"])
+
     def eps_nhwc(self, x: torch.Tensor, t: torch.Tensor, guide_hint: torch.Tensor, context: torch.Tensor):
-        return self.control_model.forward(x, guide_hint, t, context.to(self.device))
+        ctx = context.to(self.device)
+        h = self._kv_handoff
+        if ops.CONST_CACHE and h is not None and h[0] is context and h[1] == context._version \
+                and h[2]["fill"] is h[3] and h[2]["cur"][1:] == (self.store.generation, ops.stream_ptr()):
+            ent = h[2]
+        else:
+            ent = self._context_kv(context, ctx.to(self.compute_dtype).contiguous())
+        return self.control_model.forward(x, guide_hint, t, ctx, None if ent is None else ent["kv"])
 
     def eps_uncond_nhwc(self, x: torch.Tensor, t: torch.Tensor, context: torch.Tensor):
         return self.control_model.forward_unconditional(x, t, context.to(self.device))
@@ -271,11 +306,18 @@
                 for st in self._step_timesteps(steps, sampler):
                     c["ts"][int(st)] = torch.full((B,), int(st), dtype=torch.long, device=device)
             self._consts[key] = c
+        from . import _lib
+        if ops.CONST_CACHE and _lib.RECORDER is None:
+            gen = self.store.generation
+            for t in c["ts"].values():
+                if self.control_model.attached(t, "_rdeic_emb", gen) is None:
+                    t._rdeic_emb = (t._version, gen, self.control_model.time_embs(t))
         return c
 
     def _relay_decode_u8(self, c_latent, guide_hint, context, noise, steps: int, sampler: str = "ddim",
-                         step_noise=None):
+                         step_noise=None, kv=None):
         B = c_latent.shape[0]
+        self._hand_kv(context, kv)
         c = self._region_consts(B, steps, c_latent.device, sampler)
         x = torch.empty_like(c_latent)
         ops.call("rdeic_axpby", c_latent.data_ptr(), noise.data_ptr(), B, c_latent[0].numel(), c["qa"].data_ptr(),
@@ -299,10 +341,11 @@
             ins.append(step_noise.to(device=self.device, dtype=torch.float32).contiguous())
         elif sampler != "ddim":
             raise ValueError(f"sampler {sampler!r} (ddpm | ddim)")
-        fn = (lambda a, b, c, d, *e: self._relay_decode_u8(a, b, c, d, steps, sampler, e[0] if e else None))
+        kv = self._context_kv(context, ctx)
+        fn = (lambda a, b, c, d, *e: self._relay_decode_u8(a, b, c, d, steps, sampler, e[0] if e else None, kv))
         if not self.use_plans:
             return fn(*ins)
-        key = ("relay_decode", steps, sampler) + tuple((tuple(t.shape), t.dtype) for t in ins)
+        key = ("relay_decode", steps, sampler, kv is not None) + tuple((tuple(t.shape), t.dtype) for t in ins)
         return self._plans.run(key, fn, ins).clone()
 
     @torch.no_grad()
diff --git a/rdeic_amd/unet.py b/rdeic_amd/unet.py
--- a/rdeic_amd/unet.py
+++ b/rdeic_amd/unet.py
@@ -190,8 +190,18 @@
             skip = x
         return ops.conv2d(h, s.conv(rb.prefix + ".out_layers.3"), gn=ab2, gn_silu=True, res=skip, stats=stats)
 
+    def transformers(self):
+        blocks = list(self.input_blocks) + [self.middle] + list(getattr(self, "output_blocks", []))
+        return [l for blk in blocks for l in blk if isinstance(l, SpatialTransformer)]
+
+    def context_kv(self, t: SpatialTransformer, ctx_rows: torch.Tensor, ctx_batch: int,
+                   out: Optional[torch.Tensor] = None) -> torch.Tensor:
+        tb = t.prefix + ".transformer_blocks.0"
+        return ops.linear(ctx_rows, self.store.conv_cat([tb + ".attn2.to_k", tb + ".attn2.to_v"]), images=ctx_batch,
+                          out=out)
+
     def transformer(self, t: SpatialTransformer, x: torch.Tensor, ctx_kv_in: torch.Tensor, ctx_batch: int,
-                    ctx_len: int, stats: bool = False) -> torch.Tensor:
+                    ctx_len: int, stats: bool = False, kv_cache: Optional[dict] = None) -> torch.Tensor:
         s = self.store
         B, H, W_, C = x.shape
         L = H * W_
@@ -219,7 +229,7 @@
         else:
             n2 = ops.layer_norm(h, s.get(tb + ".norm2.weight"), s.get(tb + ".norm2.bias"))
             q = ops.linear(n2, s.conv(tb + ".attn2.to_q"), images=B)
-        kv = ops.linear(ctx_kv_in, s.conv_cat([tb + ".attn2.to_k", tb + ".attn2.to_v"]), images=ctx_batch)
+        kv = kv_cache[t.prefix] if kv_cache is not None else self.context_kv(t, ctx_kv_in, ctx_batch)
         ops.attention(q, kv[:, :C], kv[:, C:], o, batch=B, heads=t.heads, lq=L, lk=ctx_len, dh=t.dh, scale=scale,
                       kv_bcast=(ctx_batch == 1 and B > 1))
         h = ops.linear(o, s.conv(tb + ".attn2.to_out.0"), res=h, images=B)
@@ -239,7 +249,8 @@
                          images=B)
         return ops.tokens_to_nhwc(out, B, H, W_)
 
-    def run_layers(self, layers, x, emb_all, ctx_rows, ctx_batch, ctx_len, x2=None, stats_last: bool = True):
+    def run_layers(self, layers, x, emb_all, ctx_rows, ctx_batch, ctx_len, x2=None, stats_last: bool = True,
+                   kv_cache: Optional[dict] = None):
         s = self.store
         for li, layer in enumerate(layers):
             st = stats_last or li + 1 < len(layers)
@@ -250,7 +261,7 @@
                 x = self.resblock(layer, x, emb_all, x2=x2, stats=st)
                 x2 = None
             elif isinstance(layer, SpatialTransformer):
-                x = self.transformer(layer, x, ctx_rows, ctx_batch, ctx_len, stats=st)
+                x = self.transformer(layer, x, ctx_rows, ctx_batch, ctx_len, stats=st, kv_cache=kv_cache)
             elif isinstance(layer, Down):
                 x = ops.conv2d(x, s.conv(layer.prefix, stride=2, pad=1), stats=st)
             elif isinstance(layer, Up):
@@ -309,9 +320,31 @@
                  out.data_ptr(), ops.stream_ptr())
         return out
 
-    def forward(self, x: torch.Tensor, hint: torch.Tensor, t: torch.Tensor, ctx: torch.Tensor) -> torch.Tensor:
+    def time_embs(self, t: torch.Tensor):
         with ops.splitk_allowed():
-            return self._forward(x, hint, t, ctx)
+            temb = self.timestep_embedding(t.to(dtype=torch.int64).contiguous())
+            emb_c = self.ctrl.time_embed(temb)
+            return self.base.time_embed(temb), emb_c
+
+    def context_kv(self, ctx: torch.Tensor, out: Optional[dict] = None) -> dict:
+        Bc, Lc, Dc = ctx.shape
+        rows = ctx.view(Bc * Lc, Dc)
+        kv = {} if out is None else out
+        with ops.splitk_allowed():
+            for net in (self.base, self.ctrl):
+                for tr in net.transformers():
+                    kv[tr.prefix] = net.context_kv(tr, rows, Bc, out=kv.get(tr.prefix))
+        return kv
+
+    @staticmethod
+    def attached(t: torch.Tensor, name: str, generation: int):
+        a = getattr(t, name, None) if ops.CONST_CACHE else None
+        return a[2] if a is not None and a[0] == t._version and a[1] == generation else None
+
+    def forward(self, x: torch.Tensor, hint: torch.Tensor, t: torch.Tensor, ctx: torch.Tensor,
+                kv: Optional[dict] = None) -> torch.Tensor:
+        with ops.splitk_allowed():
+            return self._forward(x, hint, t, ctx, kv)
 
     def forward_unconditional(self, x: torch.Tensor, t: torch.Tensor, ctx: torch.Tensor) -> torch.Tensor:
         with ops.splitk_allowed():
@@ -334,14 +367,19 @@
             ab = ops.group_norm_ab(h_base, s.get(p + "out.0.weight"), s.get(p + "out.0.bias"), 32, 1e-5)
             return ops.conv2d(h_base, s.conv(p + "out.2"), gn=ab, gn_silu=True, out_f32=True)
 
-    def _forward(self, x: torch.Tensor, hint: torch.Tensor, t: torch.Tensor, ctx: torch.Tensor) -> torch.Tensor:
+    def _forward(self, x: torch.Tensor, hint: torch.Tensor, t: torch.Tensor, ctx: torch.Tensor,
+                 kvc: Optional[dict] = None) -> torch.Tensor:
         s = self.store
         dt = s.compute_dtype
         B = x.shape[0]
-        t = t.to(device=x.device, dtype=torch.int64).contiguous()
-        temb = self.timestep_embedding(t)
-        emb_c = self.ctrl.time_embed(temb)
-        emb_b = self.base.time_embed(temb)
+        embs = self.attached(t, "_rdeic_emb", s.generation)
+        if embs is not None:
+            emb_b, emb_c = embs
+        else:
+            t = t.to(device=x.device, dtype=torch.int64).contiguous()
+            temb = self.timestep_embedding(t)
+            emb_c = self.ctrl.time_embed(temb)
+            emb_b = self.base.time_embed(temb)
         ctx = ctx.to(dt).contiguous()
         Bc, Lc, Dc = ctx.shape
         ctx_rows = ctx.view(Bc * Lc, Dc)
@@ -351,25 +389,25 @@
         hs_base, hs_ctr = [], []
         for i, (lb, lc) in enumerate(zip(self.base.input_blocks, self.ctrl.input_blocks)):
             h_base0 = h_base
-            h_base = self.base.run_layers(lb, h_base, emb_b, ctx_rows, Bc, Lc, stats_last=False)
+            h_base = self.base.run_layers(lb, h_base, emb_b, ctx_rows, Bc, Lc, stats_last=False, kv_cache=kvc)
             if i == 0 and dt == torch.bfloat16 and len(lc) == 1 and isinstance(lc[0], Conv) and \
                     h_base0.shape[3] % 64 and hint.shape[3] % 64 == 0:
                 h_ctr = ops.conv2d(self._pad64(h_base0), s.conv_split_pad(lc[0].prefix, h_base0.shape[3], 64),
                                    x2=hint, stats=True)
             else:
-                h_ctr = self.ctrl.run_layers(lc, h_ctr, emb_c, ctx_rows, Bc, Lc, x2=ctr_x2)
+                h_ctr = self.ctrl.run_layers(lc, h_ctr, emb_c, ctx_rows, Bc, Lc, x2=ctr_x2, kv_cache=kvc)
             ctr_x2 = None
             h_base = ops.conv2d(h_ctr, s.conv(self.enc_zero[i], scale=sc), res=h_base, stats=True)
             hs_base.append(h_base)
             hs_ctr.append(h_ctr)
-        h_base = self.base.run_layers(self.base.middle, h_base, emb_b, ctx_rows, Bc, Lc, stats_last=False)
-        h_ctr = self.ctrl.run_layers(self.ctrl.middle, h_ctr, emb_c, ctx_rows, Bc, Lc, stats_last=False)
+        h_base = self.base.run_layers(self.base.middle, h_base, emb_b, ctx_rows, Bc, Lc, stats_last=False, kv_cache=kvc)
+        h_ctr = self.ctrl.run_layers(self.ctrl.middle, h_ctr, emb_c, ctx_rows, Bc, Lc, stats_last=False, kv_cache=kvc)
         h_base = ops.conv2d(h_ctr, s.conv(self.mid_zero, scale=sc), res=h_base, stats=True)
         nout = len(self.base.output_blocks)
         for i, lb in enumerate(self.base.output_blocks):
             h_base = ops.conv2d(hs_ctr.pop(), s.conv(self.dec_zero[i], scale=sc), res=h_base, stats=True)
             h_base = self.base.run_layers(lb, h_base, emb_b, ctx_rows, Bc, Lc, x2=hs_base.pop(),
-                                          stats_last=(i + 1 == nout))
+                                          stats_last=(i + 1 == nout), kv_cache=kvc)
         p = self.base.prefix
         ab = ops.group_norm_ab(h_base, s.get(p + "out.0.weight"), s.get(p + "out.0.bias"), 32, 1e-5)
         return ops.conv2d(h_base, s.conv(p + "out.2"), gn=ab, gn_silu=True, out_f32=True)
```

Result: no change. 161.5 images/s, median of 4 (+0.2%).
